# KohakuBlueleaf/UwUDiff

Hardware: AMD Instinct MI355X
Metric: train images/sec (whole node), DiT-S/2 256^2 latent (higher is better)
Workload: dtype bf16; 1 GPU; DiT-S/2 (L12 D384 h6), 4x32x32 synthetic latents + pooled-text cond 1280, eps-MSE, AdamW lr1e-6 wd0.01 cosine; random-init weights; per_gpu_batch=768, global_batch=768, parallelism=dp1

## Files before the change

include/uwu_hip.h:

```cpp
#ifndef UWU_HIP_H
#define UWU_HIP_H

#include <stddef.h>
#include <stdint.h>

#ifdef __cplusplus
extern "C" {
#endif

#define UWU_F32 0
#define UWU_BF16 1
#define UWU_I64 2

#define UWU_OK 0
#define UWU_EINVAL (-1)
#define UWU_ELAUNCH (-2)
#define UWU_ENOTIMPL (-3)

#define UWU_PT_EPSILON 0
#define UWU_PT_V 1
#define UWU_PT_SAMPLE 2
#define UWU_PT_RF 3

#define UWU_LOSS_MSE 0
#define UWU_LOSS_L1 1
#define UWU_LOSS_HUBER 2
#define UWU_LOSS_SMOOTH_L1 3

#define UWU_EPI_NONE 0
#define UWU_EPI_BIAS 1
#define UWU_EPI_BIAS_GELU 2
#define UWU_EPI_DGELU 3
#define UWU_EPI_BIAS_SILU 4
#define UWU_EPI_ACCUM 5

const char* uwu_last_error(void);
int uwu_version(void);
int uwu_env_refresh(void);
int uwu_memset_zero(void* p, uint64_t bytes, void* stream);


int uwu_schedule_gather(const int64_t* timesteps, const float* sigmas_desc, const float* all_snr,
                        const float* alphas_cumprod, int n_train, int B, int snr_mode, float gamma,
                        int debias, float* coef, void* stream);

int uwu_rf_time_to_sigma(const float* u01, float sigma_max, const float* log_sigmas_asc, int n_train,
                         int B, float* coef, float* timesteps, void* stream);

int uwu_qsample(const float* x, const float* noise, const float* coef, int B, int64_t n, float* noisy,
                void* noisy_bf16, void* stream);

int uwu_qsample_norm(const float* x, const float* noise, const float* coef, int B, int64_t n, float vae_mean,
                     float vae_std, float* x_norm, float* noisy, void* stream);

int uwu_philox_raw(uint32_t* out, int64_t n_counters, uint64_t seed, uint64_t offset, void* stream);
int uwu_philox_normal(float* out, int64_t n, uint64_t seed, uint64_t offset, void* stream);
int uwu_draw_timesteps(int64_t* timesteps, int n_train, int B, uint64_t seed, uint64_t offset, void* stream);
int uwu_draw_u01(float* u01, int B, uint64_t seed, uint64_t offset, void* stream);
int uwu_qsample_draw(const float* x, const float* coef, int B, int64_t n, int use_norm, float vae_mean, float vae_std,
                     float* x_norm, float* noise, float* noisy, uint64_t seed, uint64_t offset, void* stream);
int uwu_posterior_draw(const float* moments, int ldm, int B, int latent, int64_t HW, float* z, float* mean_out, float* logvar_out,
                       uint64_t seed, uint64_t offset, void* stream);

int uwu_ctx_place(const void* src, int dtype, const int64_t* mask, float* out, int B, int S, int F, int S_total,
                  int F_total, int s_off, int f_off, void* stream);

int uwu_loss_fwd_bwd(const float* x, const float* noise, const float* xt, const void* model_output,
                     int out_dtype, const float* coef, int pred_type, int target_type, int force_convert,
                     int B, int64_t n, float* losses, float* loss_mean, void* grad_out, float* pred,
                     float* target, void* stream);
int uwu_loss_elem_fwd_bwd(const float* x, const float* noise, const float* xt, const void* model_output,
                          int out_dtype, const float* coef, int pred_type, int target_type, int force_convert,
                          int loss_kind, float loss_param, int B, int64_t n, float* losses, float* loss_mean,
                          void* grad_out, float* pred, float* target, void* stream);

int uwu_scale_inplace(void* y, int dtype, int64_t n, const float* scale, void* stream);
int uwu_scale_into(const void* x, void* y, int dtype, int64_t n, const float* scale, void* stream);
int uwu_cast_i64_to_f32(const int64_t* x, float* y, int64_t n, void* stream);

int uwu_aggregate_concat(const void* emb, const int* starts, void* out, int B, int max_n, int64_t unit_bytes,
                         int elem_size, uint64_t pad_bits, void* stream);
int uwu_aggregate_split(const void* cat, const int* starts, void* out, int B, int max_n, int64_t unit_bytes,
                        void* stream);
int uwu_aggregate_first(const void* emb, const int* starts, void* out, int B, int64_t unit_bytes, void* stream);

int uwu_sampler_step(const float* x, const float* eps_cond, const float* eps_uncond, const float* noise, float* out,
                     float* denoised, int64_t n, float cfg, float sigma, float sigma_down, float sigma_up,
                     float s_noise, void* stream);
int uwu_sampler_combine(const float* base, const float* eps_cond, const float* eps_uncond, const float* noise,
                        float* out, int64_t n, float cfg, float a, float b, float c, void* stream);
int uwu_scale_copy(const float* x, float* y, int64_t n, float scale, void* stream);

int uwu_cfg_input(const float* x, float* y, int B, int64_t n, float c_in, void* stream);
int uwu_sampler_combine_draw(const float* base, const float* eps_cond, const float* eps_uncond, float* out, int64_t n, float cfg,
                             float a, float b, float c, uint64_t seed, uint64_t offset, void* stream);
size_t uwu_latent_finish_ws_bytes(int B, int64_t n);
int uwu_latent_finish(const float* x, float* y, int B, int64_t n, int rescale, float vae_std, float vae_mean, void* ws,
                      size_t ws_bytes, void* stream);
int uwu_image_u8(const void* x, int dtype, void* y, int B, int H, int W, void* stream);

#define UWU_FILTER_BILINEAR 0
#define UWU_FILTER_BICUBIC 1
#define UWU_FILTER_LANCZOS 2
int uwu_resample_ksize(int in_size, int out_size, int filter);
int uwu_resample_coeffs(int in_size, int out_size, int filter, int first, int count, int32_t* coeffs, int32_t* bounds);
size_t uwu_image_resize_crop_ws_bytes(int B, const int32_t* meta, int Ht, int Wt, int filter);
int uwu_image_resize_crop(const void* src, int64_t src_bytes, const int64_t* src_off, const int32_t* meta, const int32_t* tables,
                          int64_t tables_len, const int64_t* tab_off, void* out, int dtype, int B, int Ht, int Wt, int filter,
                          int normalize, void* ws, size_t ws_bytes, void* stream);



int uwu_grad_sqnorm_clip(const float* g, int64_t n, float pre_scale, float max_norm, float* partial,
                         float* out, void* stream);

int uwu_adamw_step(float* p, float* g, float* m, float* v, void* p_bf16, int64_t n, float lr,
                   float beta1, float beta2, float eps, float weight_decay, int step, float pre_scale,
                   const float* clip, int zero_grad, void* stream);

int uwu_lion_step(float* p, float* g, float* m, void* p_bf16, int64_t n, double lr, double beta1, double beta2,
                  double weight_decay, float pre_scale, const float* clip, int zero_grad, void* stream);

int uwu_adamw_fp16_step(float* p, float* g, void* m16, void* v16, void* p_bf16, int64_t n, double lr, double beta1,
                        double beta2, double eps, int step, float pre_scale, const float* clip, int zero_grad,
                        void* stream);

int uwu_param_decay(float* p, void* p_bf16, int64_t n, double factor, void* stream);

int uwu_adamw8_step(float* p, float* g, void* state1, void* state2, float* absmax1, float* absmax2, const float* qmap1,
                    const float* qmap2, void* p_bf16, int64_t n, int64_t e0, int64_t e1, double lr, double beta1, double beta2,
                    double eps, double weight_decay, int step, float pre_scale, const float* clip, int zero_grad, void* stream);

int uwu_lion8_step(float* p, float* g, void* state1, float* absmax1, const float* qmap1, void* p_bf16, int64_t n, int64_t e0,
                   int64_t e1, double lr, double beta1, double beta2, double weight_decay, float pre_scale, const float* clip,
                   int zero_grad, void* stream);

#define UWU_PRODIGY_SCALARS 8
#define UWU_PRODIGY_D 0
#define UWU_PRODIGY_D_MAX 1
#define UWU_PRODIGY_D_NUMERATOR 2
#define UWU_PRODIGY_D_DENOM 3
#define UWU_PRODIGY_D_HAT 4
#define UWU_PRODIGY_K 5
#define UWU_PRODIGY_SKIPPED 6
#define UWU_PRODIGY_DLR 7

int uwu_prodigy_stats_blocks(int64_t n);

int uwu_prodigy_stats(const float* p, float* g, const float* p0, float* exp_avg, float* exp_avg_sq, float* s, int64_t n,
                      const double* scalars, double* ws, int64_t ws_slots, int64_t slot0, double lr, double beta1, double beta2,
                      double beta3, double weight_decay, int decouple, double d0, int use_bias_correction, int safeguard_warmup,
                      float pre_scale, const float* clip, int zero_grad, void* stream);

int uwu_prodigy_finalize(double* scalars, const double* ws, int64_t nslots, double lr, double beta1, double beta2, double beta3,
                         double d0, double d_coef, double growth_rate, int use_bias_correction, void* stream);

int uwu_prodigy_apply(float* p, const float* exp_avg, const float* exp_avg_sq, void* p_bf16, int64_t n, const double* scalars,
                      double eps, double weight_decay, int decouple, void* stream);

int uwu_ema_update(float* avg, const float* p, int64_t n, float keep, float take, void* stream);

int uwu_ema_swap(float* avg, float* p, void* p_bf16, int64_t n, int mode, void* stream);

int uwu_sfadamw_step(float* y, float* g, float* z, float* v, void* p_bf16, int64_t n, double lr_t, double beta1, double beta2,
                     double eps, double weight_decay, double c, double bc2, float pre_scale, const float* clip, int zero_grad,
                     void* stream);

int uwu_sf_average(const float* y, const float* z, float* out, int64_t n, double weight, void* stream);

int uwu_cast_f32_to_bf16(const float* src, void* dst, int64_t n, void* stream);
int uwu_cast_bf16_to_f32(const void* src, float* dst, int64_t n, void* stream);

#define UWU_ADAPTER_NORM 0
#define UWU_ADAPTER_LORA 1
#define UWU_ADAPTER_LOKR 2
#define UWU_ADAPTER_LOKR_LOWRANK 3
int uwu_adapter_merge(const float* base, const float* p, const int64_t* table, const int64_t* blk_start, int nseg,
                      int64_t nblocks, float* eff, void* shadow, void* stream);
int uwu_adapter_grad(const float* dw, int64_t N, int64_t K, int kind, const float* p, float* g, int64_t pa, int64_t pb,
                     int64_t pc, int r, int out_k, int in_n, float scale, float* ws, int64_t ws_elems, void* stream);
int uwu_adapter_dora_norms(const float* base, const float* p, const int64_t* table, const int64_t* table_host,
                           const int64_t* blk_start, int nseg, int64_t nblocks, float* norms, void* stream);
int uwu_adapter_dora_merge(const float* base, const float* p, const int64_t* table, const int64_t* table_host,
                           const int64_t* blk_start, int nseg, int64_t nblocks, const float* norms, float* eff, void* shadow,
                           void* stream);
int uwu_adapter_dora_grad(float* dw, const float* base, int64_t N, int64_t K, int kind, const float* p, float* g, int64_t pa,
                          int64_t pb, int64_t pc, int r, int out_k, int in_n, float scale, int64_t dora_off,
                          const float* norms, int wd_on_out, float* ws, int64_t ws_elems, void* stream);
#define UWU_ADAPTER_CONV_LORA 4
#define UWU_ADAPTER_CONV_TUCKER 5
#define UWU_ADAPTER_CONV_LOKR 6
#define UWU_ADAPTER_CONV_LOKR_LOWRANK 7
int uwu_adapter_conv_merge(const float* base, const float* p, const int64_t* table, const int64_t* table_host,
                           const int64_t* blk_start, const int64_t* form_start, int nseg, int64_t nblocks, int64_t nform,
                           float* tws, int64_t tws_elems, float* eff, void* shadow, void* stream);
int uwu_adapter_conv_grad(const float* dw, int64_t cout_store, int64_t cin_store, int64_t cout, int64_t cin, int kind,
                          const float* p, float* g, int64_t pa, int64_t pb, int64_t pc, int r, int out_k, int in_n,
                          float scale, float* ws, int64_t ws_elems, void* stream);

int uwu_comm_unique_id(void* id128);
int uwu_comm_init(const void* id128, int rank, int world, void** comm);
int uwu_allreduce_flat(void* comm, float* buf, int64_t n, void* stream);
int uwu_comm_destroy(void* comm);


int uwu_gemm(const void* A, const void* B, void* C, void* C2, const float* bias, const void* aux,
             int M, int N, int K, int lda, int ldb, int ldc, int ldaux, int transA, int transB, int dtype,
             int c_dtype, int epilogue, int split_k, void* stream);
const char* uwu_gemm_last_kernel(void);

#define UWU_FP8_E4M3 0
#define UWU_FP8_E5M2 1
size_t uwu_gemm_fp8_scratch_bytes(int M, int N, int K);
int uwu_gemm_fp8(const void* A, const void* B, void* C, void* C2, const float* bias, const void* aux, int M, int N,
                 int K, int lda, int ldb, int ldc, int ldaux, int fmt_a, int epilogue, const float* scale_a,
                 const float* scale_b, void* scratch, size_t scratch_bytes, void* stream);

int uwu_gemm_fp8_emit(const void* A, const void* B, void* C, float* colsum, const float* bias, const void* aux, int M, int N,
                      int K, int lda, int ldb, int ldc, int ldaux, int fmt_a, int epilogue, const float* scale_a,
                      const float* scale_b, void* q8, int ldq, void* q8t, int ldqt, const float* q_scale, float* q_amax,
                      void* stream);

int uwu_conv3x3_implicit_ok(int B, int H, int W, int C, int Cout, int stride, int dtype);
int uwu_conv3x3_fwd(const void* x, const void* w, const float* bias, void* y, int B, int H, int W, int C, int Cout,
                    int stride, int dtype, void* stream);
size_t uwu_conv3x3_s2br_ws_bytes(int B, int H, int W, int C, int Cout, int dtype);
int uwu_conv3x3_s2br_fwd(const void* x, const void* w, const float* bias, void* y, int B, int H, int W, int C, int Cout, int dtype,
                         void* ws, size_t ws_bytes, void* stream);
int uwu_conv3x3_dgrad(const void* dy, const void* w, void* dx, int B, int H, int W, int C, int Cout, int stride, int dtype,
                      void* stream);
size_t uwu_conv3x3_wgrad_scratch_bytes(int C, int Cout, int64_t Mo);
int uwu_conv3x3_wgrad(const void* dy, const void* x, float* dw, float* db, int B, int H, int W, int C, int Cout, int stride,
                      int dtype, void* scratch, size_t scratch_bytes, void* stream);

int uwu_fp8_amax(const void* x, int dtype, int64_t n, float* amax, void* stream);
int uwu_fp8_update_scales(float* amax, float* scale, const int* fmt, int n, float margin, void* stream);
int uwu_fp8_quantize(const void* x, int dtype, int M, int K, int ldx, const float* scale, int fmt, void* out, int ldo,
                     void* out_t, int ldt, float* amax, float* colsum, void* stream);

size_t uwu_gemm_wgrad_scratch_bytes(int M, int N, int K);
int uwu_gemm_wgrad(const void* A, const void* B, float* C, float* bias_grad, int M, int N, int K, int lda, int ldb,
                   int ldc, int dtype, int blocks, void* scratch, size_t scratch_bytes, void* stream);

size_t uwu_gemm_wgrad_pair_scratch_bytes(int M_a, int N_a, int M_b, int N_b, int K);
int uwu_gemm_wgrad_pair(const void* A_a, const void* B_a, float* C_a, float* bias_grad_a, int M_a, int N_a, int lda_a,
                        int ldb_a, int ldc_a, const void* A_b, const void* B_b, float* C_b, float* bias_grad_b, int M_b,
                        int N_b, int lda_b, int ldb_b, int ldc_b, int K, int dtype, int blocks, void* scratch,
                        size_t scratch_bytes, void* stream);

int uwu_gemm_prof_enable(int on);
int uwu_gemm_prof_collect(int kind, double* ms, double* flops, int* launches);

enum {
  UWU_PROF_GEMM_FWD = 0, UWU_PROF_GEMM_DGRAD = 1, UWU_PROF_GEMM_WGRAD = 2, UWU_PROF_GEMM_FC1_GELU = 3,
  UWU_PROF_GEMM_FC2_DGELU = 4, UWU_PROF_ATTN_FWD = 5, UWU_PROF_ATTN_BWD = 6, UWU_PROF_LN_FWD = 7, UWU_PROF_LN_BWD = 8,
  UWU_PROF_CONV = 9, UWU_PROF_OTHER = 10
};
int uwu_prof_enable(int on);
int uwu_prof_collect(int tag, int kind, double* ms, double* flops, double* bytes, int* launches);

int uwu_colsum(const void* X, int dtype, int M, int N, int ldx, float* out, int accumulate, void* stream);

int uwu_skinny_linear_ok(int M, int N, int K);
int uwu_skinny_linear_fwd(const float* X, const float* W, const float* bias, float* Y, float* Y2, int M, int N, int K,
                          int epilogue, void* stream);
int uwu_skinny_linear_dgrad(const float* dY, const float* W, float* dX, int M, int N, int K, void* stream);
int uwu_skinny_linear_wgrad(const float* dY, const float* X, float* dW, float* db, int M, int N, int K, void* stream);
int uwu_colsum_batched(const void* X, int dtype, int batch, int M, int N, int ldx, float* out, int accumulate,
                       void* stream);


int uwu_add_ln_modulate_fwd(const void* x_in, const void* y, const float* gate, const float* shift,
                            const float* scale, int mod_ld, void* x_out, void* h, float* mean, float* rstd,
                            int B, int T, int D, float eps, int affine, int dtype, void* stream);
int uwu_add_ln_modulate_fwd_q8(const void* x_in, const void* y, const float* gate, const float* shift, const float* scale,
                               int mod_ld, void* x_out, void* q8, int ldq, void* q8t, int ldqt, const float* q_scale,
                               float* q_amax, float* mean, float* rstd, int B, int T, int D, float eps, void* stream);


int uwu_add_ln_modulate_bwd(const void* dh, const void* x, const float* mean, const float* rstd,
                            const float* scale, const void* dx_in, const void* y, const float* gate,
                            int mod_ld, void* dx_out, void* dy, float* dshift, float* dscale, float* dgate,
                            int B, int T, int D, int affine, int dtype, void* stream);


int uwu_attention_fwd(const void* q, const void* k, const void* v, void* o, float* lse, int B, int Tq, int Tk,
                      int H, int d, int ldq, int ldk, int ldv, int ldo, float scale, int dtype, void* stream);
int uwu_attention_d512_fwd(const void* q, const void* k, const void* v, void* o, int B, int T, int ldq, int ldk, int ldv, int ldo,
                           float scale, int dtype, void* stream);
int uwu_attention_causal_fwd(const void* q, const void* k, const void* v, const int64_t* key_mask, void* o, int B, int T, int H,
                             int d, int ldq, int ldk, int ldv, int ldo, float scale, int dtype, void* stream);
int uwu_text_embed(const int64_t* ids, const void* tok_table, const void* pos_table, void* out, int B, int T, int D, int vocab,
                   int dtype, void* stream);
#define UWU_ACT_QUICK_GELU 0
#define UWU_ACT_GELU_ERF 1
int uwu_bias_act_fwd(const void* x, const float* bias, void* y, int M, int N, int ld, int kind, int dtype, void* stream);
int uwu_text_pool(const int64_t* ids, const void* h, void* pooled, int B, int T, int D, int eos_id, int dtype, void* stream);
int uwu_attention_relbias_fwd(const void* q, const void* k, const void* v, const float* rel_bias, const int64_t* key_mask, void* o,
                              int B, int T, int H, int d, int ldq, int ldk, int ldv, int ldo, float scale, int dtype, void* stream);
int uwu_attention_bidir_fwd(const void* q, const void* k, const void* v, const int64_t* key_mask, void* o, int B, int T, int H, int d,
                            int ldq, int ldk, int ldv, int ldo, float scale, int dtype, void* stream);
int uwu_clip_patches(const void* images, int in_u8, void* out, int B, int S, int p, int ld, int normalize, const float* mean,
                     const float* std, int dtype, void* stream);
int uwu_vit_embed(const void* patch_out, const void* class_embedding, const void* pos_table, void* out, int B, int T, int D, int dtype,
                  void* stream);
int uwu_clip_score_accum(const void* image_embeds, const void* text_embeds, float* scores, double* acc, int B, int P, int dtype,
                         void* stream);
int uwu_timestep_stats_accum(const float* losses, const void* timesteps, int t_dtype, const float* loss_mean, int B, int n_steps,
                             double* stats, double* totals, void* stream);

int uwu_conv2d_ok(int B, int H, int W, int C, int Cout, int KH, int KW, int stride, int ph, int pw, int ldx, int xoff, int ldy, int yoff,
                  int dtype);
size_t uwu_conv2d_ws_bytes(int B, int H, int W, int C, int Cout, int KH, int KW, int stride, int ph, int pw, int ldx, int xoff, int ldy,
                           int yoff, int dtype);
int uwu_conv2d_fwd(const void* x, const void* w, const float* bias, void* y, int B, int H, int W, int C, int Cout, int KH, int KW,
                   int stride, int ph, int pw, int ldx, int xoff, int ldy, int yoff, int relu, int dtype, void* ws, size_t ws_bytes,
                   void* stream);
int uwu_inception_stem(const void* images, int in_u8, void* out, int B, int H, int W, int dtype, void* stream);
#define UWU_POOL_MAX_S2 0
#define UWU_POOL_MAX_S1P1 1
#define UWU_POOL_AVG_S1P1 2
int uwu_pool2d_fwd(const void* x, void* y, int B, int H, int W, int C, int mode, int ldx, int xoff, int ldy, int yoff, int dtype,
                   void* stream);
int uwu_relu_rows(void* y, int64_t M, int N, int ldy, int yoff, int dtype, void* stream);
int uwu_global_avgpool(const void* x, float* out, int B, int HW, int C, int ldx, int dtype, void* stream);
int uwu_fid_stats_accum(const float* features, double* acc, int B, int D, void* stream);

int uwu_add_rmsnorm_fwd(const void* x_in, const void* y, const float* weight, void* x_out, void* n_out, int M, int D, float eps,
                        int dtype, void* stream);
#define UWU_GATE_GELU_TANH 0
int uwu_gated_act_fwd(const void* u, void* out, int M, int F, int ldu, int ldo, int kind, int dtype, void* stream);
int uwu_t5_rel_bias(const float* weight, const int32_t* bucket, float* out, int num_buckets, int H, int n, void* stream);
int uwu_token_embed(const int64_t* ids, const void* tok_table, void* out, int B, int T, int D, int vocab, int dtype, void* stream);
int uwu_attention_bwd(const void* q, const void* k, const void* v, const void* o, const void* dO,
                      const float* lse, float* delta, void* dq, void* dk, void* dv, int B, int Tq, int Tk, int H,
                      int d, int ldq, int ldk, int ldv, int ldo, float scale, int dtype, void* stream);
int uwu_attention_bias_fwd(const void* q, const void* k, const void* v, const float* key_bias, void* o, float* lse,
                           int B, int Tq, int Tk, int H, int d, int ldq, int ldk, int ldv, int ldo, float scale,
                           int dtype, void* stream);
int uwu_attention_bias_bwd(const void* q, const void* k, const void* v, const float* key_bias, const void* o,
                           const void* dO, const float* lse, float* delta, void* dq, void* dk, void* dv, int B,
                           int Tq, int Tk, int H, int d, int ldq, int ldk, int ldv, int ldo, float scale, int dtype,
                           void* stream);
int uwu_attention_route(int pass, int Tq, int Tk, int d, int ldq, int ldk, int ldv, int ldo, int dtype);

int uwu_axial_rope_fwd(const void* x, const float* pos, const float* fh, const float* fw, void* y, int64_t rows,
                       int H, int d, int ldx, int dtype, void* stream);
int uwu_axial_rope_bwd(const void* x, const void* dy, const float* pos, const float* fh, const float* fw, void* dx,
                       float* dfh, float* dfw, int64_t rows, int H, int d, int ldx, int dtype, void* stream);

int uwu_axial_rope_bwd_shared(const void* x, const void* dy, const float* pos, int pos_rows, const float* fh, const float* fw,
                              void* dx, float* dfh, float* dfw, int64_t rows, int H, int d, int ldx, int dtype, void* stream);
int uwu_axial_rope_table(const float* pos, const float* fh, const float* fw, float* tab, int T, int H, int d, int ldt,
                         void* stream);
int uwu_attention_rope_fwd(const void* q, const void* k, const void* v, const float* rope_tab, void* o, float* lse, int B,
                           int T, int H, int d, int ldq, int ldk, int ldv, int ldo, int ldt, float scale, int dtype,
                           void* stream);
int uwu_attention_rope_bwd(const void* q, const void* k, const void* v, const float* rope_tab, const void* o, const void* dO,
                           const float* lse, void* dq, void* dk, void* dv, int B, int T, int H, int d, int ldq, int ldk,
                           int ldv, int ldo, int ldt, float scale, int dtype, void* stream);


int uwu_timestep_embedding(const float* t, int B, int dim, float max_period, void* out, int dtype,
                           void* stream);
int uwu_silu_fwd(const void* x, void* y, int64_t n, int dtype, void* stream);
int uwu_silu_bwd(const void* x, const void* dy, void* dx, int64_t n, int dtype, void* stream);

int uwu_add(const void* a, const void* b, void* out, int64_t n, int dtype, void* stream);
int uwu_transpose_bf16(const void* src, void* dst, int rows, int cols, int ld_src, int ld_dst, void* stream);

int uwu_patchify(const float* img, void* tok, int B, int C, int H, int W, int p, int dtype, void* stream);
int uwu_unpatchify(const void* tok, int dtype, float* img, int B, int C, int H, int W, int p, void* stream);
int uwu_add_pos(void* x, const float* pos, int B, int T, int D, int dtype, void* stream);


int uwu_groupnorm_fwd(const void* x, const float* gamma, const float* beta, void* y, float* mean, float* rstd,
                      int B, int HW, int C, int G, float eps, int silu, int dtype, void* stream);
size_t uwu_groupnorm_fwd_det_ws_bytes(int B, int HW, int C, int G);
int uwu_groupnorm_fwd_det(const void* x, const float* gamma, const float* beta, void* y, float* mean, float* rstd, void* ws,
                          size_t ws_bytes, int B, int HW, int C, int G, float eps, int silu, int dtype, void* stream);
int uwu_groupnorm_bwd(const void* dy, const void* x, const float* mean, const float* rstd, const float* gamma,
                      const float* beta, void* dx, float* dgamma, float* dbeta, float* ws, int B, int HW, int C, int G,
                      int silu, int dtype, void* stream);
int uwu_im2col3x3(const void* x, void* col, int B, int H, int W, int C, int stride, int dtype, void* stream);
int uwu_col2im3x3(const void* dcol, void* dx, int B, int H, int W, int C, int stride, int dtype, void* stream);
int uwu_geglu_fwd(const void* hg, void* out, int64_t M, int F, int dtype, void* stream);
int uwu_geglu_bwd(const void* hg, const void* dout, void* dhg, int64_t M, int F, int dtype, void* stream);
int uwu_upsample2x(const void* src, void* dst, int B, int H, int W, int C, int backward, int dtype, void* stream);
int uwu_add_rowvec(void* x, const void* v, int B, int HW, int C, int dtype, void* stream);
int uwu_nchw_to_cl(const float* nchw, void* cl, int B, int C, int HW, int dtype, void* stream);
int uwu_cl_to_nchw(const void* cl, float* nchw, int B, int C, int HW, int dtype, void* stream);


typedef struct uwu_dit_desc {
  int32_t B, T, D, H, L, mlp_ratio, in_ch, out_ch, patch, img, dtype, cond_dim, freq_dim;
  float ln_eps;
  int32_t mod_total;
  const void* w;
  const float* w32;
  float* g32;
  int64_t off_patch_w, off_patch_b, off_t_w1, off_t_b1, off_t_w2, off_t_b2, off_y_w, off_y_b,
      off_mod_w, off_mod_b, off_final_w, off_final_b;
  int64_t off_layer0, layer_stride;
  const float* pos;
  void* ws;
  size_t ws_bytes;
  void* const* layer_done;
  void* side_stream;
  int32_t rope;
  int64_t off_rope_h, off_rope_w;
  const float* pos_xy;
  int32_t fp8;
  float* f8_scale;
  float* f8_amax;
  const int32_t* f8_fmt;
  int32_t checkpoint;
} uwu_dit_desc;

size_t uwu_dit_workspace_bytes(const uwu_dit_desc* d);
int uwu_dit_forward(const uwu_dit_desc* d, const float* noisy, const float* t, const float* cond,
                    float* out, void* stream);
int uwu_dit_backward(const uwu_dit_desc* d, const float* dout, void* stream);
int uwu_dit_backward_cond(const uwu_dit_desc* d, const float* cond, void* stream);
int64_t uwu_dit_layer_param_stride(int D, int mlp_ratio);

#ifdef __cplusplus
}
#endif
#endif
```

uwudiff_amd/csrc/dit.cpp:

```cpp
#include <hip/hip_runtime.h>
#include <math.h>
#include <stddef.h>
#include <stdint.h>
#include <stdlib.h>

#include "../../include/uwu_hip.h"
#include "env.h"

void uwu_set_error(const char* fmt, ...);

namespace {

constexpr int WGRAD_BLOCKS = 512;

struct Layout {
  size_t es;
  int64_t M, D, D3, D4, Kp, Ko;
  size_t feat, t_pre, t_h, temb, yemb, c, sc, mod;
  size_t sc16, dmod16;
  size_t tok, xe;
  size_t layer0, layer_stride;
  bool ckpt;
  size_t keep, scratch0;
  size_t o_x0, o_m1, o_r1, o_h1, o_qkv, o_lse, o_ao, o_y1, o_x1, o_m2, o_r2, o_h2, o_u, o_f, o_y2;
  size_t o_rope;
  size_t o_h1t, o_aot, o_h2t, o_ft;
  size_t xF, mF, rF, hF, otok;
  size_t dx, dy, dh, dqkv, dao, du, delta, dotok, dmod, dsc, dc, dth, dtp;
  size_t w2t;
  size_t wsc, wsc_bytes;
  size_t x8, x8t, dy8, dy8t, w8, w8_layer;
  size_t total;
};

inline size_t al(size_t x) { return (x + 255) & ~(size_t)255; }

Layout make_layout(const uwu_dit_desc& d) {
  Layout L{};
  L.es = d.dtype == UWU_BF16 ? 2 : 4;
  L.M = (int64_t)d.B * d.T;
  L.D = d.D;
  L.D3 = 3 * (int64_t)d.D;
  L.D4 = (int64_t)d.mlp_ratio * d.D;
  L.Kp = (int64_t)d.in_ch * d.patch * d.patch;
  L.Ko = (int64_t)d.out_ch * d.patch * d.patch;
  size_t p = 0;
  auto take = [&](size_t bytes) { size_t o = p; p = al(p + bytes); return o; };
  const size_t f4 = 4;
  L.feat = take((size_t)d.B * d.freq_dim * f4);
  L.t_pre = take((size_t)d.B * d.D * f4);
  L.t_h = take((size_t)d.B * d.D * f4);
  L.temb = take((size_t)d.B * d.D * f4);
  L.yemb = take((size_t)d.B * d.D * f4);
  L.c = take((size_t)d.B * d.D * f4);
  L.sc = take((size_t)d.B * d.D * f4);
  L.mod = take((size_t)d.B * d.mod_total * f4);
  L.sc16 = take((size_t)d.B * d.D * 2);
  L.dmod16 = take((size_t)d.B * d.mod_total * 2);
  L.tok = take(L.M * L.Kp * L.es);
  L.xe = take(L.M * L.D * L.es);
  size_t q = 0;
  auto sub = [&](size_t bytes) { size_t o = q; q = al(q + bytes); return o; };
  L.o_x0 = sub(L.M * L.D * L.es);
  L.o_m1 = sub(L.M * f4);
  L.o_r1 = sub(L.M * f4);
  L.o_h1 = sub(L.M * L.D * L.es);
  L.o_qkv = sub(L.M * L.D3 * L.es);
  L.o_lse = sub((size_t)d.B * d.H * d.T * f4);
  L.o_ao = sub(L.M * L.D * L.es);
  L.o_y1 = sub(L.M * L.D * L.es);
  L.o_x1 = sub(L.M * L.D * L.es);
  L.o_m2 = sub(L.M * f4);
  L.o_r2 = sub(L.M * f4);
  L.o_h2 = sub(L.M * L.D * L.es);
  L.o_u = sub(L.M * L.D4 * L.es);
  L.o_f = sub(L.M * L.D4 * L.es);
  L.o_y2 = sub(L.M * L.D * L.es);
  if (d.rope) L.o_rope = sub((size_t)d.T * d.D * f4);
  if (d.fp8) {
    L.o_h1t = sub(L.M * L.D);
    L.o_aot = sub(L.M * L.D);
    L.o_h2t = sub(L.M * L.D);
    L.o_ft = sub(L.M * L.D4);
  }
  L.keep = L.o_h1;
  L.ckpt = d.checkpoint != 0;
  L.layer_stride = L.ckpt ? L.keep : q;
  L.layer0 = p;
  p += (size_t)d.L * L.layer_stride;
  if (L.ckpt) L.scratch0 = take(q);
  L.xF = take(L.M * L.D * L.es);
  L.mF = take(L.M * f4);
  L.rF = take(L.M * f4);
  L.hF = take(L.M * L.D * L.es);
  L.otok = take(L.M * L.Ko * L.es);
  L.dx = take(L.M * L.D * L.es);
  L.dy = take(L.M * L.D * L.es);
  L.dh = take(L.M * L.D * L.es);
  L.dqkv = take(L.M * L.D3 * L.es);
  L.dao = take(L.M * L.D * L.es);
  L.du = take(L.M * L.D4 * L.es);
  L.w2t = take((size_t)L.D4 * d.D * 2);
  L.delta = take((size_t)d.B * d.H * d.T * f4);
  L.dotok = take(L.M * L.Ko * L.es);
  L.dmod = take((size_t)d.B * d.mod_total * f4);
  L.dsc = take((size_t)d.B * d.D * f4);
  L.dc = take((size_t)d.B * d.D * f4);
  L.dth = take((size_t)d.B * d.D * f4);
  L.dtp = take((size_t)d.B * d.D * f4);
  L.wsc_bytes = uwu_gemm_wgrad_scratch_bytes((int)L.D4, d.D, (int)L.M);
  for (const size_t t : {uwu_gemm_wgrad_scratch_bytes(d.D, (int)L.D4, (int)L.M),
                         uwu_gemm_wgrad_scratch_bytes((int)L.D3, d.D, (int)L.M),
                         uwu_gemm_wgrad_scratch_bytes(d.D, d.D, (int)L.M),
                         uwu_gemm_wgrad_pair_scratch_bytes((int)L.D4, d.D, d.D, (int)L.D4, (int)L.M),
                         uwu_gemm_wgrad_pair_scratch_bytes((int)L.D3, d.D, d.D, d.D, (int)L.M)})
    if (t > L.wsc_bytes) L.wsc_bytes = t;
  if (d.fp8) {
    for (const size_t t : {uwu_gemm_fp8_scratch_bytes((int)L.D4, d.D, (int)L.M), uwu_gemm_fp8_scratch_bytes(d.D, (int)L.D4, (int)L.M),
                           uwu_gemm_fp8_scratch_bytes((int)L.D3, d.D, (int)L.M), uwu_gemm_fp8_scratch_bytes(d.D, d.D, (int)L.M)})
      if (t > L.wsc_bytes) L.wsc_bytes = t;
  }
  L.wsc_bytes = (L.wsc_bytes + 255) & ~(size_t)255;
  L.wsc = take(L.wsc_bytes * (L.M <= 16384 ? 4 : 1));
  if (d.fp8) {
    L.x8 = take(L.M * L.D4);
    L.x8t = 0;
    L.dy8 = take(L.M * L.D4);
    L.dy8t = take(L.M * L.D4);
    L.w8_layer = al((size_t)24 * d.D * d.D);
    L.w8 = take((size_t)d.L * L.w8_layer);
  }
  L.total = p;
  return L;
}

int check_desc(const uwu_dit_desc* d) {
  if (!d) { uwu_set_error("dit: null descriptor"); return UWU_EINVAL; }
  if (d->B <= 0 || d->T <= 0 || d->D <= 0 || d->H <= 0 || d->L <= 0 || d->D % d->H || d->D % 8 ||
      d->img % d->patch || (d->img / d->patch) * (d->img / d->patch) != d->T || d->mlp_ratio <= 0 ||
      d->freq_dim <= 0 || d->freq_dim % 8) {
    uwu_set_error("dit: inconsistent shape B=%d T=%d D=%d H=%d L=%d img=%d patch=%d", d->B, d->T, d->D, d->H, d->L,
                  d->img, d->patch);
    return UWU_EINVAL;
  }
  if (d->dtype != UWU_F32 && d->dtype != UWU_BF16) { uwu_set_error("dit: bad dtype"); return UWU_EINVAL; }
  if (d->mod_total != d->L * 6 * d->D + 2 * d->D) { uwu_set_error("dit: mod_total mismatch"); return UWU_EINVAL; }
  if ((d->in_ch * d->patch * d->patch) % 8 || (d->out_ch * d->patch * d->patch) % 8 || (d->cond_dim % 8)) {
    uwu_set_error("dit: C*p*p and cond_dim must be multiples of 8");
    return UWU_EINVAL;
  }
  if (!d->w || !d->w32 || !d->pos || !d->ws) { uwu_set_error("dit: null buffer"); return UWU_EINVAL; }
  if (d->rope && (d->dtype != UWU_BF16 || d->D / d->H != 64 || d->T % 64 || d->T > 256 || !d->pos_xy)) {
    uwu_set_error("dit: the fused axial-RoPE attention needs bf16, head dim 64, T a multiple of 64 up to 256 and pos_xy");
    return UWU_EINVAL;
  }
  if (d->fp8) {
    if (d->fp8 < 0 || d->fp8 > 2 || d->dtype != UWU_BF16 || d->D % 128 || d->mlp_ratio != 4 || ((int64_t)d->B * d->T) % 128 ||
        !d->f8_scale || !d->f8_amax || !d->f8_fmt) {
      uwu_set_error("dit: fp8 mode needs bf16 activations, D %% 128 == 0, B*T %% 128 == 0, mlp_ratio 4 and the scale / amax / fmt arrays");
      return UWU_EINVAL;
    }
  }
  return UWU_OK;
}

#define RUN(expr)              \
  do {                         \
    int rc_ = (expr);          \
    if (rc_ != UWU_OK) return rc_; \
  } while (0)

int lin_fwd(const void* X, const void* W, const float* bias, void* Y, void* Y2, int M, int N, int K, int dt, int cdt,
            int epi, void* st) {
  return uwu_gemm(X, W, Y, Y2, bias, nullptr, M, N, K, K, K, N, 0, 0, 0, dt, cdt, epi, 1, st);
}
int lin_fwd32(const float* X, const float* W, const float* bias, float* Y, float* Y2, int M, int N, int K, int epi, void* st) {
  if (M <= 16 && N <= 4096 && uwu_skinny_linear_ok(M, N, K)) return uwu_skinny_linear_fwd(X, W, bias, Y, Y2, M, N, K, epi, st);
  return lin_fwd(X, W, bias, Y, Y2, M, N, K, UWU_F32, UWU_F32, epi, st);
}
int lin_dgrad(const void* dY, const void* W, void* dX, const void* aux, int M, int N, int K, int dt, void* st,
              float* colsum = nullptr) {
  return uwu_gemm(dY, W, dX, colsum, nullptr, aux, M, K, N, N, K, K, K, 0, 1, dt, dt,
                  aux ? UWU_EPI_DGELU : UWU_EPI_NONE, 1, st);
}
static bool mod_bf16(const uwu_dit_desc& d) {
  return d.dtype == UWU_BF16 && d.B >= 64 && d.mod_total % 8 == 0;
}
int lin_dgrad_splitk(const void* dY, const void* W, float* dX, int M, int N, int K, void* st) {
  if (hipMemsetAsync(dX, 0, (size_t)M * K * sizeof(float), (hipStream_t)st) != hipSuccess) {
    uwu_set_error("dgrad_splitk: memset failed");
    return UWU_ELAUNCH;
  }
  const int tiles = ((M + 127) / 128) * ((K + 127) / 128);
  const int ktiles = (N + 31) / 32;
  int split = (512 + tiles - 1) / tiles;
  if (split > ktiles) split = ktiles;
  return uwu_gemm(dY, W, dX, nullptr, nullptr, nullptr, M, K, N, N, K, K, 0, 0, 1, UWU_F32, UWU_F32, UWU_EPI_ACCUM, split,
                  st);
}
int lin_wgrad(const void* dY, const void* X, float* dW, int M, int N, int K, int dt, void* st, void* scratch = nullptr,
              size_t scratch_bytes = 0, float* db = nullptr) {
  if (dt == UWU_BF16 && scratch && uwu_gemm_wgrad_scratch_bytes(N, K, M) <= scratch_bytes)
    return uwu_gemm_wgrad(dY, X, dW, db, N, K, M, N, K, K, dt, WGRAD_BLOCKS, scratch, scratch_bytes, st);
  if (db) {
    const int rc = uwu_colsum(dY, dt, M, N, N, db, 1, st);
    if (rc != UWU_OK) return rc;
  }
  const int tiles = ((N + 127) / 128) * ((K + 127) / 128);
  const int bk = dt == UWU_BF16 ? 64 : 32;
  const int ktiles = (M + bk - 1) / bk;
  const int target = tiles >= 16 ? 768 : 256;
  int split = (target + tiles - 1) / tiles;
  if (split > ktiles) split = ktiles;
  if (split < 1) split = 1;
  return uwu_gemm(dY, X, dW, nullptr, nullptr, nullptr, N, K, M, N, K, K, 0, 1, 1, dt, UWU_F32, UWU_EPI_ACCUM, split, st);
}

bool wgrad_pair_ok(int M, int Na, int Ka, int Nb, int Kb, size_t scratch_bytes) {
  const size_t need = uwu_gemm_wgrad_pair_scratch_bytes(Na, Ka, Nb, Kb, M);
  return need && need <= scratch_bytes;
}
int lin_wgrad_pair(const void* dYa, const void* Xa, float* dWa, float* dba, int Na, int Ka, const void* dYb, const void* Xb,
                   float* dWb, float* dbb, int Nb, int Kb, int M, void* st, void* scratch, size_t scratch_bytes) {
  return uwu_gemm_wgrad_pair(dYa, Xa, dWa, dba, Na, Ka, Na, Ka, Ka, dYb, Xb, dWb, dbb, Nb, Kb, Nb, Kb, Kb, M, UWU_BF16,
                             WGRAD_BLOCKS, scratch, scratch_bytes, st);
}

int lin_wgrad32(const float* dY, const float* X, float* dW, float* db, int M, int N, int K, void* st) {
  if (M <= 16 && uwu_skinny_linear_ok(M, N, K)) return uwu_skinny_linear_wgrad(dY, X, dW, db, M, N, K, st);
  RUN(lin_wgrad(dY, X, dW, M, N, K, UWU_F32, st));
  return uwu_colsum(dY, UWU_F32, M, N, N, db, 1, st);
}

struct F8 {
  int mode;
  float* scale;
  float* amax;
  const int32_t* fmt;
  char *x8, *x8t, *dy8, *dy8t, *wsc, *w8;
  size_t wsc_bytes, w8_layer;
  int D;
  void* st;
  int role(int l, int r) const { return 12 * l + r; }
  char* w(int l, int i, bool t) const {
    static const int off[4] = {0, 6, 8, 16}, sz[4] = {3, 1, 4, 4};
    return w8 + (size_t)l * w8_layer + ((size_t)off[i] + (t ? sz[i] : 0)) * D * D;
  }
  int quant(const void* x, int dtype, int M, int K, int role, void* out, void* out_t, float* colsum, bool have_scale) const {
    const int fm = role % 12 >= 4 && role % 12 < 8 ? UWU_FP8_E5M2 : UWU_FP8_E4M3;
    if (!have_scale && mode == 1) {
      RUN(uwu_fp8_amax(x, dtype, (int64_t)M * K, amax + role, st));
      RUN(uwu_fp8_update_scales(amax + role, scale + role, fmt + role, 1, 1.f, st));
    }
    return uwu_fp8_quantize(x, dtype, M, K, K, scale + role, fm, out, K, out_t, M,
                            (!have_scale && mode == 2) ? amax + role : nullptr, colsum, st);
  }
};

int f8_fwd(const F8& f, const void* X, void* Xt_save, const void* W8, const float* bias, void* Y, void* Y2, int M, int N, int K,
           int rx, int rw, int epi) {
  if (X) RUN(f.quant(X, UWU_BF16, M, K, rx, f.x8, Xt_save, nullptr, false));
  return uwu_gemm_fp8(f.x8, W8, Y, Y2, bias, nullptr, M, N, K, K, K, N, 0, UWU_FP8_E4M3, epi, f.scale + rx, f.scale + rw,
                      nullptr, 0, f.st);
}
int f8_bwd(const F8& f, const void* dY, const void* X8t, const void* W8t, float* dW, float* db, void* dX, const void* aux,
           float* dcol, int M, int N, int K, int rdy, int rx, int rw, const void* dY8 = nullptr, const void* dY8t = nullptr,
           int rnext = -1, void* q8 = nullptr, void* q8t = nullptr) {
  if (dY) {
    RUN(f.quant(dY, UWU_BF16, M, N, rdy, f.dy8, f.dy8t, db, false));
    dY8 = f.dy8;
    dY8t = f.dy8t;
  }
  RUN(uwu_gemm_fp8(dY8t, X8t, dW, nullptr, nullptr, nullptr, N, K, M, M, M, K, 0, UWU_FP8_E5M2, UWU_EPI_ACCUM,
                   f.scale + rdy, f.scale + rx, f.wsc, f.wsc_bytes, f.st));
  if (rnext >= 0)
    return uwu_gemm_fp8_emit(dY8, W8t, nullptr, dcol, nullptr, aux, M, K, N, N, N, K, K, UWU_FP8_E5M2, UWU_EPI_DGELU, f.scale + rdy,
                             f.scale + rw, q8, K, q8t, M, f.scale + rnext, f.amax + rnext, f.st);
  if (!dX) return UWU_OK;
  return uwu_gemm_fp8(dY8, W8t, dX, dcol, nullptr, aux, M, K, N, N, N, K, K, UWU_FP8_E5M2, aux ? UWU_EPI_DGELU : UWU_EPI_NONE,
                      f.scale + rdy, f.scale + rw, nullptr, 0, f.st);
}
static bool f8_emit(const uwu_dit_desc& d);
static int ln_fwd_f8(const uwu_dit_desc& d, const F8& f, const void* x_in, const void* y, const float* gate, const float* shift,
                     const float* scale, int ML, void* x_out, void* h, void* h8t, int role, float* mean, float* rstd, void* st) {
  const int64_t M = (int64_t)d.B * d.T;
  if (f8_emit(d) && d.D <= 1536 && M % 64 == 0) {
    const int rc = uwu_add_ln_modulate_fwd_q8(x_in, y, gate, shift, scale, ML, x_out, f.x8, d.D, h8t, (int)M, f.scale + role,
                                              f.amax + role, mean, rstd, d.B, d.T, d.D, d.ln_eps, st);
    return rc == UWU_OK ? 1 : rc;
  }
  const int rc = uwu_add_ln_modulate_fwd(x_in, y, gate, shift, scale, ML, x_out, h, mean, rstd, d.B, d.T, d.D, d.ln_eps, 0, d.dtype, st);
  return rc == UWU_OK ? 0 : rc;
}
static bool f8_emit(const uwu_dit_desc& d) {
  static UwuEnv on("UWU_F8_EMIT");
  return !on.get().is('0') && d.fp8 == 2;
}

struct Fork {
  hipStream_t main;
  hipStream_t side[4];
  hipEvent_t ev[8];
  bool on = false;
};
bool fork_resources(Fork& f, hipStream_t caller_side) {
  static hipEvent_t pool[8];
  static hipStream_t extra[3];
  static bool made = false;
  if (!made) {
    for (auto& e : pool)
      if (hipEventCreateWithFlags(&e, hipEventDisableTiming | hipEventReleaseToDevice) != hipSuccess) return false;
    for (auto& x : extra)
      if (hipStreamCreateWithFlags(&x, hipStreamNonBlocking) != hipSuccess) return false;
    made = true;
  }
  for (int i = 0; i < 8; ++i) f.ev[i] = pool[i];
  static int n_side = -1;
  if (n_side < 0) {
    const char* e = getenv("UWU_DIT_SIDE_STREAMS");
    n_side = e ? atoi(e) : 1;
    if (n_side < 1 || n_side > 4) n_side = 1;
  }
  for (int i = 0; i < 3; ++i) f.side[i] = n_side == 1 ? caller_side : extra[i % (n_side - 1)];
  f.side[3] = caller_side;
  return true;
}
template <typename F>
int on_side(const Fork& f, int slot, F&& fn) {
  if (!f.on) return fn(static_cast<void*>(f.main), 0);
  if (hipEventRecord(f.ev[slot], f.main) != hipSuccess || hipStreamWaitEvent(f.side[slot], f.ev[slot], 0) != hipSuccess) {
    uwu_set_error("dit_backward: stream fork failed");
    return UWU_ELAUNCH;
  }
  const int rc = fn(static_cast<void*>(f.side[slot]), f.side[slot] == f.side[3] ? 0 : slot + 1);
  if (rc != UWU_OK) return rc;
  if (hipEventRecord(f.ev[4 + slot], f.side[slot]) != hipSuccess) { uwu_set_error("dit_backward: stream fork failed"); return UWU_ELAUNCH; }
  return UWU_OK;
}
int join_side(const Fork& f, int slot) {
  if (f.on && hipStreamWaitEvent(f.main, f.ev[4 + slot], 0) != hipSuccess) {
    uwu_set_error("dit_backward: stream join failed");
    return UWU_ELAUNCH;
  }
  return UWU_OK;
}

struct Ptrs {
  char* ws;
  const Layout& L;
  template <typename T = void>
  T* at(size_t off) const { return reinterpret_cast<T*>(ws + off); }
  template <typename T = void>
  T* lay(int l, size_t sub) const {
    if (L.ckpt && sub >= L.keep) return reinterpret_cast<T*>(ws + L.scratch0 + sub);
    return reinterpret_cast<T*>(ws + L.layer0 + (size_t)l * L.layer_stride + sub);
  }
};

struct LayerW {
  const void *qkv_w, *o_w, *fc1_w, *fc2_w;
  const float *qkv_b, *o_b, *fc1_b, *fc2_b;
  int64_t off_qkv_w, off_qkv_b, off_o_w, off_o_b, off_fc1_w, off_fc1_b, off_fc2_w, off_fc2_b;
};

inline int64_t pad64(int64_t n) { return (n + 63) & ~(int64_t)63; }

LayerW layer_weights(const uwu_dit_desc& d, int l) {
  LayerW w{};
  const int64_t D = d.D, D4 = (int64_t)d.mlp_ratio * d.D;
  int64_t o = d.off_layer0 + (int64_t)l * d.layer_stride;
  w.off_qkv_w = o; o += pad64(3 * D * D);
  w.off_qkv_b = o; o += pad64(3 * D);
  w.off_o_w = o; o += pad64(D * D);
  w.off_o_b = o; o += pad64(D);
  w.off_fc1_w = o; o += pad64(D4 * D);
  w.off_fc1_b = o; o += pad64(D4);
  w.off_fc2_w = o; o += pad64(D * D4);
  w.off_fc2_b = o; o += pad64(D);
  const size_t es = d.dtype == UWU_BF16 ? 2 : 4;
  const char* wb = static_cast<const char*>(d.w);
  w.qkv_w = wb + w.off_qkv_w * es;
  w.o_w = wb + w.off_o_w * es;
  w.fc1_w = wb + w.off_fc1_w * es;
  w.fc2_w = wb + w.off_fc2_w * es;
  w.qkv_b = d.w32 + w.off_qkv_b;
  w.o_b = d.w32 + w.off_o_b;
  w.fc1_b = d.w32 + w.off_fc1_b;
  w.fc2_b = d.w32 + w.off_fc2_b;
  return w;
}


int block_forward(const uwu_dit_desc& d, const Layout& L, const Ptrs& P, const F8& f8, int l, bool recompute, void* st) {
  const int dt = d.dtype, B = d.B, T = d.T, D = d.D, M = (int)L.M, D3 = (int)L.D3, D4 = (int)L.D4;
  const size_t es = L.es;
  const float* w32 = d.w32;
  const int ML = d.mod_total;
  const float* mod = P.at<float>(L.mod);
  const float scale = 1.f / sqrtf((float)(D / d.H));
  const LayerW w = layer_weights(d, l);
  const float* m = mod + (int64_t)l * 6 * D;
  void* x0 = P.lay(l, L.o_x0);
  int h1q = 0, h2q = 0;
  if (d.fp8) {
    if (l == 0 || recompute) {
      h1q = ln_fwd_f8(d, f8, x0, nullptr, nullptr, m + 0, m + D, ML, x0, P.lay(l, L.o_h1), P.lay(l, L.o_h1t), f8.role(l, 0),
                      P.lay<float>(l, L.o_m1), P.lay<float>(l, L.o_r1), st);
    } else {
      const float* mp = mod + (int64_t)(l - 1) * 6 * D;
      h1q = ln_fwd_f8(d, f8, P.lay(l - 1, L.o_x1), P.lay(l - 1, L.o_y2), mp + 5 * D, m + 0, m + D, ML, x0, P.lay(l, L.o_h1),
                      P.lay(l, L.o_h1t), f8.role(l, 0), P.lay<float>(l, L.o_m1), P.lay<float>(l, L.o_r1), st);
    }
    if (h1q < 0) return h1q;
  } else
  if (l == 0 || recompute) {
    RUN(uwu_add_ln_modulate_fwd(x0, nullptr, nullptr, m + 0, m + D, ML, x0, P.lay(l, L.o_h1),
                                P.lay<float>(l, L.o_m1), P.lay<float>(l, L.o_r1), B, T, D, d.ln_eps, 0, dt, st));
  } else {
    const float* mp = mod + (int64_t)(l - 1) * 6 * D;
    RUN(uwu_add_ln_modulate_fwd(P.lay(l - 1, L.o_x1), P.lay(l - 1, L.o_y2), mp + 5 * D, m + 0, m + D, ML, x0,
                                P.lay(l, L.o_h1), P.lay<float>(l, L.o_m1), P.lay<float>(l, L.o_r1), B, T, D,
                                d.ln_eps, 0, dt, st));
  }
  if (d.fp8) RUN(f8_fwd(f8, h1q ? nullptr : P.lay(l, L.o_h1), P.lay(l, L.o_h1t), f8.w(l, 0, false), w.qkv_b, P.lay(l, L.o_qkv), nullptr, M, D3, D, f8.role(l, 0), f8.role(l, 8), UWU_EPI_BIAS));
  else RUN(lin_fwd(P.lay(l, L.o_h1), w.qkv_w, w.qkv_b, P.lay(l, L.o_qkv), nullptr, M, D3, D, dt, dt, UWU_EPI_BIAS, st));
  char* qkv = P.lay<char>(l, L.o_qkv);
  if (d.rope) {
    const int64_t fo = (int64_t)l * d.H * (D / d.H / 4);
    RUN(uwu_axial_rope_table(d.pos_xy, w32 + d.off_rope_h + fo, w32 + d.off_rope_w + fo, P.lay<float>(l, L.o_rope), T, d.H,
                             D / d.H, D, st));
    RUN(uwu_attention_rope_fwd(qkv, qkv + (size_t)D * es, qkv + (size_t)2 * D * es, P.lay<float>(l, L.o_rope), P.lay(l, L.o_ao),
                               P.lay<float>(l, L.o_lse), B, T, d.H, D / d.H, D3, D3, D3, D, D, scale, dt, st));
  } else
  RUN(uwu_attention_fwd(qkv, qkv + (size_t)D * es, qkv + (size_t)2 * D * es, P.lay(l, L.o_ao), P.lay<float>(l, L.o_lse),
                        B, T, T, d.H, D / d.H, D3, D3, D3, D, scale, dt, st));
  if (d.fp8) RUN(f8_fwd(f8, P.lay(l, L.o_ao), P.lay(l, L.o_aot), f8.w(l, 1, false), w.o_b, P.lay(l, L.o_y1), nullptr, M, D, D, f8.role(l, 1), f8.role(l, 9), UWU_EPI_BIAS));
  else RUN(lin_fwd(P.lay(l, L.o_ao), w.o_w, w.o_b, P.lay(l, L.o_y1), nullptr, M, D, D, dt, dt, UWU_EPI_BIAS, st));
  if (d.fp8) {
    h2q = ln_fwd_f8(d, f8, x0, P.lay(l, L.o_y1), m + 2 * D, m + 3 * D, m + 4 * D, ML, P.lay(l, L.o_x1), P.lay(l, L.o_h2),
                    P.lay(l, L.o_h2t), f8.role(l, 2), P.lay<float>(l, L.o_m2), P.lay<float>(l, L.o_r2), st);
    if (h2q < 0) return h2q;
  } else
  RUN(uwu_add_ln_modulate_fwd(x0, P.lay(l, L.o_y1), m + 2 * D, m + 3 * D, m + 4 * D, ML, P.lay(l, L.o_x1),
                              P.lay(l, L.o_h2), P.lay<float>(l, L.o_m2), P.lay<float>(l, L.o_r2), B, T, D, d.ln_eps,
                              0, dt, st));
  if (d.fp8) {
    if (f8_emit(d)) {
      const int r2 = f8.role(l, 2), r3 = f8.role(l, 3);
      if (!h2q) RUN(f8.quant(P.lay(l, L.o_h2), UWU_BF16, M, D, r2, f8.x8, P.lay(l, L.o_h2t), nullptr, false));
      RUN(uwu_gemm_fp8_emit(f8.x8, f8.w(l, 2, false), P.lay(l, L.o_u), nullptr, w.fc1_b, nullptr, M, D4, D, D, D, D4, 0, UWU_FP8_E4M3,
                            UWU_EPI_BIAS_GELU, f8.scale + r2, f8.scale + f8.role(l, 10), f8.dy8, D4, P.lay(l, L.o_ft), M, f8.scale + r3,
                            f8.amax + r3, st));
      RUN(uwu_gemm_fp8(f8.dy8, f8.w(l, 3, false), P.lay(l, L.o_y2), nullptr, w.fc2_b, nullptr, M, D, D4, D4, D4, D, 0, UWU_FP8_E4M3,
                       UWU_EPI_BIAS, f8.scale + r3, f8.scale + f8.role(l, 11), nullptr, 0, st));
      return UWU_OK;
    }
    RUN(f8_fwd(f8, h2q ? nullptr : P.lay(l, L.o_h2), P.lay(l, L.o_h2t), f8.w(l, 2, false), w.fc1_b, P.lay(l, L.o_u), P.lay(l, L.o_f), M, D4, D, f8.role(l, 2), f8.role(l, 10), UWU_EPI_BIAS_GELU));
    RUN(f8_fwd(f8, P.lay(l, L.o_f), P.lay(l, L.o_ft), f8.w(l, 3, false), w.fc2_b, P.lay(l, L.o_y2), nullptr, M, D, D4, f8.role(l, 3), f8.role(l, 11), UWU_EPI_BIAS));
  } else {
    RUN(lin_fwd(P.lay(l, L.o_h2), w.fc1_w, w.fc1_b, P.lay(l, L.o_u), P.lay(l, L.o_f), M, D4, D, dt, dt,
                UWU_EPI_BIAS_GELU, st));
    RUN(lin_fwd(P.lay(l, L.o_f), w.fc2_w, w.fc2_b, P.lay(l, L.o_y2), nullptr, M, D, D4, dt, dt, UWU_EPI_BIAS, st));
  }
  return UWU_OK;
}

}

extern "C" size_t uwu_dit_workspace_bytes(const uwu_dit_desc* d) {
  if (!d) return 0;
  return make_layout(*d).total;
}

extern "C" int64_t uwu_dit_layer_param_stride(int D, int mlp_ratio) {
  const int64_t d = D, d4 = (int64_t)mlp_ratio * D;
  return pad64(3 * d * d) + pad64(3 * d) + pad64(d * d) + pad64(d) + pad64(d4 * d) + pad64(d4) + pad64(d * d4) + pad64(d);
}

extern "C" int uwu_dit_forward(const uwu_dit_desc* dp, const float* noisy, const float* t, const float* cond,
                               float* out, void* st) {
  RUN(check_desc(dp));
  const uwu_dit_desc& d = *dp;
  if (!noisy || !t || !out) { uwu_set_error("dit_forward: null tensor"); return UWU_EINVAL; }
  if ((d.cond_dim > 0) != (cond != nullptr)) { uwu_set_error("dit_forward: cond / cond_dim mismatch"); return UWU_EINVAL; }
  const Layout L = make_layout(d);
  if (d.ws_bytes < L.total) { uwu_set_error("dit_forward: workspace too small (%zu < %zu)", d.ws_bytes, L.total); return UWU_EINVAL; }
  if (d.layer_stride != uwu_dit_layer_param_stride(d.D, d.mlp_ratio)) { uwu_set_error("dit: layer_stride mismatch"); return UWU_EINVAL; }
  Ptrs P{static_cast<char*>(d.ws), L};
  const int dt = d.dtype, B = d.B, T = d.T, D = d.D, M = (int)L.M, D3 = (int)L.D3, D4 = (int)L.D4;
  const size_t es = L.es;
  const char* wb = static_cast<const char*>(d.w);
  const float* w32 = d.w32;
  const int ML = d.mod_total;

  RUN(uwu_timestep_embedding(t, B, d.freq_dim, 10000.f, P.at(L.feat), UWU_F32, st));
  RUN(lin_fwd32(P.at<float>(L.feat), w32 + d.off_t_w1, w32 + d.off_t_b1, P.at<float>(L.t_pre), P.at<float>(L.t_h), B, D,
                d.freq_dim, UWU_EPI_BIAS_SILU, st));
  RUN(lin_fwd32(P.at<float>(L.t_h), w32 + d.off_t_w2, w32 + d.off_t_b2, P.at<float>(L.temb), nullptr, B, D, D, UWU_EPI_BIAS, st));
  const void* cptr = P.at(L.temb);
  if (cond) {
    RUN(lin_fwd32(cond, w32 + d.off_y_w, w32 + d.off_y_b, P.at<float>(L.yemb), nullptr, B, D, d.cond_dim, UWU_EPI_BIAS, st));
    RUN(uwu_add(P.at(L.temb), P.at(L.yemb), P.at(L.c), (int64_t)B * D, UWU_F32, st));
    cptr = P.at(L.c);
  }
  RUN(uwu_silu_fwd(cptr, P.at(L.sc), (int64_t)B * D, UWU_F32, st));
  if (mod_bf16(d)) {
    RUN(uwu_cast_f32_to_bf16(P.at<float>(L.sc), P.at(L.sc16), (int64_t)B * D, st));
    RUN(lin_fwd(P.at(L.sc16), wb + d.off_mod_w * es, w32 + d.off_mod_b, P.at(L.mod), nullptr, B, ML, D, UWU_BF16, UWU_F32, UWU_EPI_BIAS, st));
  } else {
    RUN(lin_fwd32(P.at<float>(L.sc), w32 + d.off_mod_w, w32 + d.off_mod_b, P.at<float>(L.mod), nullptr, B, ML, D, UWU_EPI_BIAS, st));
  }
  const float* mod = P.at<float>(L.mod);

  const F8 f8{d.fp8, d.f8_scale, d.f8_amax, d.f8_fmt, P.at<char>(L.x8), nullptr, P.at<char>(L.dy8),
              P.at<char>(L.dy8t), P.at<char>(L.wsc), P.at<char>(L.w8), L.wsc_bytes, L.w8_layer, d.D, st};
  if (d.fp8) {
    const F8 fw{2, d.f8_scale, d.f8_amax, d.f8_fmt, nullptr, nullptr, nullptr, nullptr, nullptr, f8.w8, 0, L.w8_layer, d.D, st};
    const int rows[4] = {D3, D, D4, D}, cols[4] = {D, D, D, D4};
    for (int l = 0; l < d.L; ++l) {
      const LayerW w = layer_weights(d, l);
      const void* ws4[4] = {w.qkv_w, w.o_w, w.fc1_w, w.fc2_w};
      for (int i = 0; i < 4; ++i)
        RUN(uwu_fp8_amax(ws4[i], UWU_BF16, (int64_t)rows[i] * cols[i], d.f8_amax + fw.role(l, 8 + i), st));
    }
    RUN(uwu_fp8_update_scales(d.f8_amax, d.f8_scale, d.f8_fmt, 12 * d.L, 1.f, st));
    for (int l = 0; l < d.L; ++l) {
      const LayerW w = layer_weights(d, l);
      const void* ws4[4] = {w.qkv_w, w.o_w, w.fc1_w, w.fc2_w};
      for (int i = 0; i < 4; ++i)
        RUN(fw.quant(ws4[i], UWU_BF16, rows[i], cols[i], fw.role(l, 8 + i), fw.w(l, i, false), fw.w(l, i, true), nullptr, true));
    }
  }

  RUN(uwu_patchify(noisy, P.at(L.tok), B, d.in_ch, d.img, d.img, d.patch, dt, st));
  RUN(lin_fwd(P.at(L.tok), wb + d.off_patch_w * es, w32 + d.off_patch_b, P.lay(0, L.o_x0), nullptr, M, D, (int)L.Kp, dt,
              dt, UWU_EPI_BIAS, st));
  RUN(uwu_add_pos(P.lay(0, L.o_x0), d.pos, B, T, D, dt, st));

  for (int l = 0; l < d.L; ++l) RUN(block_forward(d, L, P, f8, l, false, st));
  {
    const int l = d.L - 1;
    const float* mp = mod + (int64_t)l * 6 * D;
    const float* mf = mod + (int64_t)d.L * 6 * D;
    RUN(uwu_add_ln_modulate_fwd(P.lay(l, L.o_x1), P.lay(l, L.o_y2), mp + 5 * D, mf + 0, mf + D, ML, P.at(L.xF),
                                P.at(L.hF), P.at<float>(L.mF), P.at<float>(L.rF), B, T, D, d.ln_eps, 0, dt, st));
    RUN(lin_fwd(P.at(L.hF), wb + d.off_final_w * es, w32 + d.off_final_b, P.at(L.otok), nullptr, M, (int)L.Ko, D, dt, dt,
                UWU_EPI_BIAS, st));
    RUN(uwu_unpatchify(P.at(L.otok), dt, out, B, d.out_ch, d.img, d.img, d.patch, st));
  }
  return UWU_OK;
}

extern "C" int uwu_dit_backward(const uwu_dit_desc* dp, const float* dout, void* st) {
  RUN(check_desc(dp));
  const uwu_dit_desc& d = *dp;
  if (!dout || !d.g32) { uwu_set_error("dit_backward: null tensor"); return UWU_EINVAL; }
  const Layout L = make_layout(d);
  if (d.ws_bytes < L.total) { uwu_set_error("dit_backward: workspace too small"); return UWU_EINVAL; }
  Ptrs P{static_cast<char*>(d.ws), L};
  const int dt = d.dtype, B = d.B, T = d.T, D = d.D, M = (int)L.M, D3 = (int)L.D3, D4 = (int)L.D4;
  const size_t es = L.es;
  const char* wb = static_cast<const char*>(d.w);
  const float* w32 = d.w32;
  float* g = d.g32;
  const int ML = d.mod_total;
  const float* mod = P.at<float>(L.mod);
  float* dmod = P.at<float>(L.dmod);
  if (hipMemsetAsync(dmod, 0, (size_t)B * ML * sizeof(float), (hipStream_t)st) != hipSuccess) {
    uwu_set_error("dit_backward: memset failed");
    return UWU_ELAUNCH;
  }
  const float scale = 1.f / sqrtf((float)(D / d.H));
  const F8 f8{d.fp8, d.f8_scale, d.f8_amax, d.f8_fmt, P.at<char>(L.x8), nullptr, P.at<char>(L.dy8),
              P.at<char>(L.dy8t), P.at<char>(L.wsc), P.at<char>(L.w8), L.wsc_bytes, L.w8_layer, d.D, st};
  Fork fk{static_cast<hipStream_t>(st), {}, {}, false};
  fk.on = d.side_stream && d.side_stream != st && !d.fp8 && dt == UWU_BF16 && M <= 16384 && !L.ckpt &&
          fork_resources(fk, static_cast<hipStream_t>(d.side_stream));
  char* const wsc = P.at<char>(L.wsc);
  bool side_used[4] = {false, false, false, false};
  const bool pairs = !fk.on && !d.fp8 && dt == UWU_BF16 && M > 16384 && !L.ckpt;
  const bool pair_fc = pairs && wgrad_pair_ok(M, D4, D, D, D4, L.wsc_bytes);
  const bool pair_attn = pairs && wgrad_pair_ok(M, D3, D, D, D, L.wsc_bytes);

  RUN(uwu_patchify(dout, P.at(L.dotok), B, d.out_ch, d.img, d.img, d.patch, dt, st));
  RUN(lin_wgrad(P.at(L.dotok), P.at(L.hF), g + d.off_final_w, M, (int)L.Ko, D, dt, st));
  RUN(uwu_colsum(P.at(L.dotok), dt, M, (int)L.Ko, (int)L.Ko, g + d.off_final_b, 1, st));
  RUN(lin_dgrad(P.at(L.dotok), wb + d.off_final_w * es, P.at(L.dh), nullptr, M, (int)L.Ko, D, dt, st));
  {
    const int l = d.L - 1;
    const float* mp = mod + (int64_t)l * 6 * D;
    const float* mf = mod + (int64_t)d.L * 6 * D;
    float* dmp = dmod + (int64_t)l * 6 * D;
    float* dmf = dmod + (int64_t)d.L * 6 * D;
    RUN(uwu_add_ln_modulate_bwd(P.at(L.dh), P.at(L.xF), P.at<float>(L.mF), P.at<float>(L.rF), mf + D, nullptr,
                                P.lay(l, L.o_y2), mp + 5 * D, ML, P.at(L.dx), P.at(L.dy), dmf + 0, dmf + D, dmp + 5 * D,
                                B, T, D, 0, dt, st));
  }
  for (int l = d.L - 1; l >= 0; --l) {
    const LayerW w = layer_weights(d, l);
    const float* m = mod + (int64_t)l * 6 * D;
    float* dm = dmod + (int64_t)l * 6 * D;
    if (d.fp8) {
      if (f8_emit(d)) {
        RUN(f8_bwd(f8, P.at(L.dy), P.lay(l, L.o_ft), f8.w(l, 3, true), g + w.off_fc2_w, g + w.off_fc2_b, nullptr, P.lay(l, L.o_u),
                   g + w.off_fc1_b, M, D, D4, f8.role(l, 7), f8.role(l, 3), f8.role(l, 11), nullptr, nullptr, f8.role(l, 6), f8.x8, f8.dy8t));
        RUN(f8_bwd(f8, nullptr, P.lay(l, L.o_h2t), f8.w(l, 2, true), g + w.off_fc1_w, nullptr, P.at(L.dh), nullptr, nullptr, M, D4, D,
                   f8.role(l, 6), f8.role(l, 2), f8.role(l, 10), f8.x8, f8.dy8t));
      } else {
      RUN(f8_bwd(f8, P.at(L.dy), P.lay(l, L.o_ft), f8.w(l, 3, true), g + w.off_fc2_w, g + w.off_fc2_b, P.at(L.du), P.lay(l, L.o_u),
                 g + w.off_fc1_b, M, D, D4, f8.role(l, 7), f8.role(l, 3), f8.role(l, 11)));
      RUN(f8_bwd(f8, P.at(L.du), P.lay(l, L.o_h2t), f8.w(l, 2, true), g + w.off_fc1_w, nullptr, P.at(L.dh), nullptr, nullptr, M, D4, D,
                 f8.role(l, 6), f8.role(l, 2), f8.role(l, 10)));
      }
    } else {
    if (!pair_fc) {
    RUN(on_side(fk, 0, [&](void* s2, int k) {
      return lin_wgrad(P.at(L.dy), P.lay(l, L.o_f), g + w.off_fc2_w, M, D, D4, dt, s2, wsc + (size_t)k * L.wsc_bytes, L.wsc_bytes, g + w.off_fc2_b);
    }));
    side_used[0] = true;
    }
    if (side_used[1]) RUN(join_side(fk, 1));
    if (dt == UWU_BF16 && D == 384 && M % 256 == 0 && M >= 256 * 256 && D4 % 64 == 0 && D4 >= 1024 && D4 <= 2048) {
      RUN(uwu_transpose_bf16(w.fc2_w, P.at(L.w2t), D, D4, D4, D, st));
      RUN(uwu_gemm(P.at(L.dy), P.at(L.w2t), P.at(L.du), nullptr, nullptr, P.lay(l, L.o_u), M, D4, D, D, D, D4, D4, 0, 0, dt, dt,
                   UWU_EPI_DGELU, 1, st));
    } else {
      RUN(lin_dgrad(P.at(L.dy), w.fc2_w, P.at(L.du), P.lay(l, L.o_u), M, D, D4, dt, st, nullptr));
    }
    if (pair_fc) {
      RUN(lin_wgrad_pair(P.at(L.du), P.lay(l, L.o_h2), g + w.off_fc1_w, g + w.off_fc1_b, D4, D, P.at(L.dy), P.lay(l, L.o_f),
                         g + w.off_fc2_w, g + w.off_fc2_b, D, D4, M, st, wsc, L.wsc_bytes));
    } else {
    RUN(on_side(fk, 1, [&](void* s2, int k) {
      return lin_wgrad(P.at(L.du), P.lay(l, L.o_h2), g + w.off_fc1_w, M, D4, D, dt, s2, wsc + (size_t)k * L.wsc_bytes, L.wsc_bytes, g + w.off_fc1_b);
    }));
    side_used[1] = true;
    }
    RUN(lin_dgrad(P.at(L.du), w.fc1_w, P.at(L.dh), nullptr, M, D4, D, dt, st));
    RUN(join_side(fk, 0));
    }
    RUN(uwu_add_ln_modulate_bwd(P.at(L.dh), P.lay(l, L.o_x1), P.lay<float>(l, L.o_m2), P.lay<float>(l, L.o_r2), m + 4 * D,
                                P.at(L.dx), P.lay(l, L.o_y1), m + 2 * D, ML, P.at(L.dx), P.at(L.dy), dm + 3 * D,
                                dm + 4 * D, dm + 2 * D, B, T, D, 0, dt, st));
    if (d.fp8) {
      RUN(f8_bwd(f8, P.at(L.dy), P.lay(l, L.o_aot), f8.w(l, 1, true), g + w.off_o_w, g + w.off_o_b, P.at(L.dao), nullptr, nullptr, M, D, D,
                 f8.role(l, 5), f8.role(l, 1), f8.role(l, 9)));
    } else {
    if (!pair_attn) {
    RUN(on_side(fk, 2, [&](void* s2, int k) {
      return lin_wgrad(P.at(L.dy), P.lay(l, L.o_ao), g + w.off_o_w, M, D, D, dt, s2, wsc + (size_t)k * L.wsc_bytes, L.wsc_bytes, g + w.off_o_b);
    }));
    side_used[2] = true;
    }
    RUN(lin_dgrad(P.at(L.dy), w.o_w, P.at(L.dao), nullptr, M, D, D, dt, st));
    if (side_used[3]) RUN(join_side(fk, 3));
    }
    char* qkv = P.lay<char>(l, L.o_qkv);
    char* dqkv = P.at<char>(L.dqkv);
    if (d.rope) {
      const int64_t fo = (int64_t)l * d.H * (D / d.H / 4);
      RUN(uwu_attention_rope_bwd(qkv, qkv + (size_t)D * es, qkv + (size_t)2 * D * es, P.lay<float>(l, L.o_rope), P.lay(l, L.o_ao),
                                 P.at(L.dao), P.lay<float>(l, L.o_lse), dqkv, dqkv + (size_t)D * es, dqkv + (size_t)2 * D * es,
                                 B, T, d.H, D / d.H, D3, D3, D3, D, D, scale, dt, st));
      for (int qk = 0; qk < 2; ++qk)
        RUN(uwu_axial_rope_bwd_shared(qkv + (size_t)qk * D * es, dqkv + (size_t)qk * D * es, d.pos_xy, T,
                                      w32 + d.off_rope_h + fo, w32 + d.off_rope_w + fo, dqkv + (size_t)qk * D * es,
                                      g + d.off_rope_h + fo, g + d.off_rope_w + fo, (int64_t)M, d.H, D / d.H, D3, dt, st));
    } else
    RUN(uwu_attention_bwd(qkv, qkv + (size_t)D * es, qkv + (size_t)2 * D * es, P.lay(l, L.o_ao), P.at(L.dao),
                          P.lay<float>(l, L.o_lse), P.at<float>(L.delta), dqkv, dqkv + (size_t)D * es,
                          dqkv + (size_t)2 * D * es, B, T, T, d.H, D / d.H, D3, D3, D3, D, scale, dt, st));
    if (d.fp8) {
      RUN(f8_bwd(f8, dqkv, P.lay(l, L.o_h1t), f8.w(l, 0, true), g + w.off_qkv_w, g + w.off_qkv_b, P.at(L.dh), nullptr, nullptr, M, D3, D,
                 f8.role(l, 4), f8.role(l, 0), f8.role(l, 8)));
    } else if (pair_attn) {
      RUN(lin_wgrad_pair(dqkv, P.lay(l, L.o_h1), g + w.off_qkv_w, g + w.off_qkv_b, D3, D, P.at(L.dy), P.lay(l, L.o_ao),
                         g + w.off_o_w, g + w.off_o_b, D, D, M, st, wsc, L.wsc_bytes));
    } else {
    RUN(on_side(fk, 3, [&](void* s2, int k) {
      return lin_wgrad(dqkv, P.lay(l, L.o_h1), g + w.off_qkv_w, M, D3, D, dt, s2, wsc + (size_t)k * L.wsc_bytes, L.wsc_bytes, g + w.off_qkv_b);
    }));
    side_used[3] = true;
    }
    if (fk.on && d.layer_done && d.layer_done[l])
      for (int k = 0; k < 3; ++k)
        if (fk.side[k] != fk.side[3] && hipStreamWaitEvent(fk.side[3], fk.ev[4 + k], 0) != hipSuccess) {
          uwu_set_error("dit_backward: stream join failed");
          return UWU_ELAUNCH;
        }
    if (d.layer_done && d.layer_done[l] &&
        hipEventRecord(static_cast<hipEvent_t>(d.layer_done[l]), fk.on ? fk.side[3] : static_cast<hipStream_t>(st)) != hipSuccess) {
      uwu_set_error("dit_backward: hipEventRecord(layer_done[%d]) failed", l);
      return UWU_ELAUNCH;
    }
    if (!d.fp8) RUN(lin_dgrad(dqkv, w.qkv_w, P.at(L.dh), nullptr, M, D3, D, dt, st));
    if (!d.fp8) RUN(join_side(fk, 2));
    if (L.ckpt && l > 0) RUN(block_forward(d, L, P, f8, l - 1, true, st));
    if (l > 0) {
      const float* mp = mod + (int64_t)(l - 1) * 6 * D;
      float* dmp = dmod + (int64_t)(l - 1) * 6 * D;
      RUN(uwu_add_ln_modulate_bwd(P.at(L.dh), P.lay(l, L.o_x0), P.lay<float>(l, L.o_m1), P.lay<float>(l, L.o_r1), m + D,
                                  P.at(L.dx), P.lay(l - 1, L.o_y2), mp + 5 * D, ML, P.at(L.dx), P.at(L.dy), dm + 0,
                                  dm + D, dmp + 5 * D, B, T, D, 0, dt, st));
    } else {
      RUN(uwu_add_ln_modulate_bwd(P.at(L.dh), P.lay(l, L.o_x0), P.lay<float>(l, L.o_m1), P.lay<float>(l, L.o_r1), m + D,
                                  P.at(L.dx), nullptr, nullptr, ML, P.at(L.dx), nullptr, dm + 0, dm + D, nullptr, B, T, D, 0, dt, st));
    }
  }
  if (fk.on)
    for (int k = 0; k < 4; ++k) RUN(join_side(fk, k));
  RUN(lin_wgrad(P.at(L.dx), P.at(L.tok), g + d.off_patch_w, M, D, (int)L.Kp, dt, st));
  RUN(uwu_colsum(P.at(L.dx), dt, M, D, D, g + d.off_patch_b, 1, st));

  if (mod_bf16(d)) {
    RUN(uwu_cast_f32_to_bf16(dmod, P.at(L.dmod16), (int64_t)B * ML, st));
    RUN(lin_wgrad(P.at(L.dmod16), P.at(L.sc16), g + d.off_mod_w, B, ML, D, UWU_BF16, st));
    RUN(uwu_colsum(dmod, UWU_F32, B, ML, ML, g + d.off_mod_b, 1, st));
    if (hipMemsetAsync(P.at(L.dsc), 0, (size_t)B * D * sizeof(float), (hipStream_t)st) != hipSuccess) {
      uwu_set_error("dit_backward: memset failed");
      return UWU_ELAUNCH;
    }
    {
      const int tiles = ((B + 127) / 128) * ((D + 127) / 128), ktiles = (ML + 63) / 64;
      int split = (512 + tiles - 1) / tiles;
      if (split > ktiles) split = ktiles;
      RUN(uwu_gemm(P.at(L.dmod16), wb + d.off_mod_w * es, P.at(L.dsc), nullptr, nullptr, nullptr, B, D, ML, ML, D, D, 0, 0, 1, UWU_BF16,
                   UWU_F32, UWU_EPI_ACCUM, split, st));
    }
  } else {
    RUN(lin_wgrad32(dmod, P.at<float>(L.sc), g + d.off_mod_w, g + d.off_mod_b, B, ML, D, st));
    RUN(lin_dgrad_splitk(dmod, w32 + d.off_mod_w, P.at<float>(L.dsc), B, ML, D, st));
  }
  const void* cptr = d.cond_dim > 0 ? P.at(L.c) : P.at(L.temb);
  RUN(uwu_silu_bwd(cptr, P.at(L.dsc), P.at(L.dc), (int64_t)B * D, UWU_F32, st));
  if (d.cond_dim > 0) {
  }
  RUN(lin_wgrad32(P.at<float>(L.dc), P.at<float>(L.t_h), g + d.off_t_w2, g + d.off_t_b2, B, D, D, st));
  if (B <= 16 && uwu_skinny_linear_ok(B, D, D) && D <= 512) RUN(uwu_skinny_linear_dgrad(P.at<float>(L.dc), w32 + d.off_t_w2, P.at<float>(L.dth), B, D, D, st));
  else RUN(lin_dgrad(P.at(L.dc), w32 + d.off_t_w2, P.at(L.dth), nullptr, B, D, D, UWU_F32, st));
  RUN(uwu_silu_bwd(P.at(L.t_pre), P.at(L.dth), P.at(L.dtp), (int64_t)B * D, UWU_F32, st));
  RUN(lin_wgrad32(P.at<float>(L.dtp), P.at<float>(L.feat), g + d.off_t_w1, g + d.off_t_b1, B, D, d.freq_dim, st));
  return UWU_OK;
}

extern "C" int uwu_dit_backward_cond(const uwu_dit_desc* dp, const float* cond, void* st) {
  RUN(check_desc(dp));
  const uwu_dit_desc& d = *dp;
  if (d.cond_dim <= 0) return UWU_OK;
  if (!cond || !d.g32) { uwu_set_error("dit_backward_cond: null tensor"); return UWU_EINVAL; }
  const Layout L = make_layout(d);
  Ptrs P{static_cast<char*>(d.ws), L};
  return lin_wgrad32(P.at<float>(L.dc), cond, d.g32 + d.off_y_w, d.g32 + d.off_y_b, d.B, d.D, d.cond_dim, st);
}
```

uwudiff_amd/csrc/embed.hip:

```cpp
#include "common.h"

namespace {

template <typename T>
__global__ void timestep_embedding_kernel(const float* __restrict__ t, int B, int dim, float max_period,
                                          T* __restrict__ out) {
  const int half = dim >> 1;
  const int i = blockIdx.x * blockDim.x + threadIdx.x;
  if (i >= B * half) return;
  const int b = i / half, j = i - b * half;
  const float f = expf(-logf(max_period) * (float)j / (float)half);
  const float a = t[b] * f;
  out[(int64_t)b * dim + j] = from_f32<T>(cosf(a));
  out[(int64_t)b * dim + half + j] = from_f32<T>(sinf(a));
}

template <typename T>
__global__ void silu_fwd_kernel(const T* __restrict__ x, T* __restrict__ y, int64_t n4) {
  const int64_t stride = (int64_t)gridDim.x * blockDim.x;
  for (int64_t i = (int64_t)blockIdx.x * blockDim.x + threadIdx.x; i < n4; i += stride) {
    f32x4 v = load4(x + 4 * i);
#pragma unroll
    for (int e = 0; e < 4; ++e) v[e] = silu_f(v[e]);
    store4(y + 4 * i, v);
  }
}
template <typename T>
__global__ void silu_bwd_kernel(const T* __restrict__ x, const T* __restrict__ dy, T* __restrict__ dx, int64_t n4) {
  const int64_t stride = (int64_t)gridDim.x * blockDim.x;
  for (int64_t i = (int64_t)blockIdx.x * blockDim.x + threadIdx.x; i < n4; i += stride) {
    f32x4 v = load4(x + 4 * i), g = load4(dy + 4 * i);
#pragma unroll
    for (int e = 0; e < 4; ++e) g[e] *= dsilu_f(v[e]);
    store4(dx + 4 * i, g);
  }
}

template <typename T, bool TO_TOKENS>
__global__ void patch_kernel(float* __restrict__ img, T* __restrict__ tok, int B, int C, int H, int W, int p) {
  const int gh = H / p, gw = W / p, kp = C * p * p;
  const int64_t total = (int64_t)B * gh * gw * kp;
  const int64_t stride = (int64_t)gridDim.x * blockDim.x;
  for (int64_t i = (int64_t)blockIdx.x * blockDim.x + threadIdx.x; i < total; i += stride) {
    int64_t m = i / kp;
    int k = (int)(i - m * kp);
    int tw = (int)(m % gw);
    int64_t r = m / gw;
    int th = (int)(r % gh);
    int b = (int)(r / gh);
    int pw = k % p, ph = (k / p) % p, c = k / (p * p);
    int64_t src = (((int64_t)b * C + c) * H + (th * p + ph)) * W + (tw * p + pw);
    if (TO_TOKENS)
      tok[i] = from_f32<T>(img[src]);
    else
      img[src] = to_f32(tok[i]);
  }
}

template <typename T>
__global__ void add_kernel(const T* __restrict__ a, const T* __restrict__ b, T* __restrict__ o, int64_t n4) {
  const int64_t stride = (int64_t)gridDim.x * blockDim.x;
  for (int64_t i = (int64_t)blockIdx.x * blockDim.x + threadIdx.x; i < n4; i += stride)
    store4(o + 4 * i, load4(a + 4 * i) + load4(b + 4 * i));
}

template <typename T>
__global__ void add_pos_kernel(T* __restrict__ x, const float* __restrict__ pos, int64_t total4, int64_t td4) {
  const int64_t stride = (int64_t)gridDim.x * blockDim.x;
  for (int64_t i = (int64_t)blockIdx.x * blockDim.x + threadIdx.x; i < total4; i += stride) {
    f32x4 v = load4(x + 4 * i), pv = load4(pos + 4 * (i % td4));
    store4(x + 4 * i, v + pv);
  }
}

}

#define DISPATCH_T(dtype, NAME, ...)                                                    \
  if ((dtype) == UWU_F32) { NAME(float, __VA_ARGS__); }                                  \
  else if ((dtype) == UWU_BF16) { NAME(bf16_t, __VA_ARGS__); }                           \
  else { uwu_set_error("bad dtype %d", (int)(dtype)); return UWU_EINVAL; }

extern "C" int uwu_timestep_embedding(const float* t, int B, int dim, float max_period, void* out, int dtype,
                                      void* stream) {
  UWU_CHECK_ARG(t && out && B > 0 && dim > 0 && dim % 2 == 0, "timestep_embedding: bad args");
  hipStream_t st = (hipStream_t)stream;
  const int n = B * dim / 2;
#define TE(T, ...) hipLaunchKernelGGL((timestep_embedding_kernel<T>), dim3(cdiv(n, 256)), dim3(256), 0, st, t, B, dim, max_period, (T*)out)
  DISPATCH_T(dtype, TE, 0)
#undef TE
  UWU_LAUNCH_CHECK("timestep_embedding");
  return UWU_OK;
}

extern "C" int uwu_silu_fwd(const void* x, void* y, int64_t n, int dtype, void* stream) {
  UWU_CHECK_ARG(x && y && n > 0 && n % 4 == 0, "silu_fwd: n must be a positive multiple of 4");
  hipStream_t st = (hipStream_t)stream;
#define SF(T, ...) hipLaunchKernelGGL((silu_fwd_kernel<T>), dim3(ew_grid(n / 4, 256)), dim3(256), 0, st, (const T*)x, (T*)y, n / 4)
  DISPATCH_T(dtype, SF, 0)
#undef SF
  UWU_LAUNCH_CHECK("silu_fwd");
  return UWU_OK;
}

extern "C" int uwu_silu_bwd(const void* x, const void* dy, void* dx, int64_t n, int dtype, void* stream) {
  UWU_CHECK_ARG(x && dy && dx && n > 0 && n % 4 == 0, "silu_bwd: n must be a positive multiple of 4");
  hipStream_t st = (hipStream_t)stream;
#define SB(T, ...) hipLaunchKernelGGL((silu_bwd_kernel<T>), dim3(ew_grid(n / 4, 256)), dim3(256), 0, st, (const T*)x, (const T*)dy, (T*)dx, n / 4)
  DISPATCH_T(dtype, SB, 0)
#undef SB
  UWU_LAUNCH_CHECK("silu_bwd");
  return UWU_OK;
}

extern "C" int uwu_patchify(const float* img, void* tok, int B, int C, int H, int W, int p, int dtype, void* stream) {
  UWU_CHECK_ARG(img && tok && B > 0 && C > 0 && p > 0 && H % p == 0 && W % p == 0, "patchify: bad shape");
  hipStream_t st = (hipStream_t)stream;
  const int64_t total = (int64_t)B * C * H * W;
#define PF(T, ...) hipLaunchKernelGGL((patch_kernel<T, true>), dim3(ew_grid(total, 256)), dim3(256), 0, st, const_cast<float*>(img), (T*)tok, B, C, H, W, p)
  DISPATCH_T(dtype, PF, 0)
#undef PF
  UWU_LAUNCH_CHECK("patchify");
  return UWU_OK;
}

extern "C" int uwu_unpatchify(const void* tok, int dtype, float* img, int B, int C, int H, int W, int p, void* stream) {
  UWU_CHECK_ARG(img && tok && B > 0 && C > 0 && p > 0 && H % p == 0 && W % p == 0, "unpatchify: bad shape");
  hipStream_t st = (hipStream_t)stream;
  const int64_t total = (int64_t)B * C * H * W;
#define UF(T, ...) hipLaunchKernelGGL((patch_kernel<T, false>), dim3(ew_grid(total, 256)), dim3(256), 0, st, img, (T*)const_cast<void*>(tok), B, C, H, W, p)
  DISPATCH_T(dtype, UF, 0)
#undef UF
  UWU_LAUNCH_CHECK("unpatchify");
  return UWU_OK;
}

extern "C" int uwu_add_pos(void* x, const float* pos, int B, int T, int D, int dtype, void* stream) {
  UWU_CHECK_ARG(x && pos && B > 0 && T > 0 && D > 0 && D % 4 == 0, "add_pos: bad args");
  hipStream_t st = (hipStream_t)stream;
  const int64_t td4 = (int64_t)T * D / 4, total4 = td4 * B;
#define AP(T_, ...) hipLaunchKernelGGL((add_pos_kernel<T_>), dim3(ew_grid(total4, 256)), dim3(256), 0, st, (T_*)x, pos, total4, td4)
  DISPATCH_T(dtype, AP, 0)
#undef AP
  UWU_LAUNCH_CHECK("add_pos");
  return UWU_OK;
}

extern "C" int uwu_add(const void* a, const void* b, void* out, int64_t n, int dtype, void* stream) {
  UWU_CHECK_ARG(a && b && out && n > 0 && n % 4 == 0, "add: n must be a positive multiple of 4");
  hipStream_t st = (hipStream_t)stream;
#define AD(T, ...) hipLaunchKernelGGL((add_kernel<T>), dim3(ew_grid(n / 4, 256)), dim3(256), 0, st, (const T*)a, (const T*)b, (T*)out, n / 4)
  DISPATCH_T(dtype, AD, 0)
#undef AD
  UWU_LAUNCH_CHECK("add");
  return UWU_OK;
}

namespace {
__global__ void __launch_bounds__(256) transpose_bf16_kernel(const bf16_t* __restrict__ src, bf16_t* __restrict__ dst, int rows,
                                                             int cols, int lds, int ldd) {
  __shared__ bf16_t tile[32][34];
  const int tx = threadIdx.x & 31, ty = threadIdx.x >> 5;
  const int r0 = blockIdx.y * 32, c0 = blockIdx.x * 32;
#pragma unroll
  for (int k = 0; k < 4; ++k) {
    const int r = r0 + ty + 8 * k, c = c0 + tx;
    tile[ty + 8 * k][tx] = (r < rows && c < cols) ? src[(int64_t)r * lds + c] : (bf16_t)0.f;
  }
  __syncthreads();
#pragma unroll
  for (int k = 0; k < 4; ++k) {
    const int c = c0 + ty + 8 * k, r = r0 + tx;
    if (c < cols && r < rows) dst[(int64_t)c * ldd + r] = tile[tx][ty + 8 * k];
  }
}
}

extern "C" int uwu_transpose_bf16(const void* src, void* dst, int rows, int cols, int ld_src, int ld_dst, void* stream) {
  UWU_CHECK_ARG(src && dst && rows > 0 && cols > 0 && ld_src >= cols && ld_dst >= rows, "transpose_bf16: bad argument");
  hipLaunchKernelGGL(transpose_bf16_kernel, dim3((cols + 31) / 32, (rows + 31) / 32), dim3(256), 0, (hipStream_t)stream,
                     (const bf16_t*)src, (bf16_t*)dst, rows, cols, ld_src, ld_dst);
  UWU_LAUNCH_CHECK("transpose_bf16");
  return UWU_OK;
}
```

uwudiff_amd/csrc/gemm.hip:

```cpp
#include "gemm_shared.h"

namespace {

template <typename T, typename TC, bool TA, bool TB, bool ACC, bool GL = false, int EPI = -1>
__global__ void __launch_bounds__(256, 2) gemm_kernel(const GemmArgs g) {
  extern __shared__ __attribute__((aligned(16))) char smem[];
  constexpr int BK = GT<T>::BK;
  const int tid = threadIdx.x, lane = tid & 63, wave = tid >> 6;
  const int wm = wave >> 1, wn = wave & 1;

  const int nblk = g.tiles_m * g.tiles_n;
  int tile;
  {
    const int bid = blockIdx.x, xcd = bid & 7, loc = bid >> 3;
    const int q = nblk >> 3, rm = nblk & 7;
    tile = (xcd < rm ? xcd * (q + 1) : rm * (q + 1) + (xcd - rm) * q) + loc;
  }
  const int tm = tile / g.tiles_n, tn = tile - tm * g.tiles_n;
  const int m0 = tm * BM, n0 = tn * BN;

  const int ktiles = (g.K + BK - 1) / BK;
  const int kt_begin = blockIdx.z * g.k_tiles_per_split;
  int kt_end = kt_begin + g.k_tiles_per_split;
  if (kt_end > ktiles) kt_end = ktiles;
  if (kt_begin >= kt_end) return;

  const T* A = static_cast<const T*>(g.A);
  const T* B = static_cast<const T*>(g.B);

  Stager<T, TA> sa;
  Stager<T, TB> sb;
  EpiPre<T, 4, 4> pre;
  if constexpr (!ACC && EPI >= 0) epi_prefetch<T, 4, 4, EPI>(pre, g, m0 + wm * 64, n0 + wn * 64, lane & 15, lane >> 4);
  f32x4 acc[4][4];
#pragma unroll
  for (int i = 0; i < 4; ++i)
#pragma unroll
    for (int j = 0; j < 4; ++j) acc[i][j] = f32x4{0.f, 0.f, 0.f, 0.f};

  if constexpr (GL) {
    glds_tile<T>(A, g.lda, m0, kt_begin * BK, g.M, smem, tid);
    glds_tile<T>(B, g.ldb, n0, kt_begin * BK, g.N, smem + TILE_BYTES, tid);
  } else {
    sa.load(A, g.lda, m0, kt_begin * BK, g.M, g.K, tid);
    sb.load(B, g.ldb, n0, kt_begin * BK, g.N, g.K, tid);
    sa.store(smem, tid);
    sb.store(smem + TILE_BYTES, tid);
  }
  __syncthreads();

  const int fr = lane & 15, fq = lane >> 4;
  for (int kt = kt_begin; kt < kt_end; ++kt) {
    const int cur = (kt - kt_begin) & 1;
    const char* la = smem + cur * 2 * TILE_BYTES;
    const char* lb = la + TILE_BYTES;
    const bool more = (kt + 1 < kt_end);
    if (more) {
      if constexpr (GL) {
        char* na = smem + (cur ^ 1) * 2 * TILE_BYTES;
        glds_tile<T>(A, g.lda, m0, (kt + 1) * BK, g.M, na, tid);
        glds_tile<T>(B, g.ldb, n0, (kt + 1) * BK, g.N, na + TILE_BYTES, tid);
      } else {
        sa.load(A, g.lda, m0, (kt + 1) * BK, g.M, g.K, tid);
        sb.load(B, g.ldb, n0, (kt + 1) * BK, g.N, g.K, tid);
      }
    }
    if constexpr (GL) {
      uint4 af[2][4], bf[2][4];
#pragma unroll
      for (int kk = 0; kk < 2; ++kk) {
#pragma unroll
        for (int i = 0; i < 4; ++i) af[kk][i] = lds_read128_asm(la + swz(wm * 64 + 16 * i + fr, 4 * kk + fq));
#pragma unroll
        for (int j = 0; j < 4; ++j) bf[kk][j] = lds_read128_asm(lb + swz(wn * 64 + 16 * j + fr, 4 * kk + fq));
        if (kk == 0) asm volatile("s_waitcnt lgkmcnt(0)" ::: "memory");
      }
      __builtin_amdgcn_sched_barrier(0);
#pragma unroll
      for (int i = 0; i < 4; ++i)
#pragma unroll
        for (int j = 0; j < 4; ++j) mma_frag<T>(bf[0][j], af[0][i], acc[i][j]);
      asm volatile("s_waitcnt lgkmcnt(0)" ::: "memory");
      __builtin_amdgcn_sched_barrier(0);
#pragma unroll
      for (int i = 0; i < 4; ++i)
#pragma unroll
        for (int j = 0; j < 4; ++j) mma_frag<T>(bf[1][j], af[1][i], acc[i][j]);
      asm volatile("s_waitcnt vmcnt(0)" ::: "memory");
      __builtin_amdgcn_s_barrier();
      continue;
    }
#pragma unroll
    for (int kk = 0; kk < 2; ++kk) {
      uint4 af[4], bf[4];
#pragma unroll
      for (int i = 0; i < 4; ++i)
        af[i] = *reinterpret_cast<const uint4*>(la + swz(wm * 64 + 16 * i + fr, 4 * kk + fq));
#pragma unroll
      for (int j = 0; j < 4; ++j)
        bf[j] = *reinterpret_cast<const uint4*>(lb + swz(wn * 64 + 16 * j + fr, 4 * kk + fq));
#pragma unroll
      for (int i = 0; i < 4; ++i)
#pragma unroll
        for (int j = 0; j < 4; ++j) {
          if constexpr (ACC)
            mma_frag<T>(af[i], bf[j], acc[i][j]);
          else
            mma_frag<T>(bf[j], af[i], acc[i][j]);
        }
    }
    if constexpr (!GL) {
      if (more) {
        char* na = smem + (cur ^ 1) * 2 * TILE_BYTES;
        sa.store(na, tid);
        sb.store(na + TILE_BYTES, tid);
      }
    }
    __syncthreads();
  }

  if constexpr (ACC) {
    float* C = static_cast<float*>(g.C);
    const bool alone = gridDim.z == 1;
#pragma unroll
    for (int i = 0; i < 4; ++i)
#pragma unroll
      for (int j = 0; j < 4; ++j) {
        const int n = n0 + wn * 64 + 16 * j + fr;
#pragma unroll
        for (int r = 0; r < 4; ++r) {
          const int m = m0 + wm * 64 + 16 * i + 4 * fq + r;
          if (m < g.M && n < g.N) {
            float* c = C + (int64_t)m * g.ldc + n;
            if (alone) *c += acc[i][j][r];
            else atomicAdd(c, acc[i][j][r]);
          }
        }
      }
  } else {
    if constexpr (EPI < 0) epi_prefetch<T, 4, 4, EPI>(pre, g, m0 + wm * 64, n0 + wn * 64, fr, fq);
    epilogue_tile<T, TC, 4, 4, EPI>(acc, pre, g, m0 + wm * 64, n0 + wn * 64, fr, fq, reinterpret_cast<float*>(smem), wm, wn);
  }
}


template <typename TC, int EPI, bool TB, int FI, int CONV = 0>
__global__ void __launch_bounds__(256, 2) gemm_r3_kernel(const GemmArgs g) {
  extern __shared__ __attribute__((aligned(16))) char smem[];
  typedef bf16_t T;
  static_assert(FI == 8 || FI == 4, "256x128 or 128x128");
  constexpr int RBM = 32 * FI, RBN = 128;
  constexpr int A_BYTES = RBM * R_ROWB, STAGE = A_BYTES + R_BSUB;
  constexpr int NST = FI == 8 ? 3 : 4;
  constexpr int QA = FI / 2, PS = QA + 2;
  const int tid = threadIdx.x, lane = tid & 63, wave = tid >> 6;
  const int wm = wave >> 1, wn = wave & 1;
  const int fr = lane & 15, fq = lane >> 4;
  const int nblk = g.tiles_m * g.tiles_n;
  int tile;
  {
    const int bid = blockIdx.x, xcd = bid & 7, loc = bid >> 3;
    const int q = nblk >> 3, rm = nblk & 7;
    tile = (xcd < rm ? xcd * (q + 1) : rm * (q + 1) + (xcd - rm) * q) + loc;
  }
  const int tm = tile / g.tiles_n, tn = tile - tm * g.tiles_n;
  const int m0 = tm * RBM, n0 = tn * RBN;
  const int nk = g.K >> 5;

  const int prow = lane >> 2;
  const int csrc = ((lane & 3) ^ r_gsw(prow)) & 3;
  const T* pa[QA];
  const T* pb[2];
  int cy[QA], cx[QA];
  const T* const zsrc = static_cast<const T*>(g.zero) + 8 * 0;
#pragma unroll
  for (int q = 0; q < QA; ++q) {
    int row = m0 + 16 * (wave + 4 * q) + prow;
    if constexpr (CONV == 0) {
      if (row >= g.M) row = g.M - 1;
      pa[q] = static_cast<const T*>(g.A) + (int64_t)row * g.lda + 8 * csrc;
    } else {
      const int RH = CONV != 2 ? g.cHo : g.cH, RW = CONV != 2 ? g.cWo : g.cW;
      const int GH = CONV != 2 ? g.cH : g.cHo, GW = CONV != 2 ? g.cW : g.cWo;
      int b, rem, y, x;
      divmod24(row < g.M ? row : 0, RH * RW, 1.f / (float)(RH * RW), b, rem);
      divmod24(rem, RW, 1.f / (float)RW, y, x);
      if (row >= g.M) y = -100000;
      cy[q] = y;
      cx[q] = x;
      pa[q] = static_cast<const T*>(g.A) + (int64_t)b * GH * GW * g.lda + 8 * csrc;
    }
  }
#pragma unroll
  for (int q = 0; q < 2; ++q) {
    if constexpr (!TB) {
      int row = n0 + 16 * (wave + 4 * q) + prow;
      if (row >= g.N) row = g.N - 1;
      pb[q] = static_cast<const T*>(g.B) + (int64_t)row * g.ldb + 8 * csrc;
    } else {
      const int drow = lane >> 4;
      const int dchunk = (lane & 15) ^ (((drow & 3) << 2) | (wave & 3));
      int x = n0 + 8 * dchunk;
      if (x > g.N - 8) x = g.N - 8;
      pb[q] = static_cast<const T*>(g.B) + (int64_t)(4 * (wave + 4 * q) + drow) * g.ldb + x;
    }
  }
  const int64_t bstep = TB ? (int64_t)32 * g.ldb : 32;
  auto issue = [&](int s) {
    char* st = smem + (s % NST) * STAGE + wave * 1024;
    int64_t boff = s * bstep;
    if constexpr (CONV != 0) {
      const int ch = s / 9, tap = s - 9 * ch, ky = tap / 3, kx = tap - 3 * ky;
      boff = TB ? (int64_t)32 * ch * g.ldb + tap * g.cC : (int64_t)tap * g.cC + 32 * ch;
#pragma unroll
      for (int q = 0; q < QA; ++q) {
        int gy, gx;
        bool ok;
        if constexpr (CONV == 1) {
          gy = cy[q] * g.cS + ky - 1;
          gx = cx[q] * g.cS + kx - 1;
          ok = gy >= 0 && gy < g.cH && gx >= 0 && gx < g.cW;
        } else if constexpr (CONV == 3) {
          gy = cy[q] * 2 + ky;
          gx = cx[q] * 2 + kx;
          ok = gy >= 0 && gy < g.cH && gx < g.cW;
        } else {
          const int ty = cy[q] + 1 - ky, tx = cx[q] + 1 - kx;
          ok = ty >= 0 && tx >= 0;
          if (g.cS == 2) {
            ok = ok && !((ty | tx) & 1);
            gy = ty >> 1;
            gx = tx >> 1;
          } else {
            gy = ty;
            gx = tx;
          }
          ok = ok && gy < g.cHo && gx < g.cWo;
        }
        const int GW = CONV != 2 ? g.cW : g.cWo;
        const T* src = ok ? pa[q] + (int64_t)(gy * GW + gx) * g.lda + 32 * ch : zsrc;
        __builtin_amdgcn_global_load_lds((const __attribute__((address_space(1))) void*)src,
                                         (__attribute__((address_space(3))) void*)(st + q * 4096), 16, 0, 0);
      }
    } else {
#pragma unroll
      for (int q = 0; q < QA; ++q)
        __builtin_amdgcn_global_load_lds((const __attribute__((address_space(1))) void*)(pa[q] + s * 32),
                                         (__attribute__((address_space(3))) void*)(st + q * 4096), 16, 0, 0);
    }
#pragma unroll
    for (int q = 0; q < 2; ++q)
      __builtin_amdgcn_global_load_lds((const __attribute__((address_space(1))) void*)(pb[q] + boff),
                                       (__attribute__((address_space(3))) void*)(st + A_BYTES + q * 4096), 16, 0, 0);
  };

  f32x4 acc[FI][4];
#pragma unroll
  for (int i = 0; i < FI; ++i)
#pragma unroll
    for (int j = 0; j < 4; ++j) acc[i][j] = f32x4{0.f, 0.f, 0.f, 0.f};
  EpiPre<T, FI, 4> pre;
  if constexpr (EPI >= 0) epi_prefetch<T, FI, 4, EPI>(pre, g, m0 + wm * 16 * FI, n0 + wn * 64, fr, fq);

  const unsigned smem_base = (unsigned)(size_t)((const __attribute__((address_space(3))) char*)smem);
  const unsigned a_off = (unsigned)r_swz(wm * 16 * FI + fr, fq);
  const unsigned b_off = (unsigned)(A_BYTES + r_swz(wn * 64 + fr, fq));
  const unsigned b_t0 = A_BYTES + tr_lane_base(lane, 0, 8 * wn), b_t1 = A_BYTES + tr_lane_base(lane, 1, 8 * wn);

  issue(0);
  if (nk > 1) issue(1);
  if (NST > 3 && nk > 2) issue(2);
  for (int s = 0; s < nk; ++s) {
    const int ahead = nk - 1 - s < NST - 2 ? nk - 1 - s : NST - 2;
    if (ahead >= 2) r_wait_vm<2 * PS>();
    else if (ahead == 1) r_wait_vm<PS>();
    else r_wait_vm<0>();
    __builtin_amdgcn_s_barrier();
    if (s + NST - 1 < nk) issue(s + NST - 1);
    const unsigned sb0 = smem_base + (unsigned)((s % NST) * STAGE);
    uint4 bf[4], af[FI];
    if constexpr (!TB) {
      bf[0] = r_read128<0>(sb0 + b_off);
      bf[1] = r_read128<1024>(sb0 + b_off);
      bf[2] = r_read128<2048>(sb0 + b_off);
      bf[3] = r_read128<3072>(sb0 + b_off);
    } else {
#pragma unroll
      for (int j = 0; j < 4; ++j) {
        const uint2 lo = t_read_tr<0>(sb0 + (b_t0 ^ (unsigned)(j << 5)));
        const uint2 hi = t_read_tr<0>(sb0 + (b_t1 ^ (unsigned)(j << 5)));
        bf[j] = uint4{lo.x, lo.y, hi.x, hi.y};
      }
    }
    const unsigned sa = sb0 + a_off;
    af[0] = r_read128<0>(sa);
    af[1] = r_read128<1024>(sa);
    af[2] = r_read128<2048>(sa);
    af[3] = r_read128<3072>(sa);
    asm volatile("s_waitcnt lgkmcnt(0)" ::: "memory");
    if constexpr (FI == 8) {
      af[4] = r_read128<4096>(sa);
      af[5] = r_read128<5120>(sa);
      af[6] = r_read128<6144>(sa);
      af[7] = r_read128<7168>(sa);
    }
    __builtin_amdgcn_sched_barrier(0);
#pragma unroll
    for (int i = 0; i < 4; ++i)
#pragma unroll
      for (int j = 0; j < 4; ++j) mma_frag<T>(bf[j], af[i], acc[i][j]);
    if constexpr (FI == 8) {
      asm volatile("s_waitcnt lgkmcnt(0)" ::: "memory");
      __builtin_amdgcn_sched_barrier(0);
#pragma unroll
      for (int i = 4; i < 8; ++i)
#pragma unroll
        for (int j = 0; j < 4; ++j) mma_frag<T>(bf[j], af[i], acc[i][j]);
    }
  }
  if constexpr (EPI < 0) epi_prefetch<T, FI, 4, EPI>(pre, g, m0 + wm * 16 * FI, n0 + wn * 64, fr, fq);
  epilogue_tile<T, TC, FI, 4, EPI>(acc, pre, g, m0 + wm * 16 * FI, n0 + wn * 64, fr, fq, reinterpret_cast<float*>(smem),
                                   wm, wn);
}

template <typename TC, int EPI, bool TB>
__global__ void __launch_bounds__(512, 2) gemm_big_kernel(const GemmArgs g) {
  extern __shared__ __attribute__((aligned(16))) char smem[];
  typedef bf16_t T;
  constexpr int STAGE = 4 * TILE_BYTES;
  const int tid = threadIdx.x, lane = tid & 63, wave = tid >> 6;
  const int wm = wave >> 2, wn = wave & 3;
  const int fr = lane & 15, fq = lane >> 4;
  const int nblk = g.tiles_m * g.tiles_n;
  int tile;
  {
    const int bid = blockIdx.x, xcd = bid & 7, loc = bid >> 3;
    const int q = nblk >> 3, rm = nblk & 7;
    tile = (xcd < rm ? xcd * (q + 1) : rm * (q + 1) + (xcd - rm) * q) + loc;
  }
  const int tm = tile / g.tiles_n, tn = tile - tm * g.tiles_n;
  const int m0 = tm * 256, n0 = tn * 256;
  const int nk = g.K >> 6;
  const T* A = static_cast<const T*>(g.A);
  const T* B = static_cast<const T*>(g.B);
  const int half = tid >> 8, t256 = tid & 255;
  const T* pbt[2] = {nullptr, nullptr};
  if constexpr (TB) {
    const int drow = lane >> 4;
    const int dchunk = (lane & 15) ^ (((drow & 3) << 2) | (wave & 3));
#pragma unroll
    for (int nh = 0; nh < 2; ++nh) {
      int x = n0 + 128 * nh + 8 * dchunk;
      if (x > g.N - 8) x = g.N - 8;
      pbt[nh] = B + (int64_t)(4 * wave + drow) * g.ldb + x;
    }
  }
  auto issue = [&](int s) {
    char* st = smem + (s & 1) * STAGE;
    glds_tile<T>(A, g.lda, m0 + 128 * half, s * 64, g.M, st + half * TILE_BYTES, t256);
    if constexpr (!TB) {
      glds_tile<T>(B, g.ldb, n0 + 128 * half, s * 64, g.N, st + (2 + half) * TILE_BYTES, t256);
    } else {
#pragma unroll
      for (int kh = 0; kh < 2; ++kh)
#pragma unroll
        for (int nh = 0; nh < 2; ++nh)
          __builtin_amdgcn_global_load_lds(
              (const __attribute__((address_space(1))) void*)(pbt[nh] + (int64_t)(64 * s + 32 * kh) * g.ldb),
              (__attribute__((address_space(3))) void*)(st + 2 * TILE_BYTES + (2 * kh + nh) * R_BSUB + wave * 1024), 16,
              0, 0);
    }
  };
  const unsigned smem_base = (unsigned)(size_t)((const __attribute__((address_space(3))) char*)smem);
  const unsigned b_t0 = tr_lane_base(lane, 0, 8 * (wn & 1)), b_t1 = tr_lane_base(lane, 1, 8 * (wn & 1));
  f32x4 acc[8][4];
#pragma unroll
  for (int i = 0; i < 8; ++i)
#pragma unroll
    for (int j = 0; j < 4; ++j) acc[i][j] = f32x4{0.f, 0.f, 0.f, 0.f};

  issue(0);
  for (int s = 0; s < nk; ++s) {
    asm volatile("s_waitcnt vmcnt(0)" ::: "memory");
    __builtin_amdgcn_s_barrier();
    if (s + 1 < nk) issue(s + 1);
    const char* la = smem + (s & 1) * STAGE + wm * TILE_BYTES;
    const char* lb = smem + (s & 1) * STAGE + (2 + (wn >> 1)) * TILE_BYTES;
#pragma unroll
    for (int kk = 0; kk < 2; ++kk) {
      uint4 bf[4], af[8];
      if constexpr (!TB) {
#pragma unroll
        for (int j = 0; j < 4; ++j) bf[j] = lds_read128_asm(lb + swz((wn & 1) * 64 + 16 * j + fr, 4 * kk + fq));
      } else {
        const unsigned sub = smem_base + (unsigned)((s & 1) * STAGE + 2 * TILE_BYTES + (2 * kk + (wn >> 1)) * R_BSUB);
#pragma unroll
        for (int j = 0; j < 4; ++j) {
          const uint2 lo = t_read_tr<0>(sub + (b_t0 ^ (unsigned)(j << 5)));
          const uint2 hi = t_read_tr<0>(sub + (b_t1 ^ (unsigned)(j << 5)));
          bf[j] = uint4{lo.x, lo.y, hi.x, hi.y};
        }
      }
#pragma unroll
      for (int i = 0; i < 4; ++i) af[i] = lds_read128_asm(la + swz(16 * i + fr, 4 * kk + fq));
      asm volatile("s_waitcnt lgkmcnt(0)" ::: "memory");
#pragma unroll
      for (int i = 4; i < 8; ++i) af[i] = lds_read128_asm(la + swz(16 * i + fr, 4 * kk + fq));
      __builtin_amdgcn_sched_barrier(0);
#pragma unroll
      for (int i = 0; i < 4; ++i)
#pragma unroll
        for (int j = 0; j < 4; ++j) mma_frag<T>(bf[j], af[i], acc[i][j]);
      asm volatile("s_waitcnt lgkmcnt(0)" ::: "memory");
      __builtin_amdgcn_sched_barrier(0);
#pragma unroll
      for (int i = 4; i < 8; ++i)
#pragma unroll
        for (int j = 0; j < 4; ++j) mma_frag<T>(bf[j], af[i], acc[i][j]);
    }
  }
  EpiPre<T, 8, 4> pre;
  epi_prefetch<T, 8, 4, EPI>(pre, g, m0 + wm * 128, n0 + wn * 64, fr, fq);
  epilogue_tile<T, TC, 8, 4, EPI>(acc, pre, g, m0 + wm * 128, n0 + wn * 64, fr, fq,
                                  reinterpret_cast<float*>(smem) + (wn >> 1) * 256, wm, wn & 1, wm == 0 ? (tid & 127) : 128);
}

template <typename TC, int EPI, bool TB>
__global__ void __launch_bounds__(512, 2) gemm_wide_kernel(const GemmArgs g) {
  extern __shared__ __attribute__((aligned(16))) char smem[];
  typedef bf16_t T;
  constexpr int FI = 6, FJ = 6, BMR = 192, BNC = 384;
  constexpr int A_BYTES = BMR * ROW_BYTES, STAGE = (BMR + BNC) * ROW_BYTES;
  const int tid = threadIdx.x, lane = tid & 63, wave = tid >> 6;
  const int wm = wave >> 2, wn = wave & 3;
  const int fr = lane & 15, fq = lane >> 4;
  const int nblk = g.tiles_m * g.tiles_n;
  int tile;
  {
    const int bid = blockIdx.x, xcd = bid & 7, loc = bid >> 3;
    const int q = nblk >> 3, rm = nblk & 7;
    tile = (xcd < rm ? xcd * (q + 1) : rm * (q + 1) + (xcd - rm) * q) + loc;
  }
  const int tm = tile / g.tiles_n, tn = tile - tm * g.tiles_n;
  const int m0 = tm * BMR, n0 = tn * BNC;
  const int nk = g.K >> 6;
  const T* A = static_cast<const T*>(g.A);
  const T* B = static_cast<const T*>(g.B);

  const T* pa[3];
  const T* pb[6];
#pragma unroll
  for (int q = 0; q < 3; ++q) {
    const int row = 8 * (wave + 8 * q) + (lane >> 3);
    const int c = ((lane & 7) ^ (row >> 1) ^ (row >> 4)) & 7;
    int grow = m0 + row;
    if (grow >= g.M) grow = g.M - 1;
    pa[q] = A + (int64_t)grow * g.lda + 8 * c;
  }
#pragma unroll
  for (int q = 0; q < 6; ++q) {
    if constexpr (!TB) {
      const int row = 8 * (wave + 8 * q) + (lane >> 3);
      const int c = ((lane & 7) ^ (row >> 1) ^ (row >> 4)) & 7;
      int grow = n0 + row;
      if (grow >= g.N) grow = g.N - 1;
      pb[q] = B + (int64_t)grow * g.ldb + 8 * c;
    } else {
      const int kh = q / 3, nh = q - 3 * kh;
      const int drow = lane >> 4;
      const int dchunk = (lane & 15) ^ (((drow & 3) << 2) | (wave & 3));
      int x = n0 + 128 * nh + 8 * dchunk;
      if (x > g.N - 8) x = g.N - 8;
      pb[q] = B + (int64_t)(32 * kh + 4 * wave + drow) * g.ldb + x;
    }
  }
  const bool a_once = g.tiles_n == 1;
  auto issue = [&](int s) {
    char* st = smem + (s & 1) * STAGE;
    if (a_once) {
#pragma unroll
      for (int q = 0; q < 3; ++q)
        __builtin_amdgcn_global_load_lds((const __attribute__((address_space(1))) void*)(pa[q] + 64 * s),
                                         (__attribute__((address_space(3))) void*)(st + (wave + 8 * q) * 1024), 16, 0, 2);
    } else {
#pragma unroll
      for (int q = 0; q < 3; ++q)
        __builtin_amdgcn_global_load_lds((const __attribute__((address_space(1))) void*)(pa[q] + 64 * s),
                                         (__attribute__((address_space(3))) void*)(st + (wave + 8 * q) * 1024), 16, 0, 0);
    }
#pragma unroll
    for (int q = 0; q < 6; ++q) {
      if constexpr (!TB)
        __builtin_amdgcn_global_load_lds((const __attribute__((address_space(1))) void*)(pb[q] + 64 * s),
                                         (__attribute__((address_space(3))) void*)(st + A_BYTES + (wave + 8 * q) * 1024),
                                         16, 0, 0);
      else
        __builtin_amdgcn_global_load_lds((const __attribute__((address_space(1))) void*)(pb[q] + (int64_t)(64 * s) * g.ldb),
                                         (__attribute__((address_space(3))) void*)(st + A_BYTES + q * R_BSUB + wave * 1024),
                                         16, 0, 0);
    }
  };
  const unsigned smem_base = (unsigned)(size_t)((const __attribute__((address_space(3))) char*)smem);
  unsigned tb0[FJ], tb1[FJ];
  if constexpr (TB) {
#pragma unroll
    for (int j = 0; j < FJ; ++j) {
      const int col = 96 * wn + 16 * j;
      tb0[j] = A_BYTES + (col >> 7) * R_BSUB + tr_lane_base(lane, 0, (col & 127) >> 3);
      tb1[j] = A_BYTES + (col >> 7) * R_BSUB + tr_lane_base(lane, 1, (col & 127) >> 3);
    }
  }
  f32x4 acc[FI][FJ];
#pragma unroll
  for (int i = 0; i < FI; ++i)
#pragma unroll
    for (int j = 0; j < FJ; ++j) acc[i][j] = f32x4{0.f, 0.f, 0.f, 0.f};

  issue(0);
  for (int s = 0; s < nk; ++s) {
    asm volatile("s_waitcnt vmcnt(0)" ::: "memory");
    __builtin_amdgcn_s_barrier();
    if (s + 1 < nk) issue(s + 1);
    const char* la = smem + (s & 1) * STAGE;
    const char* lb = la + A_BYTES;
#pragma unroll
    for (int kk = 0; kk < 2; ++kk) {
      uint4 bf[FJ], af[FI];
      if constexpr (!TB) {
#pragma unroll
        for (int j = 0; j < FJ; ++j) bf[j] = lds_read128_asm(lb + swz(96 * wn + 16 * j + fr, 4 * kk + fq));
      } else {
        const unsigned sb = smem_base + (unsigned)((s & 1) * STAGE + kk * 3 * R_BSUB);
#pragma unroll
        for (int j = 0; j < FJ; ++j) {
          const uint2 lo = t_read_tr<0>(sb + tb0[j]);
          const uint2 hi = t_read_tr<0>(sb + tb1[j]);
          bf[j] = uint4{lo.x, lo.y, hi.x, hi.y};
        }
      }
#pragma unroll
      for (int i = 0; i < 3; ++i) af[i] = lds_read128_asm(la + swz(96 * wm + 16 * i + fr, 4 * kk + fq));
      asm volatile("s_waitcnt lgkmcnt(0)" ::: "memory");
#pragma unroll
      for (int i = 3; i < FI; ++i) af[i] = lds_read128_asm(la + swz(96 * wm + 16 * i + fr, 4 * kk + fq));
      __builtin_amdgcn_sched_barrier(0);
#pragma unroll
      for (int i = 0; i < 3; ++i)
#pragma unroll
        for (int j = 0; j < FJ; ++j) mma_frag<T>(bf[j], af[i], acc[i][j]);
      asm volatile("s_waitcnt lgkmcnt(0)" ::: "memory");
      __builtin_amdgcn_sched_barrier(0);
#pragma unroll
      for (int i = 3; i < FI; ++i)
#pragma unroll
        for (int j = 0; j < FJ; ++j) mma_frag<T>(bf[j], af[i], acc[i][j]);
    }
  }
  EpiPre<T, FI, FJ> pre;
  epi_prefetch<T, FI, FJ, EPI>(pre, g, m0 + wm * 96, n0 + wn * 96, fr, fq);
  epilogue_tile<T, TC, FI, FJ, EPI>(acc, pre, g, m0 + wm * 96, n0 + wn * 96, fr, fq, nullptr, wm, wn & 1);
}

constexpr int M64_NST = 3;
template <typename TC, int EPI, bool TB>
__global__ void __launch_bounds__(256, 2) gemm_m64_kernel(const GemmArgs g) {
  extern __shared__ __attribute__((aligned(16))) char smem[];
  typedef bf16_t T;
  constexpr int A_BYTES = 64 * ROW_BYTES, STAGE = A_BYTES + TILE_BYTES;
  const int tid = threadIdx.x, lane = tid & 63, wave = tid >> 6;
  const int wm = wave >> 1, wn = wave & 1;
  const int fr = lane & 15, fq = lane >> 4;
  const int nblk = g.tiles_m * g.tiles_n;
  int tile;
  {
    const int bid = blockIdx.x, xcd = bid & 7, loc = bid >> 3;
    const int q = nblk >> 3, rm = nblk & 7;
    tile = (xcd < rm ? xcd * (q + 1) : rm * (q + 1) + (xcd - rm) * q) + loc;
  }
  const int tm = tile / g.tiles_n, tn = tile - tm * g.tiles_n;
  const int m0 = tm * 64, n0 = tn * 128;
  const int nk = g.K >> 6;
  const T* A = static_cast<const T*>(g.A);
  const T* B = static_cast<const T*>(g.B);
  const T* pa[2];
  const T* pbt[2] = {nullptr, nullptr};
#pragma unroll
  for (int q = 0; q < 2; ++q) {
    const int row = 8 * (wave + 4 * q) + (lane >> 3);
    const int c = ((lane & 7) ^ (row >> 1) ^ (row >> 4)) & 7;
    int grow = m0 + row;
    if (grow >= g.M) grow = g.M - 1;
    pa[q] = A + (int64_t)grow * g.lda + 8 * c;
    if constexpr (TB) {
      const int drow = lane >> 4;
      const int dchunk = (lane & 15) ^ (((drow & 3) << 2) | (wave & 3));
      int x = n0 + 8 * dchunk;
      if (x > g.N - 8) x = g.N - 8;
      pbt[q] = B + (int64_t)(4 * (wave + 4 * q) + drow) * g.ldb + x;
    }
  }
  auto issue = [&](int s) {
    char* st = smem + (s % M64_NST) * STAGE;
#pragma unroll
    for (int q = 0; q < 2; ++q)
      __builtin_amdgcn_global_load_lds((const __attribute__((address_space(1))) void*)(pa[q] + 64 * s),
                                       (__attribute__((address_space(3))) void*)(st + (wave + 4 * q) * 1024), 16, 0, 0);
    if constexpr (!TB) {
      glds_tile<T>(B, g.ldb, n0, s * 64, g.N, st + A_BYTES, tid);
    } else {
#pragma unroll
      for (int kh = 0; kh < 2; ++kh)
#pragma unroll
        for (int q = 0; q < 2; ++q)
          __builtin_amdgcn_global_load_lds(
              (const __attribute__((address_space(1))) void*)(pbt[q] + (int64_t)(64 * s + 32 * kh) * g.ldb),
              (__attribute__((address_space(3))) void*)(st + A_BYTES + kh * R_BSUB + (wave + 4 * q) * 1024), 16, 0, 0);
    }
  };
  const unsigned smem_base = (unsigned)(size_t)((const __attribute__((address_space(3))) char*)smem);
  const unsigned b_t0 = A_BYTES + tr_lane_base(lane, 0, 8 * wn), b_t1 = A_BYTES + tr_lane_base(lane, 1, 8 * wn);
  f32x4 acc[2][4];
#pragma unroll
  for (int i = 0; i < 2; ++i)
#pragma unroll
    for (int j = 0; j < 4; ++j) acc[i][j] = f32x4{0.f, 0.f, 0.f, 0.f};
  EpiPre<T, 2, 4> pre;
  epi_prefetch<T, 2, 4, EPI>(pre, g, m0 + wm * 32, n0 + wn * 64, fr, fq);

  issue(0);
  if (nk > 1) issue(1);
  for (int s = 0; s < nk; ++s) {
    if (s + 1 < nk) r_wait_vm<6>(); else r_wait_vm<0>();
    __builtin_amdgcn_s_barrier();
    if (s + 2 < nk) issue(s + 2);
    const char* la = smem + (s % M64_NST) * STAGE;
    const char* lb = la + A_BYTES;
    uint4 af[2][2], bf[2][4];
#pragma unroll
    for (int kk = 0; kk < 2; ++kk) {
#pragma unroll
      for (int i = 0; i < 2; ++i) af[kk][i] = lds_read128_asm(la + swz(wm * 32 + 16 * i + fr, 4 * kk + fq));
      if constexpr (!TB) {
#pragma unroll
        for (int j = 0; j < 4; ++j) bf[kk][j] = lds_read128_asm(lb + swz(wn * 64 + 16 * j + fr, 4 * kk + fq));
      } else {
        const unsigned sb = smem_base + (unsigned)((s % M64_NST) * STAGE + kk * R_BSUB);
#pragma unroll
        for (int j = 0; j < 4; ++j) {
          const uint2 lo = t_read_tr<0>(sb + (b_t0 ^ (unsigned)(j << 5)));
          const uint2 hi = t_read_tr<0>(sb + (b_t1 ^ (unsigned)(j << 5)));
          bf[kk][j] = uint4{lo.x, lo.y, hi.x, hi.y};
        }
      }
    }
    asm volatile("s_waitcnt lgkmcnt(0)" ::: "memory");
    __builtin_amdgcn_sched_barrier(0);
#pragma unroll
    for (int kk = 0; kk < 2; ++kk)
#pragma unroll
      for (int i = 0; i < 2; ++i)
#pragma unroll
        for (int j = 0; j < 4; ++j) mma_frag<T>(bf[kk][j], af[kk][i], acc[i][j]);
  }
  epilogue_tile<T, TC, 2, 4, EPI>(acc, pre, g, m0 + wm * 32, n0 + wn * 64, fr, fq, reinterpret_cast<float*>(smem), wm, wn);
}

template <typename T, typename TC, bool TA, bool TB, bool ACC, bool GL = false, int EPI = -1>
int launch(const GemmArgs& g, int split, hipStream_t st) {
  const GemmProf prof = {gemm_tag(g, TB, ACC), sizeof(T) == 2 ? 0 : 1, 2.0 * g.M * g.N * g.K, gemm_bytes(g, sizeof(T), sizeof(TC))};
  return gemm_launch<gemm_kernel<T, TC, TA, TB, ACC, GL, EPI>>("gemm", 4 * TILE_BYTES, dim3(g.tiles_m * g.tiles_n, 1, split), 256, st,
                                                              prof, g);
}

template <typename TC, int EPI, bool TB, int FI, int CONV = 0>
int launch_r3(GemmArgs g, hipStream_t st) {
  constexpr int LDS = (FI == 8 ? 3 : 4) * (32 * FI * R_ROWB + R_BSUB);
  g.tiles_m = (g.M + 32 * FI - 1) / (32 * FI);
  g.tiles_n = (g.N + 127) / 128;
  GemmProf prof = gemm_prof(g, TB, sizeof(TC));
  if (CONV) prof = {UWU_PROF_CONV, 0, 2.0 * g.M * g.N * g.K, ((double)g.M * g.K / 9 + (double)g.N * g.K + (double)g.M * g.N) * 2};
  return gemm_launch<gemm_r3_kernel<TC, EPI, TB, FI, CONV>>(FI == 8 ? "gemm_r3_256" : "gemm_r3_128", LDS,
                                                           dim3(g.tiles_m * g.tiles_n), 256, st, prof, g);
}
template <typename TC, int EPI, bool TB>
int launch_big(GemmArgs g, hipStream_t st) {
  g.tiles_m = (g.M + 255) / 256;
  g.tiles_n = (g.N + 255) / 256;
  return gemm_launch<gemm_big_kernel<TC, EPI, TB>>("gemm_big", 2 * 4 * TILE_BYTES, dim3(g.tiles_m * g.tiles_n), 512, st,
                                                  gemm_prof(g, TB, sizeof(TC)), g);
}
template <typename TC, int EPI, bool TB>
int launch_wide(GemmArgs g, hipStream_t st) {
  g.tiles_m = (g.M + 191) / 192;
  g.tiles_n = g.N / 384;
  return gemm_launch<gemm_wide_kernel<TC, EPI, TB>>("gemm_wide", 2 * (192 + 384) * ROW_BYTES, dim3(g.tiles_m * g.tiles_n), 512, st,
                                                   gemm_prof(g, TB, sizeof(TC)), g);
}
template <typename TC, int EPI, bool TB>
int launch_m64(GemmArgs g, hipStream_t st) {
  g.tiles_m = (g.M + 63) / 64;
  g.tiles_n = (g.N + 127) / 128;
  return gemm_launch<gemm_m64_kernel<TC, EPI, TB>>("gemm_m64", M64_NST * (64 * ROW_BYTES + TILE_BYTES), dim3(g.tiles_m * g.tiles_n),
                                                  256, st, gemm_prof(g, TB, sizeof(TC)), g);
}

static int pick_r3(const GemmArgs& g, bool tb) {
  static UwuEnv on("UWU_GEMM_R3");
  if (on.get().is('0')) return 0;
  if (g.K % 32 || g.K < 96) return 0;
  if ((((uintptr_t)g.A | (uintptr_t)g.B) & 15) || g.lda % 8 || g.ldb % 8) return 0;
  if (tb && (g.N % 8 || g.N < 8)) return 0;
  const int64_t t8 = (int64_t)((g.M + 255) / 256) * ((g.N + 127) / 128);
  if (t8 >= (g.K >= 640 ? 256 : 512)) return 8;
  const int64_t t4 = (int64_t)((g.M + 127) / 128) * ((g.N + 127) / 128);
  return (tb && t4 >= 128) ? 4 : 0;
}

static bool use_big(const GemmArgs& g) {
  static UwuEnv on("UWU_GEMM_BIG");
  return !on.get().is('0') && g.K % 64 == 0 && g.N % 256 == 0;
}

static bool use_wide(const GemmArgs& g) {
  if (g.K % 64 || g.N % 384 || g.N % 256 == 0) return false;
  static UwuEnv on("UWU_GEMM_WIDE");
  if (on.get().is('0')) return false;
  if (on.is('1')) return true;
  const int64_t tiles = (int64_t)((g.M + 191) / 192) * (g.N / 384);
  const int64_t rounds = (tiles + 255) / 256;
  return tiles * 100 >= rounds * 256 * 85;
}
static bool use_m64(const GemmArgs& g, bool tb) {
  static UwuEnv on("UWU_GEMM_M64");
  if (on.get().is('0')) return false;
  if (g.K % 64 || (((uintptr_t)g.A | (uintptr_t)g.B) & 15) || g.lda % 8 || g.ldb % 8) return false;
  if (tb && (g.N % 8 || g.N < 8)) return false;
  const int64_t tiles = (int64_t)((g.M + 127) / 128) * ((g.N + 127) / 128);
  return tiles < 256 && g.M > 64;
}

template <typename T, typename TC>
int dispatch_trans(const GemmArgs& g, int ta, int tb, bool acc, int split, hipStream_t st) {
  if (acc) {
    if constexpr (sizeof(TC) == 4) {
      if constexpr (sizeof(T) == 2) {
        if (ta == 1 && tb == 1) {
          const int tr = split > 1 ? uwu_gemm_pick_tr(g) : 0;
          GemmArgs gt = g;
          gt.bias = nullptr;
          if (tr == 1) return uwu_launch_gemm_tr<8, 4>(gt, nullptr, 0, st);
          if (tr == 2) return uwu_launch_gemm_tr<4, 8>(gt, nullptr, 0, st);
        }
      }
      if (ta == 1 && tb == 1) return launch<T, float, true, true, true>(g, split, st);
      if (ta == 0 && tb == 0) return launch<T, float, false, false, true>(g, split, st);
      if (ta == 0 && tb == 1) return launch<T, float, false, true, true>(g, split, st);
    }
    uwu_set_error("gemm: ACCUM epilogue needs fp32 C and (transA,transB) in {(0,0),(0,1),(1,1)}");
    return UWU_EINVAL;
  }
  constexpr bool hot = sizeof(T) == 2 && sizeof(TC) == 2;
  if (ta == 0 && tb == 0) {
    if constexpr (hot) {
      if (uwu_gemm_p8_ok(g, false)) return uwu_launch_gemm_p8(g, false, st);
      if (g.N % 256 && uwu_gemm_p8n_ok(g, false)) return uwu_launch_gemm_p8n(g, false, st);
    }
    if constexpr (sizeof(T) == 2) {
      const int r3 = pick_r3(g, false);
      if (r3 == 8) {
        if constexpr (hot) {
          if (g.epi == UWU_EPI_BIAS && uwu_gemm_use_as_bias() && uwu_gemm_use_as(g, sizeof(TC))) return uwu_launch_gemm_as<TC, UWU_EPI_BIAS>(g, st);
          if (use_wide(g)) {
            if (g.epi == UWU_EPI_NONE) return launch_wide<TC, UWU_EPI_NONE, false>(g, st);
            if (g.epi == UWU_EPI_BIAS) return launch_wide<TC, UWU_EPI_BIAS, false>(g, st);
          }
          if (g.epi == UWU_EPI_BIAS_GELU && uwu_gemm_use_as(g, sizeof(TC))) return uwu_launch_gemm_as<TC, UWU_EPI_BIAS_GELU>(g, st);
          if (g.epi == UWU_EPI_DGELU && g.C2 == nullptr && g.aux && g.ldaux % 8 == 0 && ((uintptr_t)g.aux & 15) == 0 &&
              uwu_gemm_use_as(g, sizeof(TC)))
            return uwu_launch_gemm_as<TC, UWU_EPI_DGELU>(g, st);
          if (use_big(g)) {
            if (g.epi == UWU_EPI_BIAS_GELU) return launch_big<TC, UWU_EPI_BIAS_GELU, false>(g, st);
            if (g.epi == UWU_EPI_NONE) return launch_big<TC, UWU_EPI_NONE, false>(g, st);
            if (g.epi == UWU_EPI_BIAS) return launch_big<TC, UWU_EPI_BIAS, false>(g, st);
          }
          if (g.epi == UWU_EPI_NONE) return launch_r3<TC, UWU_EPI_NONE, false, 8>(g, st);
          if (g.epi == UWU_EPI_BIAS) return launch_r3<TC, UWU_EPI_BIAS, false, 8>(g, st);
          if (g.epi == UWU_EPI_BIAS_GELU) return launch_r3<TC, UWU_EPI_BIAS_GELU, false, 8>(g, st);
        }
        return launch_r3<TC, -1, false, 8>(g, st);
      }
    }
    if constexpr (hot) {
      if (use_m64(g, false)) {
        if (g.epi == UWU_EPI_NONE) return launch_m64<TC, UWU_EPI_NONE, false>(g, st);
        if (g.epi == UWU_EPI_BIAS) return launch_m64<TC, UWU_EPI_BIAS, false>(g, st);
        if (g.epi == UWU_EPI_BIAS_GELU) return launch_m64<TC, UWU_EPI_BIAS_GELU, false>(g, st);
      }
    }
    if (g.K % GT<T>::BK == 0) {
      if constexpr (hot) {
        if (g.epi == UWU_EPI_NONE) return launch<T, TC, false, false, false, true, UWU_EPI_NONE>(g, split, st);
        if (g.epi == UWU_EPI_BIAS) return launch<T, TC, false, false, false, true, UWU_EPI_BIAS>(g, split, st);
        if (g.epi == UWU_EPI_BIAS_GELU) return launch<T, TC, false, false, false, true, UWU_EPI_BIAS_GELU>(g, split, st);
      }
      return launch<T, TC, false, false, false, true>(g, split, st);
    }
    return launch<T, TC, false, false, false>(g, split, st);
  }
  if (ta == 0 && tb == 1) {
    if constexpr (hot) {
      if (uwu_gemm_p8_ok(g, true)) return uwu_launch_gemm_p8(g, true, st);
      if (g.N % 256 && uwu_gemm_p8n_ok(g, true)) return uwu_launch_gemm_p8n(g, true, st);
      const int r3 = pick_r3(g, true);
      if (r3 == 8 && use_wide(g) && g.epi == UWU_EPI_NONE) return launch_wide<TC, UWU_EPI_NONE, true>(g, st);
      if (r3 == 8 && use_big(g)) {
        if (g.epi == UWU_EPI_DGELU) return launch_big<TC, UWU_EPI_DGELU, true>(g, st);
        if (g.epi == UWU_EPI_NONE) return launch_big<TC, UWU_EPI_NONE, true>(g, st);
      }
      if (r3 == 8 && g.epi == UWU_EPI_NONE) return launch_r3<TC, UWU_EPI_NONE, true, 8>(g, st);
      if (r3 == 8 && g.epi == UWU_EPI_DGELU) return launch_r3<TC, UWU_EPI_DGELU, true, 8>(g, st);
      if (r3 != 8 && use_m64(g, true)) {
        if (g.epi == UWU_EPI_NONE) return launch_m64<TC, UWU_EPI_NONE, true>(g, st);
        if (g.epi == UWU_EPI_DGELU) return launch_m64<TC, UWU_EPI_DGELU, true>(g, st);
      }
      if (r3 == 4 && g.epi == UWU_EPI_NONE) return launch_r3<TC, UWU_EPI_NONE, true, 4>(g, st);
      if (r3 == 4 && g.epi == UWU_EPI_DGELU) return launch_r3<TC, UWU_EPI_DGELU, true, 4>(g, st);
      if (g.epi == UWU_EPI_NONE) return launch<T, TC, false, true, false, false, UWU_EPI_NONE>(g, split, st);
      if (g.epi == UWU_EPI_DGELU) return launch<T, TC, false, true, false, false, UWU_EPI_DGELU>(g, split, st);
    }
    return launch<T, TC, false, true, false>(g, split, st);
  }
  if (ta == 1 && tb == 1) return launch<T, TC, true, true, false>(g, split, st);
  uwu_set_error("gemm: (transA=1, transB=0) is not instantiated");
  return UWU_EINVAL;
}

}

__device__ uint4 g_conv_zero[4];

static const void* conv_zero_page() {
  static void* p = nullptr;
  if (!p && hipGetSymbolAddress(&p, HIP_SYMBOL(g_conv_zero)) != hipSuccess) p = nullptr;
  return p;
}

extern "C" int uwu_conv3x3_implicit_ok(int B, int H, int W, int C, int Cout, int stride, int dtype) {
  if (dtype != UWU_BF16 || C % 32 || Cout % 32 || C < 32 || Cout < 32 || (stride != 1 && stride != 2)) return 0;
  if (B <= 0 || H <= 0 || W <= 0) return 0;
  const int Ho = (H - 1) / stride + 1, Wo = (W - 1) / stride + 1;
  const int64_t Mi = (int64_t)B * H * W, Mo = (int64_t)B * Ho * Wo;
  if (Mi >= (1 << 24) || Mo >= (1 << 24) || Mo % 32 || 9 * (int64_t)C >= (1 << 24)) return 0;
  return 1;
}

int uwu_conv3x3_args(GemmArgs& g, int B, int H, int W, int C, int stride) {
  g.cH = H; g.cW = W; g.cC = C; g.cS = stride;
  g.cHo = (H - 1) / stride + 1;
  g.cWo = (W - 1) / stride + 1;
  g.zero = conv_zero_page();
  if (!g.zero) { uwu_set_error("conv3x3: zero page unavailable"); return UWU_ELAUNCH; }
  return UWU_OK;
}

extern "C" int uwu_conv3x3_fwd(const void* x, const void* w, const float* bias, void* y, int B, int H, int W, int C, int Cout,
                               int stride, int dtype, void* stream) {
  UWU_CHECK_ARG(x && w && y && B > 0 && H > 0 && W > 0, "conv3x3_fwd: bad argument");
  UWU_CHECK_ARG(uwu_conv3x3_implicit_ok(B, H, W, C, Cout, stride, dtype), "conv3x3_fwd: shape not covered by the implicit-GEMM kernel (C=%d Cout=%d)", C, Cout);
  UWU_CHECK_ARG((((uintptr_t)x | (uintptr_t)w | (uintptr_t)y) & 15) == 0 && (!bias || ((uintptr_t)bias & 15) == 0), "conv3x3_fwd: misaligned tensor");
  GemmArgs g{};
  RETURN_IF(uwu_conv3x3_args(g, B, H, W, C, stride));
  g.A = x; g.B = w; g.C = y; g.bias = bias;
  g.M = B * g.cHo * g.cWo; g.N = Cout; g.K = 9 * C; g.lda = C; g.ldb = 9 * C; g.ldc = Cout;
  g.epi = bias ? UWU_EPI_BIAS : UWU_EPI_NONE;
  g.wide = (Cout % 8 == 0) ? 1 : 0;
  hipStream_t st = (hipStream_t)stream;
  if (bias) return launch_r3<bf16_t, UWU_EPI_BIAS, false, 8, 1>(g, st);
  return launch_r3<bf16_t, UWU_EPI_NONE, false, 8, 1>(g, st);
}

extern "C" int uwu_conv3x3_dgrad(const void* dy, const void* w, void* dx, int B, int H, int W, int C, int Cout, int stride,
                                 int dtype, void* stream) {
  UWU_CHECK_ARG(dy && w && dx && B > 0 && H > 0 && W > 0, "conv3x3_dgrad: bad argument");
  UWU_CHECK_ARG(uwu_conv3x3_implicit_ok(B, H, W, C, Cout, stride, dtype), "conv3x3_dgrad: shape not covered by the implicit-GEMM kernel");
  UWU_CHECK_ARG((((uintptr_t)dy | (uintptr_t)w | (uintptr_t)dx) & 15) == 0, "conv3x3_dgrad: misaligned tensor");
  GemmArgs g{};
  RETURN_IF(uwu_conv3x3_args(g, B, H, W, C, stride));
  g.A = dy; g.B = w; g.C = dx;
  g.M = B * H * W; g.N = C; g.K = 9 * Cout; g.lda = Cout; g.ldb = 9 * C; g.ldc = C;
  g.epi = UWU_EPI_NONE;
  g.wide = (C % 8 == 0) ? 1 : 0;
  return launch_r3<bf16_t, UWU_EPI_NONE, true, 8, 2>(g, (hipStream_t)stream);
}

int uwu_im2col3x3_s2br(const void* x, void* col, int B, int H, int W, int C, int dtype, hipStream_t st);

static bool conv_s2br_implicit(int B, int H, int W, int C, int Cout, int dtype) {
  if (dtype != UWU_BF16 || C % 32 || Cout % 32 || C < 32 || Cout < 32) return false;
  const int Ho = (H - 2) / 2 + 1, Wo = (W - 2) / 2 + 1;
  const int64_t Mi = (int64_t)B * H * W, Mo = (int64_t)B * Ho * Wo;
  return Mi < (1 << 24) && Mo % 32 == 0 && 9 * (int64_t)C < (1 << 24);
}

static bool conv_s2br_shape_ok(int B, int H, int W, int C, int Cout, int dtype) {
  if (dtype != UWU_BF16 && dtype != UWU_F32) return false;
  const int epc = dtype == UWU_BF16 ? 8 : 4;
  if (B <= 0 || H < 2 || W < 2 || C <= 0 || Cout <= 0 || C % epc) return false;
  return (int64_t)B * H * W < ((int64_t)1 << 31) / 9 && (int64_t)B * H * W * C < ((int64_t)1 << 40);
}

extern "C" size_t uwu_conv3x3_s2br_ws_bytes(int B, int H, int W, int C, int Cout, int dtype) {
  if (!conv_s2br_shape_ok(B, H, W, C, Cout, dtype) || conv_s2br_implicit(B, H, W, C, Cout, dtype)) return 0;
  const int Ho = (H - 2) / 2 + 1, Wo = (W - 2) / 2 + 1;
  return (size_t)B * Ho * Wo * 9 * C * (dtype == UWU_BF16 ? 2 : 4);
}

extern "C" int uwu_conv3x3_s2br_fwd(const void* x, const void* w, const float* bias, void* y, int B, int H, int W, int C, int Cout,
                                    int dtype, void* ws, size_t ws_bytes, void* stream) {
  UWU_CHECK_ARG(x && w && y, "conv3x3_s2br_fwd: null pointer");
  UWU_CHECK_ARG(conv_s2br_shape_ok(B, H, W, C, Cout, dtype),
                "conv3x3_s2br_fwd: bad shape B=%d H=%d W=%d C=%d Cout=%d dtype=%d (H, W >= 2; C a multiple of 8 (bf16) / 4 (fp32))", B, H, W, C,
                Cout, dtype);
  UWU_CHECK_ARG((((uintptr_t)x | (uintptr_t)w | (uintptr_t)y) & 15) == 0 && (!bias || ((uintptr_t)bias & 15) == 0),
                "conv3x3_s2br_fwd: misaligned tensor");
  const int Ho = (H - 2) / 2 + 1, Wo = (W - 2) / 2 + 1;
  hipStream_t st = (hipStream_t)stream;
  if (conv_s2br_implicit(B, H, W, C, Cout, dtype)) {
    GemmArgs g{};
    RETURN_IF(uwu_conv3x3_args(g, B, H, W, C, 2));
    g.cHo = Ho; g.cWo = Wo;
    g.A = x; g.B = w; g.C = y; g.bias = bias;
    g.M = B * Ho * Wo; g.N = Cout; g.K = 9 * C; g.lda = C; g.ldb = 9 * C; g.ldc = Cout;
    g.epi = bias ? UWU_EPI_BIAS : UWU_EPI_NONE;
    g.wide = (Cout % 8 == 0) ? 1 : 0;
    if (bias) return launch_r3<bf16_t, UWU_EPI_BIAS, false, 8, 3>(g, st);
    return launch_r3<bf16_t, UWU_EPI_NONE, false, 8, 3>(g, st);
  }
  const size_t need = (size_t)B * Ho * Wo * 9 * C * (dtype == UWU_BF16 ? 2 : 4);
  UWU_CHECK_ARG(ws && ws_bytes >= need && ((uintptr_t)ws & 15) == 0,
                "conv3x3_s2br_fwd: this shape needs a 16-byte aligned workspace of %zu bytes (uwu_conv3x3_s2br_ws_bytes)", need);
  RETURN_IF(uwu_im2col3x3_s2br(x, ws, B, H, W, C, dtype, st));
  return uwu_gemm(ws, w, y, nullptr, bias, nullptr, B * Ho * Wo, Cout, 9 * C, 9 * C, 9 * C, Cout, 0, 0, 0, dtype, dtype,
                  bias ? UWU_EPI_BIAS : UWU_EPI_NONE, 1, stream);
}

extern "C" int uwu_gemm(const void* A, const void* B, void* C, void* C2, const float* bias, const void* aux, int M,
                        int N, int K, int lda, int ldb, int ldc, int ldaux, int transA, int transB, int dtype,
                        int c_dtype, int epilogue, int split_k, void* stream) {
  UWU_CHECK_ARG(A && B && C, "gemm: null operand");
  UWU_CHECK_ARG(M > 0 && N > 0 && K > 0, "gemm: bad shape M=%d N=%d K=%d", M, N, K);
  UWU_CHECK_ARG(dtype == UWU_F32 || dtype == UWU_BF16, "gemm: bad dtype %d", dtype);
  UWU_CHECK_ARG(c_dtype == UWU_F32 || c_dtype == dtype, "gemm: c_dtype must be fp32 or the operand dtype");
  const int epc = dtype == UWU_BF16 ? 8 : 4;
  const int bk = dtype == UWU_BF16 ? 64 : 32;
  UWU_CHECK_ARG((((uintptr_t)A | (uintptr_t)B) & 15) == 0, "gemm: A/B must be 16-byte aligned");
  UWU_CHECK_ARG(lda % epc == 0 && ldb % epc == 0, "gemm: lda/ldb must be multiples of %d", epc);
  UWU_CHECK_ARG(transA ? (M % epc == 0) : (K % epc == 0), "gemm: A contiguous extent must be a multiple of %d", epc);
  UWU_CHECK_ARG(transB ? (N % epc == 0) : (K % epc == 0), "gemm: B contiguous extent must be a multiple of %d", epc);
  UWU_CHECK_ARG(lda >= (transA ? M : K) && ldb >= (transB ? N : K), "gemm: leading dimension too small");
  UWU_CHECK_ARG(epilogue >= UWU_EPI_NONE && epilogue <= UWU_EPI_ACCUM, "gemm: bad epilogue %d", epilogue);
  const bool acc = epilogue == UWU_EPI_ACCUM;
  if (!acc) {
    UWU_CHECK_ARG(split_k <= 1, "gemm: split_k needs UWU_EPI_ACCUM");
    UWU_CHECK_ARG(N % 4 == 0 && ldc % 4 == 0 && ldc >= N, "gemm: N and ldc must be multiples of 4");
    const int cal = c_dtype == UWU_BF16 ? 7 : 15;
    UWU_CHECK_ARG(((uintptr_t)C & cal) == 0, "gemm: C misaligned");
    if (epilogue == UWU_EPI_BIAS || epilogue == UWU_EPI_BIAS_GELU || epilogue == UWU_EPI_BIAS_SILU)
      UWU_CHECK_ARG(bias && ((uintptr_t)bias & 15) == 0, "gemm: bias missing/misaligned");
    if (epilogue == UWU_EPI_BIAS_GELU || epilogue == UWU_EPI_BIAS_SILU)
      UWU_CHECK_ARG(C2 && ((uintptr_t)C2 & cal) == 0, "gemm: C2 missing/misaligned");
    if (epilogue == UWU_EPI_DGELU)
      UWU_CHECK_ARG(aux && ldaux % 4 == 0 && ldaux >= N && ((uintptr_t)aux & (dtype == UWU_BF16 ? 7 : 15)) == 0,
                    "gemm: aux missing/misaligned");
  } else {
    UWU_CHECK_ARG(c_dtype == UWU_F32 && ldc >= N, "gemm: ACCUM needs fp32 C");
  }
  GemmArgs g{};
  g.A = A; g.B = B; g.C = C; g.C2 = C2; g.bias = bias; g.aux = aux;
  g.M = M; g.N = N; g.K = K; g.lda = lda; g.ldb = ldb; g.ldc = ldc; g.ldaux = ldaux; g.epi = epilogue;
  g.tiles_m = (M + BM - 1) / BM;
  g.tiles_n = (N + BN - 1) / BN;
  g.wide = (!acc && c_dtype == UWU_BF16 && N % 8 == 0 && ldc % 8 == 0 && ((uintptr_t)C & 15) == 0 &&
            (C2 == nullptr || epilogue == UWU_EPI_DGELU || ((uintptr_t)C2 & 15) == 0)) ? 1 : 0;
  g.aux16 = (epilogue == UWU_EPI_DGELU && dtype == UWU_BF16 && N % 8 == 0 && ldaux % 8 == 0 && ((uintptr_t)aux & 15) == 0) ? 1 : 0;

  const int ktiles = (K + bk - 1) / bk;
  int split = split_k < 1 ? 1 : split_k;
  if (split > ktiles) split = ktiles;
  g.k_tiles_per_split = (ktiles + split - 1) / split;
  split = (ktiles + g.k_tiles_per_split - 1) / g.k_tiles_per_split;
  hipStream_t st = (hipStream_t)stream;
  if (dtype == UWU_BF16) {
    if (c_dtype == UWU_BF16) return dispatch_trans<bf16_t, bf16_t>(g, transA, transB, acc, split, st);
    return dispatch_trans<bf16_t, float>(g, transA, transB, acc, split, st);
  }
  return dispatch_trans<float, float>(g, transA, transB, acc, split, st);
}
```

uwudiff_amd/csrc/gemm_shared.h:

```cpp
#pragma once
#include <stdlib.h>

#include <atomic>
#include <type_traits>

#include "common.h"

#define RETURN_IF(...)             \
  do {                             \
    const int rc_ = (__VA_ARGS__); \
    if (rc_ != UWU_OK) return rc_; \
  } while (0)

extern std::atomic<const char*> g_uwu_gemm_last_kernel;

struct GemmArgs {
  const void* A;
  const void* B;
  void* C;
  void* C2;
  const float* bias;
  const void* aux;
  int M, N, K, lda, ldb, ldc, ldaux, epi, tiles_m, tiles_n, k_tiles_per_split, wide;
  int xs, nloc, part_m;
  int aux16;
  int cH, cW, cC, cHo, cWo, cS;
  const void* zero;
  void* q8;
  void* q8t;
  const float* q_scale;
  float* q_amax;
  int ldq, ldqt;
};

namespace {

constexpr int BM = 128, BN = 128;
constexpr int ROW_BYTES = 128;
constexpr int TILE_BYTES = 128 * ROW_BYTES;

template <typename T> struct GT;
template <> struct GT<bf16_t> { static constexpr int EPC = 8; static constexpr int BK = 64; };
template <> struct GT<float> { static constexpr int EPC = 4; static constexpr int BK = 32; };

__device__ __forceinline__ int swz(int row, int chunk) {
  return row * ROW_BYTES + (((chunk ^ (row >> 1) ^ (row >> 4)) & 7) << 4);
}

typedef unsigned gu32x4 __attribute__((ext_vector_type(4)));
__device__ __forceinline__ uint4 lds_read128_asm(const char* p) {
  gu32x4 v;
  const unsigned a = (unsigned)(size_t)((const __attribute__((address_space(3))) char*)p);
  asm volatile("ds_read_b128 %0, %1" : "=v"(v) : "v"(a) : "memory");
  return uint4{v[0], v[1], v[2], v[3]};
}

template <typename T, bool TRANS>
struct Stager {
  uint4 r[4];

  __device__ __forceinline__ void load(const T* __restrict__ base, int ld, int row0, int k0, int nrows, int K,
                                       int tid) {
    constexpr int EPC = GT<T>::EPC;
    if constexpr (!TRANS) {
      const int c = tid & 7, rr = tid >> 3;
      const int kk = k0 + c * EPC;
#pragma unroll
      for (int p = 0; p < 4; ++p) {
        const int grow = row0 + rr + 32 * p;
        if (grow < nrows && kk < K)
          r[p] = *reinterpret_cast<const uint4*>(base + (int64_t)grow * ld + kk);
        else
          r[p] = uint4{0, 0, 0, 0};
      }
    } else if constexpr (sizeof(T) == 2) {
      const int xg = tid & 15, kg = tid >> 4;
      const int x = row0 + 8 * xg;
#pragma unroll
      for (int kr = 0; kr < 4; ++kr) {
        const int k = k0 + 4 * kg + kr;
        if (k < K && x < nrows)
          r[kr] = *reinterpret_cast<const uint4*>(base + (int64_t)k * ld + x);
        else
          r[kr] = uint4{0, 0, 0, 0};
      }
    } else {
      const int xg = tid & 31, kg = tid >> 5;
      const int x = row0 + 4 * xg;
#pragma unroll
      for (int kr = 0; kr < 4; ++kr) {
        const int k = k0 + 4 * kg + kr;
        if (k < K && x < nrows)
          r[kr] = *reinterpret_cast<const uint4*>(base + (int64_t)k * ld + x);
        else
          r[kr] = uint4{0, 0, 0, 0};
      }
    }
  }

  __device__ __forceinline__ void store(char* __restrict__ lds, int tid) const {
    if constexpr (!TRANS) {
      const int c = tid & 7, rr = tid >> 3;
#pragma unroll
      for (int p = 0; p < 4; ++p) *reinterpret_cast<uint4*>(lds + swz(rr + 32 * p, c)) = r[p];
    } else if constexpr (sizeof(T) == 2) {
      const int xg = tid & 15, kg = tid >> 4;
      const unsigned* w0 = reinterpret_cast<const unsigned*>(&r[0]);
      const unsigned* w1 = reinterpret_cast<const unsigned*>(&r[1]);
      const unsigned* w2 = reinterpret_cast<const unsigned*>(&r[2]);
      const unsigned* w3 = reinterpret_cast<const unsigned*>(&r[3]);
#pragma unroll
      for (int xi = 0; xi < 8; ++xi) {
        const int row = 8 * xg + xi;
        const unsigned sel = (xi & 1) ? 0x07060302u : 0x05040100u;
        uint2 o;
        o.x = __builtin_amdgcn_perm(w1[xi >> 1], w0[xi >> 1], sel);
        o.y = __builtin_amdgcn_perm(w3[xi >> 1], w2[xi >> 1], sel);
        *reinterpret_cast<uint2*>(lds + swz(row, kg >> 1) + 8 * (kg & 1)) = o;
      }
    } else {
      const int xg = tid & 31, kg = tid >> 5;
      const unsigned* w0 = reinterpret_cast<const unsigned*>(&r[0]);
      const unsigned* w1 = reinterpret_cast<const unsigned*>(&r[1]);
      const unsigned* w2 = reinterpret_cast<const unsigned*>(&r[2]);
      const unsigned* w3 = reinterpret_cast<const unsigned*>(&r[3]);
#pragma unroll
      for (int xi = 0; xi < 4; ++xi) {
        const int row = 4 * xg + xi;
        *reinterpret_cast<uint4*>(lds + swz(row, kg)) = uint4{w0[xi], w1[xi], w2[xi], w3[xi]};
      }
    }
  }
};

template <typename T>
__device__ __forceinline__ void glds_tile(const T* __restrict__ base, int ld, int row0, int k0, int nrows,
                                          char* __restrict__ lds_tile, int tid) {
  constexpr int EPC = GT<T>::EPC;
  const int wave = tid >> 6, lane = tid & 63;
#pragma unroll
  for (int g = 0; g < 4; ++g) {
    const int grp = wave + 4 * g;
    const int row = 8 * grp + (lane >> 3);
    const int c = ((lane & 7) ^ (row >> 1) ^ (row >> 4)) & 7;
    int grow = row0 + row;
    if (grow >= nrows) grow = nrows - 1;
    const T* src = base + (int64_t)grow * ld + k0 + c * EPC;
    __builtin_amdgcn_global_load_lds((const __attribute__((address_space(1))) void*)src,
                                     (__attribute__((address_space(3))) void*)(lds_tile + grp * 1024), 16, 0, 0);
  }
}

template <typename T>
__device__ __forceinline__ void mma_frag(const uint4& a, const uint4& b, f32x4& c) {
  if constexpr (sizeof(T) == 2) {
    c = __builtin_amdgcn_mfma_f32_16x16x32_bf16(*reinterpret_cast<const bf16x8*>(&a),
                                                *reinterpret_cast<const bf16x8*>(&b), c, 0, 0, 0);
  } else {
    const float* af = reinterpret_cast<const float*>(&a);
    const float* bf = reinterpret_cast<const float*>(&b);
#pragma unroll
    for (int e = 0; e < 4; ++e) c = __builtin_amdgcn_mfma_f32_16x16x4f32(af[e], bf[e], c, 0, 0, 0);
  }
}



__device__ __forceinline__ void divmod24(int n, int d, float rcp, int& q, int& r) {
  q = (int)((float)n * rcp);
  r = n - q * d;
  if (r < 0) { r += d; --q; }
  if (r >= d) { r -= d; ++q; }
}

template <typename T, int FI, int FJ>
struct EpiPre {
  static constexpr int PD = FI < 4 ? FI : 4;
  typedef typename std::conditional<sizeof(T) == 2, uint2, f32x4>::type AuxRaw;
  f32x4 bias[FJ];
  AuxRaw aux[PD][FJ];
};
template <typename T, int FI, int FJ>
__device__ __forceinline__ void epi_load_aux_row(const GemmArgs& g, int m_w, int n_w, int fr, int fq, int i,
                                                 typename EpiPre<T, FI, FJ>::AuxRaw (&dst)[FJ]) {
  typedef typename EpiPre<T, FI, FJ>::AuxRaw AuxRaw;
  const T* aux = static_cast<const T*>(g.aux);
  const int m = m_w + 16 * i + fr;
  if constexpr (sizeof(T) == 2 && FJ % 2 == 0) {
    if (g.aux16) {
      const bool odd = fq & 1;
#pragma unroll
      for (int jp = 0; jp < FJ / 2; ++jp) {
        const int nb = n_w + 32 * jp;
        const int n = odd ? nb + 16 + 4 * (fq - 1) : nb + 4 * fq;
        uint4 v = {0u, 0u, 0u, 0u};
        if (m < g.M && n < g.N) v = *reinterpret_cast<const uint4*>(aux + (int64_t)m * g.ldaux + n);
        dst[2 * jp] = AuxRaw{v.x, v.y};
        dst[2 * jp + 1] = AuxRaw{v.z, v.w};
      }
      return;
    }
  }
#pragma unroll
  for (int j = 0; j < FJ; ++j) {
    const int n = n_w + 16 * j + 4 * fq;
    if (m < g.M && n < g.N) dst[j] = *reinterpret_cast<const AuxRaw*>(aux + (int64_t)m * g.ldaux + n);
    else dst[j] = AuxRaw{};
  }
}
template <typename T, int FI, int FJ, int EPI>
__device__ __forceinline__ void epi_prefetch(EpiPre<T, FI, FJ>& pre, const GemmArgs& g, int m_w, int n_w, int fr,
                                             int fq) {
  const int epi = EPI >= 0 ? EPI : g.epi;
  const bool has_bias = epi == UWU_EPI_BIAS || epi == UWU_EPI_BIAS_GELU || epi == UWU_EPI_BIAS_SILU;
#pragma unroll
  for (int j = 0; j < FJ; ++j) {
    const int n = n_w + 16 * j + 4 * fq;
    pre.bias[j] = (has_bias && n < g.N) ? load4(g.bias + n) : f32x4{0.f, 0.f, 0.f, 0.f};
  }
  if (epi == UWU_EPI_DGELU) {
#pragma unroll
    for (int i = 0; i < EpiPre<T, FI, FJ>::PD; ++i) epi_load_aux_row<T, FI, FJ>(g, m_w, n_w, fr, fq, i, pre.aux[i]);
  }
}

template <typename T, typename TC, int FI, int FJ, int EPI = -1>
__device__ __forceinline__ void epilogue_tile(f32x4 (&acc)[FI][FJ], EpiPre<T, FI, FJ>& pre, const GemmArgs& g, int m_w,
                                              int n_w, int fr, int fq, float* cs_lds, int wm, int wn, int cs_t = -1,
                                              f32x4* cs_out = nullptr) {
  TC* C = static_cast<TC*>(g.C);
  TC* C2 = static_cast<TC*>(g.C2);
  const int epi = EPI >= 0 ? EPI : g.epi;
  const bool has_bias = epi == UWU_EPI_BIAS || epi == UWU_EPI_BIAS_GELU || epi == UWU_EPI_BIAS_SILU;
  const bool two = epi == UWU_EPI_BIAS_GELU || epi == UWU_EPI_BIAS_SILU;
  const bool dgelu = epi == UWU_EPI_DGELU;
  constexpr int PD = EpiPre<T, FI, FJ>::PD;
  typedef typename EpiPre<T, FI, FJ>::AuxRaw AuxRaw;
  auto aux_f32 = [](const AuxRaw& r) {
    if constexpr (sizeof(T) == 2) {
      const bf16x4 b = *reinterpret_cast<const bf16x4*>(&r);
      return f32x4{(float)b[0], (float)b[1], (float)b[2], (float)b[3]};
    } else {
      return r;
    }
  };

  auto finish = [&](f32x4 v, const f32x4& b, const AuxRaw& a, f32x4& second) {
    if (has_bias) v = v + b;
    if (dgelu) {
      v = v * dgelu_tanh_f4(aux_f32(a));
    }
    if (epi == UWU_EPI_BIAS_GELU) {
      second = gelu_tanh_f4(v);
    } else if (epi == UWU_EPI_BIAS_SILU) {
#pragma unroll
      for (int e = 0; e < 4; ++e) second[e] = silu_f(v[e]);
    }
    return v;
  };
  float* colsum = dgelu ? reinterpret_cast<float*>(g.C2) : nullptr;
  f32x4 csum[FJ];
#pragma unroll
  for (int j = 0; j < FJ; ++j) csum[j] = f32x4{0.f, 0.f, 0.f, 0.f};
  auto add_cs = [&](f32x4& acc_, const f32x4& v) { acc_ = acc_ + v; };
  auto flush_cs = [&]() {
    if (!colsum) return;
    constexpr int BNT = 2 * 16 * FJ;
    __syncthreads();
#pragma unroll
    for (int j = 0; j < FJ; ++j) {
      f32x4 v = csum[j];
#pragma unroll
      for (int e = 0; e < 4; ++e) v[e] = row16_sum(v[e]);
      if (fr == 0) store4(cs_lds + wm * BNT + wn * 16 * FJ + 16 * j + 4 * fq, v);
    }
    __syncthreads();
    const int t = cs_t >= 0 ? cs_t : (int)threadIdx.x, n = n_w - wn * 16 * FJ + t;
    if (t < BNT && n < g.N) atomicAdd(colsum + n, cs_lds[t] + cs_lds[BNT + t]);
  };
  const bool wide = sizeof(TC) == 2 && g.wide;
  const bool odd = fq & 1;
  auto pack = [](const f32x4& v) {
    bf16x4 b = {(bf16_t)v[0], (bf16_t)v[1], (bf16_t)v[2], (bf16_t)v[3]};
    return *reinterpret_cast<uint2*>(&b);
  };
#pragma unroll
  for (int i = 0; i < FI; ++i) {
    const int m = m_w + 16 * i + fr;
    const bool mok = m < g.M;
    AuxRaw(&arow)[FJ] = pre.aux[i % PD];
    if constexpr (sizeof(T) == 2 && FJ % 2 == 0) {
      if (dgelu && g.aux16) {
#pragma unroll
        for (int jp = 0; jp < FJ / 2; ++jp) {
          typedef unsigned su32x2 __attribute__((ext_vector_type(2)));
          const su32x2 sx = __builtin_amdgcn_permlane16_swap(arow[2 * jp].x, arow[2 * jp + 1].x, false, false);
          const su32x2 sy = __builtin_amdgcn_permlane16_swap(arow[2 * jp].y, arow[2 * jp + 1].y, false, false);
          arow[2 * jp] = AuxRaw{sx[0], sy[0]};
          arow[2 * jp + 1] = AuxRaw{sx[1], sy[1]};
        }
      }
    }
    f32x4 v[FJ], sec[FJ];
#pragma unroll
    for (int j = 0; j < FJ; ++j) {
      const int n = n_w + 16 * j + 4 * fq;
      sec[j] = f32x4{0.f, 0.f, 0.f, 0.f};
      v[j] = (mok && n < g.N) ? finish(acc[i][j], pre.bias[j], arow[j], sec[j]) : acc[i][j];
      if (colsum && mok && n < g.N) add_cs(csum[j], v[j]);
    }
    if (dgelu && i + PD < FI) epi_load_aux_row<T, FI, FJ>(g, m_w, n_w, fr, fq, i + PD, arow);
    if (wide) {
      if constexpr (sizeof(TC) == 2) {
#pragma unroll
        for (int jp = 0; jp < FJ / 2; ++jp) {
          const int nb = n_w + 32 * jp;
          auto exchange_store = [&](TC* dst, const f32x4& x0, const f32x4& x1, bool stream_out = false) {
            const uint2 p0 = pack(x0), p1 = pack(x1);
            typedef unsigned su32x2 __attribute__((ext_vector_type(2)));
            const su32x2 sx = __builtin_amdgcn_permlane16_swap(p0.x, p1.x, false, false);
            const su32x2 sy = __builtin_amdgcn_permlane16_swap(p0.y, p1.y, false, false);
            const int n = odd ? nb + 16 + 4 * (fq - 1) : nb + 4 * fq;
            if (mok && n < g.N) {
              typedef unsigned su32x4 __attribute__((ext_vector_type(4)));
              const su32x4 o = su32x4{sx[0], sy[0], sx[1], sy[1]};
              su32x4* ptr = reinterpret_cast<su32x4*>(dst + (int64_t)m * g.ldc + n);
              if (stream_out) __builtin_nontemporal_store(o, ptr);
              else *ptr = o;
            }
          };
          exchange_store(C, v[2 * jp], v[2 * jp + 1], epi == UWU_EPI_BIAS_GELU);
          if (two) exchange_store(C2, sec[2 * jp], sec[2 * jp + 1], false);
        }
      }
    } else {
#pragma unroll
      for (int j = 0; j < FJ; ++j) {
        const int n = n_w + 16 * j + 4 * fq;
        if (!mok || n >= g.N) continue;
        store4(C + (int64_t)m * g.ldc + n, v[j]);
        if (two) store4(C2 + (int64_t)m * g.ldc + n, sec[j]);
      }
    }
  }
  if (cs_out) {
#pragma unroll
    for (int j = 0; j < FJ; ++j) cs_out[j] = cs_out[j] + csum[j];
  } else {
    flush_cs();
  }
}

constexpr int R_ROWB = 64;
constexpr int R_BSUB = 32 * 256;

__device__ __forceinline__ int r_gsw(int row) { return (0 - (row >> 2)) & 3; }
__device__ __forceinline__ int r_swz(int row, int chunk) { return row * R_ROWB + (((chunk ^ r_gsw(row)) & 3) << 4); }
template <int OFF>
__device__ __forceinline__ uint4 r_read128(unsigned addr) {
  gu32x4 v;
  asm volatile("ds_read_b128 %0, %1 offset:%2" : "=v"(v) : "v"(addr), "n"(OFF) : "memory");
  return uint4{v[0], v[1], v[2], v[3]};
}
template <int N>
__device__ __forceinline__ void r_wait_vm() {
  asm volatile("s_waitcnt vmcnt(%0)" ::"n"(N) : "memory");
}
__device__ __forceinline__ void glds16_asm(const void* gsrc, unsigned lds_dst ) {
  unsigned keep;
  asm volatile("s_mov_b32 %0, m0\n\ts_mov_b32 m0, %2\n\ts_nop 0\n\tglobal_load_lds_dwordx4 %1, off\n\ts_mov_b32 m0, %0"
               : "=&s"(keep)
               : "v"(gsrc), "s"(lds_dst)
               : "memory");
}
template <int H>
using IC = std::integral_constant<int, H>;
__device__ __forceinline__ int p8_swz(int row, int chunk) { return row * ROW_BYTES + (((chunk ^ (row >> 1)) & 7) << 4); }

template <int OFF>
__device__ __forceinline__ uint2 t_read_tr(unsigned addr) {
  typedef unsigned tu32x2 __attribute__((ext_vector_type(2)));
  tu32x2 v;
  asm volatile("ds_read_b64_tr_b16 %0, %1 offset:%2" : "=v"(v) : "v"(addr), "n"(OFF) : "memory");
  return uint2{v[0], v[1]};
}
__device__ __forceinline__ unsigned tr_lane_base(int lane, int t, int xb8) {
  const int tg = lane >> 4, tq = (lane >> 2) & 3, tp = lane & 3;
  const int krow = 8 * tg + 4 * t + tq;
  const int f = (tq << 2) | ((2 * tg + t) & 3);
  return (unsigned)(256 * krow + 16 * ((xb8 + (tp >> 1)) ^ f) + 8 * (tp & 1));
}

static int gemm_tag(const GemmArgs& g, bool tb, bool acc) {
  if (acc) return UWU_PROF_GEMM_WGRAD;
  if (g.epi == UWU_EPI_BIAS_GELU) return UWU_PROF_GEMM_FC1_GELU;
  if (g.epi == UWU_EPI_DGELU) return UWU_PROF_GEMM_FC2_DGELU;
  return tb ? UWU_PROF_GEMM_DGRAD : UWU_PROF_GEMM_FWD;
}
static double gemm_bytes(const GemmArgs& g, int es, int esc) {
  double b = ((double)g.M * g.K + (double)g.N * g.K) * es + (double)g.M * g.N * esc;
  if (g.epi == UWU_EPI_BIAS_GELU || g.epi == UWU_EPI_BIAS_SILU) b += (double)g.M * g.N * esc;
  if (g.epi == UWU_EPI_DGELU) b += (double)g.M * g.N * es;
  return b;
}

template <auto KERN>
int gemm_lds_optin(const char* name, int lds) {
  static unsigned char done[UWU_MAX_DEV];
  if (uwu_func_lds(reinterpret_cast<const void*>(KERN), lds, done)) return UWU_OK;
  uwu_set_error("%s: the device cannot give a workgroup %d bytes of LDS", name, lds);
  return UWU_ELAUNCH;
}
struct GemmProf {
  int tag, kind;
  double flops, bytes;
};
static GemmProf gemm_prof(const GemmArgs& g, bool tb, int esc) {
  return {gemm_tag(g, tb, false), 0, 2.0 * g.M * g.N * g.K, gemm_bytes(g, 2, esc)};
}
template <auto KERN, typename... Args>
int gemm_launch(const char* name, int lds, dim3 grid, int block, hipStream_t st, const GemmProf& p, const Args&... args) {
  RETURN_IF(gemm_lds_optin<KERN>(name, lds));
  g_uwu_gemm_last_kernel.store(name, std::memory_order_relaxed);
  UwuProfScope prof(st);
  hipLaunchKernelGGL(KERN, grid, dim3(block), lds, st, args...);
  prof.done(p.tag, p.kind, p.flops, p.bytes);
  UWU_LAUNCH_CHECK(name);
  return UWU_OK;
}

}

bool uwu_gemm_use_as(const GemmArgs& g, int out_bytes);
bool uwu_gemm_use_as_bias();
template <typename TC, int EPI> int uwu_launch_gemm_as(GemmArgs g, hipStream_t st);
int uwu_conv3x3_args(GemmArgs& g, int B, int H, int W, int C, int stride);
int uwu_gemm_pick_tr(const GemmArgs& g);
template <int FI, int FJ, bool CONVW = false> int uwu_launch_gemm_tr(GemmArgs g, void* scratch, size_t scratch_bytes, hipStream_t st);
void uwu_launch_splitk_reduce(const float* part, float* C, int M, int N, int ldc, int split, hipStream_t st);
int uwu_launch_gemm_p8(const GemmArgs& g, bool tb, hipStream_t st);
int uwu_p8_cus();
bool uwu_gemm_p8_ok(const GemmArgs& g, bool tb);
int uwu_launch_gemm_p8n(const GemmArgs& g, bool tb, hipStream_t st);
bool uwu_gemm_p8n_ok(const GemmArgs& g, bool tb);
bool uwu_gemm_p8f_ok(const GemmArgs& g);
int uwu_launch_gemm_p8f(GemmArgs g, int fmt_a, const float* sa, const float* sb, hipStream_t st);
int uwu_gemm_p8f_split(int tiles, int steps);
bool uwu_gemm_p8f_part_ok(const GemmArgs& g);
int uwu_launch_gemm_p8f_part(GemmArgs& g, int fmt_a, const float* sa, const float* sb, void* scratch, hipStream_t st);
```

uwudiff_amd/lib.py:

```python
import ctypes
import os
from ctypes import c_char_p, c_double, c_float, c_int, c_int32, c_int64, c_size_t, c_void_p

import torch

_HERE = os.path.dirname(os.path.abspath(__file__))
LIB_PATH = os.path.join(_HERE, "libuwu_hip.so")

F32, BF16, I64 = 0, 1, 2
PT = {"epsilon": 0, "v_prediction": 1, "sample": 2, "rectified_flow": 3}
LOSS_MSE, LOSS_L1, LOSS_HUBER, LOSS_SMOOTH_L1 = 0, 1, 2, 3
EPI_NONE, EPI_BIAS, EPI_BIAS_GELU, EPI_DGELU, EPI_BIAS_SILU, EPI_ACCUM = 0, 1, 2, 3, 4, 5
ACT = {"quick_gelu": 0, "gelu": 1}
GATE = {"gated-gelu": 0}
FILTER = {"bilinear": 0, "bicubic": 1, "lanczos": 2}


class UwuError(RuntimeError):
    pass


class DitDesc(ctypes.Structure):
    _fields_ = (
        [(n, c_int32) for n in ("B", "T", "D", "H", "L", "mlp_ratio", "in_ch", "out_ch", "patch", "img", "dtype",
                                "cond_dim", "freq_dim")]
        + [("ln_eps", c_float), ("mod_total", c_int32)]
        + [("w", c_void_p), ("w32", c_void_p), ("g32", c_void_p)]
        + [(n, c_int64) for n in ("off_patch_w", "off_patch_b", "off_t_w1", "off_t_b1", "off_t_w2", "off_t_b2",
                                  "off_y_w", "off_y_b", "off_mod_w", "off_mod_b", "off_final_w", "off_final_b",
                                  "off_layer0", "layer_stride")]
        + [("pos", c_void_p), ("ws", c_void_p), ("ws_bytes", c_size_t), ("layer_done", c_void_p)]
        + [("side_stream", c_void_p)]
        + [("rope", c_int32), ("off_rope_h", c_int64), ("off_rope_w", c_int64), ("pos_xy", c_void_p)]
        + [("fp8", c_int32), ("f8_scale", c_void_p), ("f8_amax", c_void_p), ("f8_fmt", c_void_p)]
        + [("checkpoint", c_int32)]
    )


P = c_void_p
_SIGS = {
    "uwu_last_error": (c_char_p, []),
    "uwu_version": (c_int, []),
    "uwu_env_refresh": (c_int, []),
    "uwu_memset_zero": (c_int, [P, ctypes.c_uint64, P]),
    "uwu_schedule_gather": (c_int, [P, P, P, P, c_int, c_int, c_int, c_float, c_int, P, P]),
    "uwu_rf_time_to_sigma": (c_int, [P, c_float, P, c_int, c_int, P, P, P]),
    "uwu_qsample": (c_int, [P, P, P, c_int, c_int64, P, P, P]),
    "uwu_philox_raw": (c_int, [P, c_int64, ctypes.c_uint64, ctypes.c_uint64, P]),
    "uwu_philox_normal": (c_int, [P, c_int64, ctypes.c_uint64, ctypes.c_uint64, P]),
    "uwu_draw_timesteps": (c_int, [P, c_int, c_int, ctypes.c_uint64, ctypes.c_uint64, P]),
    "uwu_draw_u01": (c_int, [P, c_int, ctypes.c_uint64, ctypes.c_uint64, P]),
    "uwu_qsample_draw": (c_int, [P, P, c_int, c_int64, c_int, c_float, c_float, P, P, P, ctypes.c_uint64, ctypes.c_uint64, P]),
    "uwu_posterior_draw": (c_int, [P, c_int, c_int, c_int, c_int64, P, P, P, ctypes.c_uint64, ctypes.c_uint64, P]),
    "uwu_qsample_norm": (c_int, [P, P, P, c_int, c_int64, c_float, c_float, P, P, P]),
    "uwu_ctx_place": (c_int, [P, c_int, P, P] + [c_int] * 7 + [P]),
    "uwu_loss_fwd_bwd": (c_int, [P, P, P, P, c_int, P, c_int, c_int, c_int, c_int, c_int64, P, P, P, P, P, P]),
    "uwu_loss_elem_fwd_bwd": (c_int, [P, P, P, P, c_int, P, c_int, c_int, c_int, c_int, c_float, c_int, c_int64, P, P, P, P, P, P]),
    "uwu_scale_inplace": (c_int, [P, c_int, c_int64, P, P]),
    "uwu_scale_into": (c_int, [P, P, c_int, c_int64, P, P]),
    "uwu_cast_i64_to_f32": (c_int, [P, P, c_int64, P]),
    "uwu_sampler_step": (c_int, [P, P, P, P, P, P, c_int64, c_float, c_float, c_float, c_float, c_float, P]),
    "uwu_aggregate_concat": (c_int, [P, P, P, c_int, c_int, c_int64, c_int, ctypes.c_uint64, P]),
    "uwu_aggregate_split": (c_int, [P, P, P, c_int, c_int, c_int64, P]),
    "uwu_aggregate_first": (c_int, [P, P, P, c_int, c_int64, P]),
    "uwu_sampler_combine": (c_int, [P, P, P, P, P, c_int64, c_float, c_float, c_float, c_float, P]),
    "uwu_scale_copy": (c_int, [P, P, c_int64, c_float, P]),
    "uwu_cfg_input": (c_int, [P, P, c_int, c_int64, c_float, P]),
    "uwu_sampler_combine_draw": (c_int, [P, P, P, P, c_int64, c_float, c_float, c_float, c_float, ctypes.c_uint64, ctypes.c_uint64, P]),
    "uwu_latent_finish_ws_bytes": (ctypes.c_size_t, [c_int, c_int64]),
    "uwu_latent_finish": (c_int, [P, P, c_int, c_int64, c_int, c_float, c_float, P, ctypes.c_size_t, P]),
    "uwu_image_u8": (c_int, [P, c_int, P, c_int, c_int, c_int, P]),
    "uwu_resample_ksize": (c_int, [c_int, c_int, c_int]),
    "uwu_resample_coeffs": (c_int, [c_int, c_int, c_int, c_int, c_int, P, P]),
    "uwu_image_resize_crop_ws_bytes": (ctypes.c_size_t, [c_int, P, c_int, c_int, c_int]),
    "uwu_image_resize_crop": (c_int, [P, c_int64, P, P, P, c_int64, P, P] + [c_int] * 6 + [P, ctypes.c_size_t, P]),
    "uwu_grad_sqnorm_clip": (c_int, [P, c_int64, c_float, c_float, P, P, P]),
    "uwu_adamw_step": (c_int, [P, P, P, P, P, c_int64, c_float, c_float, c_float, c_float, c_float, c_int, c_float,
                               P, c_int, P]),
    "uwu_lion_step": (c_int, [P, P, P, P, c_int64, c_double, c_double, c_double, c_double, c_float, P, c_int, P]),
    "uwu_adamw_fp16_step": (c_int, [P, P, P, P, P, c_int64, c_double, c_double, c_double, c_double, c_int, c_float, P,
                                    c_int, P]),
    "uwu_param_decay": (c_int, [P, P, c_int64, c_double, P]),
    "uwu_adamw8_step": (c_int, [P] * 9 + [c_int64] * 3 + [c_double] * 5 + [c_int, c_float, P, c_int, P]),
    "uwu_lion8_step": (c_int, [P] * 6 + [c_int64] * 3 + [c_double] * 4 + [c_float, P, c_int, P]),
    "uwu_prodigy_stats_blocks": (c_int, [c_int64]),
    "uwu_prodigy_stats": (c_int, [P] * 6 + [c_int64, P, P, c_int64, c_int64] + [c_double] * 5 + [c_int, c_double, c_int, c_int,
                                  c_float, P, c_int, P]),
    "uwu_prodigy_finalize": (c_int, [P, P, c_int64] + [c_double] * 7 + [c_int, P]),
    "uwu_prodigy_apply": (c_int, [P, P, P, P, c_int64, P, c_double, c_double, c_int, P]),
    "uwu_ema_update": (c_int, [P, P, c_int64, c_float, c_float, P]),
    "uwu_ema_swap": (c_int, [P, P, P, c_int64, c_int, P]),
    "uwu_sfadamw_step": (c_int, [P, P, P, P, P, c_int64] + [c_double] * 7 + [c_float, P, c_int, P]),
    "uwu_sf_average": (c_int, [P, P, P, c_int64, c_double, P]),
    "uwu_cast_f32_to_bf16": (c_int, [P, P, c_int64, P]),
    "uwu_cast_bf16_to_f32": (c_int, [P, P, c_int64, P]),
    "uwu_adapter_merge": (c_int, [P, P, P, P, c_int, c_int64, P, P, P]),
    "uwu_adapter_grad": (c_int, [P, c_int64, c_int64, c_int, P, P, c_int64, c_int64, c_int64, c_int, c_int, c_int, c_float,
                                 P, c_int64, P]),
    "uwu_adapter_dora_norms": (c_int, [P, P, P, P, P, c_int, c_int64, P, P]),
    "uwu_adapter_dora_merge": (c_int, [P, P, P, P, P, c_int, c_int64, P, P, P, P]),
    "uwu_adapter_dora_grad": (c_int, [P, P, c_int64, c_int64, c_int, P, P, c_int64, c_int64, c_int64, c_int, c_int, c_int,
                                      c_float, c_int64, P, c_int, P, c_int64, P]),
    "uwu_adapter_conv_merge": (c_int, [P, P, P, P, P, P, c_int, c_int64, c_int64, P, c_int64, P, P, P]),
    "uwu_adapter_conv_grad": (c_int, [P, c_int64, c_int64, c_int64, c_int64, c_int, P, P, c_int64, c_int64, c_int64, c_int,
                                      c_int, c_int, c_float, P, c_int64, P]),
    "uwu_comm_unique_id": (c_int, [P]),
    "uwu_comm_init": (c_int, [P, c_int, c_int, ctypes.POINTER(c_void_p)]),
    "uwu_allreduce_flat": (c_int, [P, P, c_int64, P]),
    "uwu_comm_destroy": (c_int, [P]),
    "uwu_gemm": (c_int, [P, P, P, P, P, P] + [c_int] * 13 + [P]),
    "uwu_gemm_last_kernel": (c_char_p, []),
    "uwu_gemm_fp8_scratch_bytes": (ctypes.c_size_t, [c_int, c_int, c_int]),
    "uwu_gemm_fp8": (c_int, [P, P, P, P, P, P] + [c_int] * 9 + [P, P, P, ctypes.c_size_t, P]),
    "uwu_fp8_amax": (c_int, [P, c_int, c_int64, P, P]),
    "uwu_fp8_update_scales": (c_int, [P, P, P, c_int, c_float, P]),
    "uwu_fp8_quantize": (c_int, [P, c_int, c_int, c_int, c_int, P, c_int, P, c_int, P, c_int, P, P, P]),
    "uwu_gemm_fp8_emit": (c_int, [P, P, P, P, P, P, c_int, c_int, c_int, c_int, c_int, c_int, c_int, c_int, c_int, P, P, P, c_int, P, c_int, P,
                                  P, P]),
    "uwu_gemm_wgrad_scratch_bytes": (ctypes.c_size_t, [c_int, c_int, c_int]),
    "uwu_gemm_wgrad": (c_int, [P, P, P, P] + [c_int] * 8 + [P, ctypes.c_size_t, P]),
    "uwu_gemm_wgrad_pair_scratch_bytes": (ctypes.c_size_t, [c_int] * 5),
    "uwu_gemm_wgrad_pair": (c_int, ([P, P, P, P] + [c_int] * 5) * 2 + [c_int] * 3 + [P, ctypes.c_size_t, P]),
    "uwu_gemm_prof_enable": (c_int, [c_int]),
    "uwu_gemm_prof_collect": (c_int, [c_int, P, P, P]),
    "uwu_prof_enable": (c_int, [c_int]),
    "uwu_prof_collect": (c_int, [c_int, c_int, P, P, P, P]),
    "uwu_colsum": (c_int, [P, c_int, c_int, c_int, c_int, P, c_int, P]),
    "uwu_colsum_batched": (c_int, [P, c_int, c_int, c_int, c_int, c_int, P, c_int, P]),
    "uwu_skinny_linear_ok": (c_int, [c_int, c_int, c_int]),
    "uwu_skinny_linear_fwd": (c_int, [P, P, P, P, P, c_int, c_int, c_int, c_int, P]),
    "uwu_skinny_linear_dgrad": (c_int, [P, P, P, c_int, c_int, c_int, P]),
    "uwu_skinny_linear_wgrad": (c_int, [P, P, P, P, c_int, c_int, c_int, P]),
    "uwu_add_ln_modulate_fwd": (c_int, [P, P, P, P, P, c_int, P, P, P, P, c_int, c_int, c_int, c_float, c_int, c_int, P]),
    "uwu_add_ln_modulate_fwd_q8": (c_int, [P, P, P, P, P, c_int, P, P, c_int, P, c_int, P, P, P, P, c_int, c_int, c_int, c_float, P]),
    "uwu_add_ln_modulate_bwd": (c_int, [P, P, P, P, P, P, P, P, c_int, P, P, P, P, P, c_int, c_int, c_int, c_int, c_int, P]),
    "uwu_attention_fwd": (c_int, [P, P, P, P, P] + [c_int] * 9 + [c_float, c_int, P]),
    "uwu_attention_d512_fwd": (c_int, [P, P, P, P] + [c_int] * 6 + [c_float, c_int, P]),
    "uwu_attention_causal_fwd": (c_int, [P] * 5 + [c_int] * 8 + [c_float, c_int, P]),
    "uwu_text_embed": (c_int, [P, P, P, P, c_int, c_int, c_int, c_int, c_int, P]),
    "uwu_bias_act_fwd": (c_int, [P, P, P, c_int, c_int, c_int, c_int, c_int, P]),
    "uwu_text_pool": (c_int, [P, P, P, c_int, c_int, c_int, c_int, c_int, P]),
    "uwu_attention_relbias_fwd": (c_int, [P] * 6 + [c_int] * 8 + [c_float, c_int, P]),
    "uwu_attention_bidir_fwd": (c_int, [P] * 5 + [c_int] * 8 + [c_float, c_int, P]),
    "uwu_clip_patches": (c_int, [P, c_int, P] + [c_int] * 5 + [P, P, c_int, P]),
    "uwu_vit_embed": (c_int, [P, P, P, P, c_int, c_int, c_int, c_int, P]),
    "uwu_clip_score_accum": (c_int, [P, P, P, P, c_int, c_int, c_int, P]),
    "uwu_timestep_stats_accum": (c_int, [P, P, c_int, P, c_int, c_int, P, P, P]),
    "uwu_conv2d_ok": (c_int, [c_int] * 15),
    "uwu_conv2d_ws_bytes": (ctypes.c_size_t, [c_int] * 15),
    "uwu_conv2d_fwd": (c_int, [P, P, P, P] + [c_int] * 16 + [P, ctypes.c_size_t, P]),
    "uwu_inception_stem": (c_int, [P, c_int, P, c_int, c_int, c_int, c_int, P]),
    "uwu_pool2d_fwd": (c_int, [P, P] + [c_int] * 10 + [P]),
    "uwu_relu_rows": (c_int, [P, c_int64, c_int, c_int, c_int, c_int, P]),
    "uwu_global_avgpool": (c_int, [P, P, c_int, c_int, c_int, c_int, c_int, P]),
    "uwu_fid_stats_accum": (c_int, [P, P, c_int, c_int, P]),
    "uwu_add_rmsnorm_fwd": (c_int, [P] * 5 + [c_int, c_int, c_float, c_int, P]),
    "uwu_gated_act_fwd": (c_int, [P, P] + [c_int] * 6 + [P]),
    "uwu_t5_rel_bias": (c_int, [P, P, P, c_int, c_int, c_int, P]),
    "uwu_token_embed": (c_int, [P, P, P, c_int, c_int, c_int, c_int, c_int, P]),
    "uwu_attention_bwd": (c_int, [P] * 10 + [c_int] * 9 + [c_float, c_int, P]),
    "uwu_attention_bias_fwd": (c_int, [P] * 6 + [c_int] * 9 + [c_float, c_int, P]),
    "uwu_attention_bias_bwd": (c_int, [P] * 11 + [c_int] * 9 + [c_float, c_int, P]),
    "uwu_attention_route": (c_int, [c_int] * 9),
    "uwu_axial_rope_fwd": (c_int, [P, P, P, P, P, c_int64, c_int, c_int, c_int, c_int, P]),
    "uwu_axial_rope_bwd": (c_int, [P, P, P, P, P, P, P, P, c_int64, c_int, c_int, c_int, c_int, P]),
    "uwu_axial_rope_bwd_shared": (c_int, [P, P, P, c_int, P, P, P, P, P, c_int64, c_int, c_int, c_int, c_int, P]),
    "uwu_axial_rope_table": (c_int, [P, P, P, P, c_int, c_int, c_int, c_int, P]),
    "uwu_attention_rope_fwd": (c_int, [P] * 6 + [c_int] * 9 + [c_float, c_int, P]),
    "uwu_attention_rope_bwd": (c_int, [P] * 10 + [c_int] * 9 + [c_float, c_int, P]),
    "uwu_timestep_embedding": (c_int, [P, c_int, c_int, c_float, P, c_int, P]),
    "uwu_silu_fwd": (c_int, [P, P, c_int64, c_int, P]),
    "uwu_silu_bwd": (c_int, [P, P, P, c_int64, c_int, P]),
    "uwu_add": (c_int, [P, P, P, c_int64, c_int, P]),
    "uwu_transpose_bf16": (c_int, [P, P, c_int, c_int, c_int, c_int, P]),
    "uwu_patchify": (c_int, [P, P, c_int, c_int, c_int, c_int, c_int, c_int, P]),
    "uwu_unpatchify": (c_int, [P, c_int, P, c_int, c_int, c_int, c_int, c_int, P]),
    "uwu_add_pos": (c_int, [P, P, c_int, c_int, c_int, c_int, P]),
    "uwu_groupnorm_fwd": (c_int, [P, P, P, P, P, P, c_int, c_int, c_int, c_int, c_float, c_int, c_int, P]),
    "uwu_groupnorm_fwd_det_ws_bytes": (ctypes.c_size_t, [c_int] * 4),
    "uwu_groupnorm_fwd_det": (c_int, [P, P, P, P, P, P, P, ctypes.c_size_t, c_int, c_int, c_int, c_int, c_float, c_int, c_int, P]),
    "uwu_groupnorm_bwd": (c_int, [P] * 10 + [c_int] * 6 + [P]),
    "uwu_im2col3x3": (c_int, [P, P] + [c_int] * 6 + [P]),
    "uwu_col2im3x3": (c_int, [P, P] + [c_int] * 6 + [P]),
    "uwu_conv3x3_implicit_ok": (c_int, [c_int] * 7),
    "uwu_conv3x3_fwd": (c_int, [P, P, P, P] + [c_int] * 7 + [P]),
    "uwu_conv3x3_s2br_ws_bytes": (ctypes.c_size_t, [c_int] * 6),
    "uwu_conv3x3_s2br_fwd": (c_int, [P, P, P, P] + [c_int] * 6 + [P, ctypes.c_size_t, P]),
    "uwu_conv3x3_dgrad": (c_int, [P, P, P] + [c_int] * 7 + [P]),
    "uwu_conv3x3_wgrad_scratch_bytes": (ctypes.c_size_t, [c_int, c_int, c_int64]),
    "uwu_conv3x3_wgrad": (c_int, [P, P, P, P] + [c_int] * 7 + [P, ctypes.c_size_t, P]),
    "uwu_geglu_fwd": (c_int, [P, P, c_int64, c_int, c_int, P]),
    "uwu_geglu_bwd": (c_int, [P, P, P, c_int64, c_int, c_int, P]),
    "uwu_upsample2x": (c_int, [P, P] + [c_int] * 6 + [P]),
    "uwu_add_rowvec": (c_int, [P, P, c_int, c_int, c_int, c_int, P]),
    "uwu_nchw_to_cl": (c_int, [P, P, c_int, c_int, c_int, c_int, P]),
    "uwu_cl_to_nchw": (c_int, [P, P, c_int, c_int, c_int, c_int, P]),
    "uwu_dit_workspace_bytes": (c_size_t, [ctypes.POINTER(DitDesc)]),
    "uwu_dit_forward": (c_int, [ctypes.POINTER(DitDesc), P, P, P, P, P]),
    "uwu_dit_backward": (c_int, [ctypes.POINTER(DitDesc), P, P]),
    "uwu_dit_backward_cond": (c_int, [ctypes.POINTER(DitDesc), P, P]),
    "uwu_dit_layer_param_stride": (c_int64, [c_int, c_int]),
}

_lib = None


def exported_symbols():
    return sorted(_SIGS)


def load():
    global _lib
    if _lib is not None:
        return _lib
    if not os.path.exists(LIB_PATH):
        raise UwuError(
            f"{LIB_PATH} not found: build it with `python -m uwudiff_amd.build` "
            "(the HIP extension is required; there is no fallback path)"
        )
    lib = ctypes.CDLL(LIB_PATH)
    for name, (res, args) in _SIGS.items():
        fn = getattr(lib, name)
        fn.restype = res
        fn.argtypes = args
    _lib = lib
    return lib


def check(rc, what=""):
    if rc != 0:
        msg = load().uwu_last_error().decode(errors="replace")
        raise UwuError(f"{what} failed (code {rc}): {msg}")


def dt(t: torch.Tensor) -> int:
    if t.dtype == torch.float32:
        return F32
    if t.dtype == torch.bfloat16:
        return BF16
    raise UwuError(f"unsupported dtype {t.dtype}")


def ptr(t):
    if t is None:
        return None
    if not t.is_cuda:
        raise UwuError("libuwu_hip kernels need device tensors (got a CPU tensor); there is no CPU path")
    if not t.is_contiguous():
        raise UwuError("libuwu_hip kernels need contiguous tensors")
    return t.data_ptr()


def stream():
    return torch.cuda.current_stream().cuda_stream


def call(name, *args):
    lib = load()
    rc = getattr(lib, name)(*args)
    check(rc, name)
```

Before: 17990 images/s.

## Fuse DiT edge ops: patch-embed bias+pos table epilogue, batched fc2 transpose, fused colsum

```diff
diff --git a/include/uwu_hip.h b/include/uwu_hip.h
--- a/include/uwu_hip.h
+++ b/include/uwu_hip.h
@@ -33,6 +33,7 @@
 #define UWU_EPI_DGELU 3
 #define UWU_EPI_BIAS_SILU 4
 #define UWU_EPI_ACCUM 5
+#define UWU_EPI_BIAS_TABLE 6
 
 const char* uwu_last_error(void);
 int uwu_version(void);
@@ -207,6 +208,8 @@
 int uwu_gemm(const void* A, const void* B, void* C, void* C2, const float* bias, const void* aux,
              int M, int N, int K, int lda, int ldb, int ldc, int ldaux, int transA, int transB, int dtype,
              int c_dtype, int epilogue, int split_k, void* stream);
+int uwu_gemm_bias_table(const void* A, const void* B, void* C, const float* bias, const float* table, int table_rows,
+                        int M, int N, int K, int lda, int ldb, int ldc, int dtype, int c_dtype, void* stream);
 const char* uwu_gemm_last_kernel(void);
 
 #define UWU_FP8_E4M3 0
@@ -368,6 +371,8 @@
 
 int uwu_add(const void* a, const void* b, void* out, int64_t n, int dtype, void* stream);
 int uwu_transpose_bf16(const void* src, void* dst, int rows, int cols, int ld_src, int ld_dst, void* stream);
+int uwu_transpose_bf16_batched(const void* src, void* dst, int batch, int rows, int cols, int ld_src, int ld_dst,
+                               int64_t stride_src, int64_t stride_dst, void* stream);
 
 int uwu_patchify(const float* img, void* tok, int B, int C, int H, int W, int p, int dtype, void* stream);
 int uwu_unpatchify(const void* tok, int dtype, float* img, int B, int C, int H, int W, int p, void* stream);
@@ -418,6 +423,7 @@
 } uwu_dit_desc;
 
 size_t uwu_dit_workspace_bytes(const uwu_dit_desc* d);
+int uwu_dit_workspace_region(const uwu_dit_desc* d, const char* name, int layer, size_t* offset, size_t* bytes);
 int uwu_dit_forward(const uwu_dit_desc* d, const float* noisy, const float* t, const float* cond,
                     float* out, void* stream);
 int uwu_dit_backward(const uwu_dit_desc* d, const float* dout, void* stream);
diff --git a/uwudiff_amd/csrc/dit.cpp b/uwudiff_amd/csrc/dit.cpp
--- a/uwudiff_amd/csrc/dit.cpp
+++ b/uwudiff_amd/csrc/dit.cpp
@@ -3,6 +3,7 @@
 #include <stddef.h>
 #include <stdint.h>
 #include <stdlib.h>
+#include <string.h>
 
 #include "../../include/uwu_hip.h"
 #include "env.h"
@@ -27,13 +28,22 @@
   size_t o_h1t, o_aot, o_h2t, o_ft;
   size_t xF, mF, rF, hF, otok;
   size_t dx, dy, dh, dqkv, dao, du, delta, dotok, dmod, dsc, dc, dth, dtp;
-  size_t w2t;
+  size_t w2t, w2t_stride;
   size_t wsc, wsc_bytes;
   size_t x8, x8t, dy8, dy8t, w8, w8_layer;
   size_t total;
 };
 
 inline size_t al(size_t x) { return (x + 255) & ~(size_t)255; }
+
+bool edge_fuse() {
+  static UwuEnv on("UWU_DIT_EDGE_FUSE");
+  return !on.get().is('0');
+}
+bool dgelu_as(const uwu_dit_desc& d) {
+  const int64_t M = (int64_t)d.B * d.T, D4 = (int64_t)d.mlp_ratio * d.D;
+  return !d.fp8 && d.dtype == UWU_BF16 && d.D == 384 && M % 256 == 0 && M >= 256 * 256 && D4 % 64 == 0 && D4 >= 1024 && D4 <= 2048;
+}
 
 Layout make_layout(const uwu_dit_desc& d) {
   Layout L{};
@@ -100,7 +110,8 @@
   L.dqkv = take(L.M * L.D3 * L.es);
   L.dao = take(L.M * L.D * L.es);
   L.du = take(L.M * L.D4 * L.es);
-  L.w2t = take((size_t)L.D4 * d.D * 2);
+  L.w2t_stride = al((size_t)L.D4 * d.D * 2);
+  L.w2t = take(L.w2t_stride * (dgelu_as(d) ? d.L : 1));
   L.delta = take((size_t)d.B * d.H * d.T * f4);
   L.dotok = take(L.M * L.Ko * L.es);
   L.dmod = take((size_t)d.B * d.mod_total * f4);
@@ -202,7 +213,8 @@
               size_t scratch_bytes = 0, float* db = nullptr) {
   if (dt == UWU_BF16 && scratch && uwu_gemm_wgrad_scratch_bytes(N, K, M) <= scratch_bytes)
     return uwu_gemm_wgrad(dY, X, dW, db, N, K, M, N, K, K, dt, WGRAD_BLOCKS, scratch, scratch_bytes, st);
-  if (db) {
+  const bool fused_db = db && edge_fuse();
+  if (db && !fused_db) {
     const int rc = uwu_colsum(dY, dt, M, N, N, db, 1, st);
     if (rc != UWU_OK) return rc;
   }
@@ -213,7 +225,7 @@
   int split = (target + tiles - 1) / tiles;
   if (split > ktiles) split = ktiles;
   if (split < 1) split = 1;
-  return uwu_gemm(dY, X, dW, nullptr, nullptr, nullptr, N, K, M, N, K, K, 0, 1, 1, dt, UWU_F32, UWU_EPI_ACCUM, split, st);
+  return uwu_gemm(dY, X, dW, nullptr, fused_db ? db : nullptr, nullptr, N, K, M, N, K, K, 0, 1, 1, dt, UWU_F32, UWU_EPI_ACCUM, split, st);
 }
 
 bool wgrad_pair_ok(int M, int Na, int Ka, int Nb, int Kb, size_t scratch_bytes) {
@@ -472,6 +484,37 @@
   return make_layout(*d).total;
 }
 
+extern "C" int uwu_dit_workspace_region(const uwu_dit_desc* dp, const char* name, int layer, size_t* offset, size_t* bytes) {
+  RUN(check_desc(dp));
+  if (!name || !offset || !bytes) { uwu_set_error("dit_workspace_region: null argument"); return UWU_EINVAL; }
+  const uwu_dit_desc& d = *dp;
+  const Layout L = make_layout(d);
+  const size_t md = L.M * L.D * L.es, md3 = L.M * L.D3 * L.es, md4 = L.M * L.D4 * L.es;
+  const struct { const char* n; size_t sub, sz; } per_layer[] = {
+      {"x0", L.o_x0, md}, {"h1", L.o_h1, md}, {"qkv", L.o_qkv, md3}, {"ao", L.o_ao, md}, {"y1", L.o_y1, md},
+      {"x1", L.o_x1, md}, {"h2", L.o_h2, md}, {"u", L.o_u, md4}, {"f", L.o_f, md4}, {"y2", L.o_y2, md}};
+  for (const auto& e : per_layer)
+    if (!strcmp(name, e.n)) {
+      if (layer < 0 || layer >= d.L) { uwu_set_error("dit_workspace_region: layer %d of %d", layer, d.L); return UWU_EINVAL; }
+      *offset = (L.ckpt && e.sub >= L.keep) ? L.scratch0 + e.sub : L.layer0 + (size_t)layer * L.layer_stride + e.sub;
+      *bytes = e.sz;
+      return UWU_OK;
+    }
+  const struct { const char* n; size_t off, sz; } flat[] = {
+      {"tok", L.tok, L.M * L.Kp * L.es}, {"xF", L.xF, md}, {"hF", L.hF, md}, {"otok", L.otok, L.M * L.Ko * L.es},
+      {"dx", L.dx, md}, {"dy", L.dy, md}, {"dh", L.dh, md}, {"dqkv", L.dqkv, md3}, {"dao", L.dao, md}, {"du", L.du, md4},
+      {"w2t", L.w2t, L.w2t_stride * (dgelu_as(d) ? d.L : 1)}, {"dotok", L.dotok, L.M * L.Ko * L.es},
+      {"dmod", L.dmod, (size_t)d.B * d.mod_total * 4}};
+  for (const auto& e : flat)
+    if (!strcmp(name, e.n)) {
+      *offset = e.off;
+      *bytes = e.sz;
+      return UWU_OK;
+    }
+  uwu_set_error("dit_workspace_region: unknown tensor '%s'", name);
+  return UWU_EINVAL;
+}
+
 extern "C" int64_t uwu_dit_layer_param_stride(int D, int mlp_ratio) {
   const int64_t d = D, d4 = (int64_t)mlp_ratio * D;
   return pad64(3 * d * d) + pad64(3 * d) + pad64(d * d) + pad64(d) + pad64(d4 * d) + pad64(d4) + pad64(d * d4) + pad64(d);
@@ -533,9 +576,14 @@
   }
 
   RUN(uwu_patchify(noisy, P.at(L.tok), B, d.in_ch, d.img, d.img, d.patch, dt, st));
-  RUN(lin_fwd(P.at(L.tok), wb + d.off_patch_w * es, w32 + d.off_patch_b, P.lay(0, L.o_x0), nullptr, M, D, (int)L.Kp, dt,
-              dt, UWU_EPI_BIAS, st));
-  RUN(uwu_add_pos(P.lay(0, L.o_x0), d.pos, B, T, D, dt, st));
+  if (edge_fuse()) {
+    RUN(uwu_gemm_bias_table(P.at(L.tok), wb + d.off_patch_w * es, P.lay(0, L.o_x0), w32 + d.off_patch_b, d.pos, T, M, D, (int)L.Kp,
+                            (int)L.Kp, (int)L.Kp, D, dt, dt, st));
+  } else {
+    RUN(lin_fwd(P.at(L.tok), wb + d.off_patch_w * es, w32 + d.off_patch_b, P.lay(0, L.o_x0), nullptr, M, D, (int)L.Kp, dt,
+                dt, UWU_EPI_BIAS, st));
+    RUN(uwu_add_pos(P.lay(0, L.o_x0), d.pos, B, T, D, dt, st));
+  }
 
   for (int l = 0; l < d.L; ++l) RUN(block_forward(d, L, P, f8, l, false, st));
   {
@@ -582,9 +630,12 @@
   const bool pair_fc = pairs && wgrad_pair_ok(M, D4, D, D, D4, L.wsc_bytes);
   const bool pair_attn = pairs && wgrad_pair_ok(M, D3, D, D, D, L.wsc_bytes);
 
+  const bool w2t_all = dgelu_as(d);
+  if (w2t_all && edge_fuse())
+    RUN(uwu_transpose_bf16_batched(layer_weights(d, 0).fc2_w, P.at(L.w2t), d.L, D, D4, D4, D, d.layer_stride, (int64_t)(L.w2t_stride / 2), st));
+
   RUN(uwu_patchify(dout, P.at(L.dotok), B, d.out_ch, d.img, d.img, d.patch, dt, st));
-  RUN(lin_wgrad(P.at(L.dotok), P.at(L.hF), g + d.off_final_w, M, (int)L.Ko, D, dt, st));
-  RUN(uwu_colsum(P.at(L.dotok), dt, M, (int)L.Ko, (int)L.Ko, g + d.off_final_b, 1, st));
+  RUN(lin_wgrad(P.at(L.dotok), P.at(L.hF), g + d.off_final_w, M, (int)L.Ko, D, dt, st, nullptr, 0, g + d.off_final_b));
   RUN(lin_dgrad(P.at(L.dotok), wb + d.off_final_w * es, P.at(L.dh), nullptr, M, (int)L.Ko, D, dt, st));
   {
     const int l = d.L - 1;
@@ -620,9 +671,10 @@
     side_used[0] = true;
     }
     if (side_used[1]) RUN(join_side(fk, 1));
-    if (dt == UWU_BF16 && D == 384 && M % 256 == 0 && M >= 256 * 256 && D4 % 64 == 0 && D4 >= 1024 && D4 <= 2048) {
-      RUN(uwu_transpose_bf16(w.fc2_w, P.at(L.w2t), D, D4, D4, D, st));
-      RUN(uwu_gemm(P.at(L.dy), P.at(L.w2t), P.at(L.du), nullptr, nullptr, P.lay(l, L.o_u), M, D4, D, D, D, D4, D4, 0, 0, dt, dt,
+    if (w2t_all) {
+      void* w2t = P.at<char>(L.w2t) + (size_t)l * L.w2t_stride;
+      if (!edge_fuse()) RUN(uwu_transpose_bf16(w.fc2_w, w2t, D, D4, D4, D, st));
+      RUN(uwu_gemm(P.at(L.dy), w2t, P.at(L.du), nullptr, nullptr, P.lay(l, L.o_u), M, D4, D, D, D, D4, D4, 0, 0, dt, dt,
                    UWU_EPI_DGELU, 1, st));
     } else {
       RUN(lin_dgrad(P.at(L.dy), w.fc2_w, P.at(L.du), P.lay(l, L.o_u), M, D, D4, dt, st, nullptr));
@@ -709,8 +761,7 @@
   }
   if (fk.on)
     for (int k = 0; k < 4; ++k) RUN(join_side(fk, k));
-  RUN(lin_wgrad(P.at(L.dx), P.at(L.tok), g + d.off_patch_w, M, D, (int)L.Kp, dt, st));
-  RUN(uwu_colsum(P.at(L.dx), dt, M, D, D, g + d.off_patch_b, 1, st));
+  RUN(lin_wgrad(P.at(L.dx), P.at(L.tok), g + d.off_patch_w, M, D, (int)L.Kp, dt, st, nullptr, 0, g + d.off_patch_b));
 
   if (mod_bf16(d)) {
     RUN(uwu_cast_f32_to_bf16(dmod, P.at(L.dmod16), (int64_t)B * ML, st));
diff --git a/uwudiff_amd/csrc/embed.hip b/uwudiff_amd/csrc/embed.hip
--- a/uwudiff_amd/csrc/embed.hip
+++ b/uwudiff_amd/csrc/embed.hip
@@ -157,8 +157,10 @@
 
 namespace {
 __global__ void __launch_bounds__(256) transpose_bf16_kernel(const bf16_t* __restrict__ src, bf16_t* __restrict__ dst, int rows,
-                                                             int cols, int lds, int ldd) {
+                                                             int cols, int lds, int ldd, int64_t ss, int64_t sd) {
   __shared__ bf16_t tile[32][34];
+  src += blockIdx.z * ss;
+  dst += blockIdx.z * sd;
   const int tx = threadIdx.x & 31, ty = threadIdx.x >> 5;
   const int r0 = blockIdx.y * 32, c0 = blockIdx.x * 32;
 #pragma unroll
@@ -178,7 +180,18 @@
 extern "C" int uwu_transpose_bf16(const void* src, void* dst, int rows, int cols, int ld_src, int ld_dst, void* stream) {
   UWU_CHECK_ARG(src && dst && rows > 0 && cols > 0 && ld_src >= cols && ld_dst >= rows, "transpose_bf16: bad argument");
   hipLaunchKernelGGL(transpose_bf16_kernel, dim3((cols + 31) / 32, (rows + 31) / 32), dim3(256), 0, (hipStream_t)stream,
-                     (const bf16_t*)src, (bf16_t*)dst, rows, cols, ld_src, ld_dst);
+                     (const bf16_t*)src, (bf16_t*)dst, rows, cols, ld_src, ld_dst, (int64_t)0, (int64_t)0);
   UWU_LAUNCH_CHECK("transpose_bf16");
   return UWU_OK;
 }
+
+extern "C" int uwu_transpose_bf16_batched(const void* src, void* dst, int batch, int rows, int cols, int ld_src, int ld_dst,
+                                          int64_t stride_src, int64_t stride_dst, void* stream) {
+  UWU_CHECK_ARG(src && dst && rows > 0 && cols > 0 && ld_src >= cols && ld_dst >= rows, "transpose_bf16_batched: bad argument");
+  UWU_CHECK_ARG(batch > 0 && batch <= 65535 && stride_src >= 0 && stride_dst >= (int64_t)(cols - 1) * ld_dst + rows,
+                "transpose_bf16_batched: batch must be 1 .. 65535 and the outputs must not overlap");
+  hipLaunchKernelGGL(transpose_bf16_kernel, dim3((cols + 31) / 32, (rows + 31) / 32, batch), dim3(256), 0, (hipStream_t)stream,
+                     (const bf16_t*)src, (bf16_t*)dst, rows, cols, ld_src, ld_dst, stride_src, stride_dst);
+  UWU_LAUNCH_CHECK("transpose_bf16_batched");
+  return UWU_OK;
+}
diff --git a/uwudiff_amd/csrc/gemm.hip b/uwudiff_amd/csrc/gemm.hip
--- a/uwudiff_amd/csrc/gemm.hip
+++ b/uwudiff_amd/csrc/gemm.hip
@@ -31,7 +31,8 @@
   Stager<T, TA> sa;
   Stager<T, TB> sb;
   EpiPre<T, 4, 4> pre;
-  if constexpr (!ACC && EPI >= 0) epi_prefetch<T, 4, 4, EPI>(pre, g, m0 + wm * 64, n0 + wn * 64, lane & 15, lane >> 4);
+  constexpr bool pre_late = EPI < 0 || (GL && EPI == UWU_EPI_BIAS_TABLE);
+  if constexpr (!ACC && !pre_late) epi_prefetch<T, 4, 4, EPI>(pre, g, m0 + wm * 64, n0 + wn * 64, lane & 15, lane >> 4);
   f32x4 acc[4][4];
 #pragma unroll
   for (int i = 0; i < 4; ++i)
@@ -138,7 +139,7 @@
         }
       }
   } else {
-    if constexpr (EPI < 0) epi_prefetch<T, 4, 4, EPI>(pre, g, m0 + wm * 64, n0 + wn * 64, fr, fq);
+    if constexpr (pre_late) epi_prefetch<T, 4, 4, EPI>(pre, g, m0 + wm * 64, n0 + wn * 64, fr, fq);
     epilogue_tile<T, TC, 4, 4, EPI>(acc, pre, g, m0 + wm * 64, n0 + wn * 64, fr, fq, reinterpret_cast<float*>(smem), wm, wn);
   }
 }
@@ -260,7 +261,8 @@
 #pragma unroll
     for (int j = 0; j < 4; ++j) acc[i][j] = f32x4{0.f, 0.f, 0.f, 0.f};
   EpiPre<T, FI, 4> pre;
-  if constexpr (EPI >= 0) epi_prefetch<T, FI, 4, EPI>(pre, g, m0 + wm * 16 * FI, n0 + wn * 64, fr, fq);
+  constexpr bool pre_late = EPI < 0 || EPI == UWU_EPI_BIAS_TABLE;
+  if constexpr (!pre_late) epi_prefetch<T, FI, 4, EPI>(pre, g, m0 + wm * 16 * FI, n0 + wn * 64, fr, fq);
 
   const unsigned smem_base = (unsigned)(size_t)((const __attribute__((address_space(3))) char*)smem);
   const unsigned a_off = (unsigned)r_swz(wm * 16 * FI + fr, fq);
@@ -318,7 +320,7 @@
         for (int j = 0; j < 4; ++j) mma_frag<T>(bf[j], af[i], acc[i][j]);
     }
   }
-  if constexpr (EPI < 0) epi_prefetch<T, FI, 4, EPI>(pre, g, m0 + wm * 16 * FI, n0 + wn * 64, fr, fq);
+  if constexpr (pre_late) epi_prefetch<T, FI, 4, EPI>(pre, g, m0 + wm * 16 * FI, n0 + wn * 64, fr, fq);
   epilogue_tile<T, TC, FI, 4, EPI>(acc, pre, g, m0 + wm * 16 * FI, n0 + wn * 64, fr, fq, reinterpret_cast<float*>(smem),
                                    wm, wn);
 }
@@ -746,12 +748,11 @@
       if constexpr (sizeof(T) == 2) {
         if (ta == 1 && tb == 1) {
           const int tr = split > 1 ? uwu_gemm_pick_tr(g) : 0;
-          GemmArgs gt = g;
-          gt.bias = nullptr;
-          if (tr == 1) return uwu_launch_gemm_tr<8, 4>(gt, nullptr, 0, st);
-          if (tr == 2) return uwu_launch_gemm_tr<4, 8>(gt, nullptr, 0, st);
+          if (tr == 1) return uwu_launch_gemm_tr<8, 4>(g, nullptr, 0, st);
+          if (tr == 2) return uwu_launch_gemm_tr<4, 8>(g, nullptr, 0, st);
         }
       }
+      if (g.bias && ta == 1 && tb == 1) RETURN_IF(uwu_colsum(g.A, sizeof(T) == 2 ? UWU_BF16 : UWU_F32, g.K, g.M, g.lda, const_cast<float*>(g.bias), 1, st));
       if (ta == 1 && tb == 1) return launch<T, float, true, true, true>(g, split, st);
       if (ta == 0 && tb == 0) return launch<T, float, false, false, true>(g, split, st);
       if (ta == 0 && tb == 1) return launch<T, float, false, true, true>(g, split, st);
@@ -760,6 +761,13 @@
     return UWU_EINVAL;
   }
   constexpr bool hot = sizeof(T) == 2 && sizeof(TC) == 2;
+  if (g.epi == UWU_EPI_BIAS_TABLE) {
+    if constexpr (sizeof(T) == 2) {
+      if (pick_r3(g, false) == 8) return launch_r3<TC, UWU_EPI_BIAS_TABLE, false, 8>(g, st);
+    }
+    if (g.K % GT<T>::BK == 0) return launch<T, TC, false, false, false, true, UWU_EPI_BIAS_TABLE>(g, 1, st);
+    return launch<T, TC, false, false, false, false, UWU_EPI_BIAS_TABLE>(g, 1, st);
+  }
   if (ta == 0 && tb == 0) {
     if constexpr (hot) {
       if (uwu_gemm_p8_ok(g, false)) return uwu_launch_gemm_p8(g, false, st);
@@ -974,6 +982,7 @@
                     "gemm: aux missing/misaligned");
   } else {
     UWU_CHECK_ARG(c_dtype == UWU_F32 && ldc >= N, "gemm: ACCUM needs fp32 C");
+    UWU_CHECK_ARG(!bias || (transA && transB), "gemm: ACCUM takes a bias (+= column sums of A) with transA = transB = 1 only");
   }
   GemmArgs g{};
   g.A = A; g.B = B; g.C = C; g.C2 = C2; g.bias = bias; g.aux = aux;
@@ -996,3 +1005,29 @@
   }
   return dispatch_trans<float, float>(g, transA, transB, acc, split, st);
 }
+
+extern "C" int uwu_gemm_bias_table(const void* A, const void* B, void* C, const float* bias, const float* table, int table_rows,
+                                   int M, int N, int K, int lda, int ldb, int ldc, int dtype, int c_dtype, void* stream) {
+  UWU_CHECK_ARG(A && B && C && bias && table, "gemm_bias_table: null operand");
+  UWU_CHECK_ARG(M > 0 && N > 0 && K > 0 && table_rows > 0, "gemm_bias_table: bad shape M=%d N=%d K=%d table_rows=%d", M, N, K, table_rows);
+  UWU_CHECK_ARG(dtype == UWU_F32 || dtype == UWU_BF16, "gemm_bias_table: bad dtype %d", dtype);
+  UWU_CHECK_ARG(c_dtype == UWU_F32 || c_dtype == dtype, "gemm_bias_table: c_dtype must be fp32 or the operand dtype");
+  const int epc = dtype == UWU_BF16 ? 8 : 4;
+  UWU_CHECK_ARG((((uintptr_t)A | (uintptr_t)B | (uintptr_t)bias | (uintptr_t)table) & 15) == 0, "gemm_bias_table: A, B, bias and table must be 16-byte aligned");
+  UWU_CHECK_ARG(lda % epc == 0 && ldb % epc == 0 && K % epc == 0 && lda >= K && ldb >= K, "gemm_bias_table: K, lda, ldb must be multiples of %d, lda, ldb >= K", epc);
+  UWU_CHECK_ARG(N % 4 == 0 && ldc % 4 == 0 && ldc >= N && ((uintptr_t)C & (c_dtype == UWU_BF16 ? 7 : 15)) == 0, "gemm_bias_table: N and ldc must be multiples of 4, C aligned");
+  UWU_CHECK_ARG((int64_t)table_rows * N < ((int64_t)1 << 31), "gemm_bias_table: table too large");
+  GemmArgs g{};
+  g.A = A; g.B = B; g.C = C; g.bias = bias; g.tab = table; g.tab_rows = table_rows;
+  g.M = M; g.N = N; g.K = K; g.lda = lda; g.ldb = ldb; g.ldc = ldc; g.epi = UWU_EPI_BIAS_TABLE;
+  g.tiles_m = (M + BM - 1) / BM;
+  g.tiles_n = (N + BN - 1) / BN;
+  g.wide = (c_dtype == UWU_BF16 && N % 8 == 0 && ldc % 8 == 0 && ((uintptr_t)C & 15) == 0) ? 1 : 0;
+  g.k_tiles_per_split = (K + (dtype == UWU_BF16 ? 64 : 32) - 1) / (dtype == UWU_BF16 ? 64 : 32);
+  hipStream_t st = (hipStream_t)stream;
+  if (dtype == UWU_BF16) {
+    if (c_dtype == UWU_BF16) return dispatch_trans<bf16_t, bf16_t>(g, 0, 0, false, 1, st);
+    return dispatch_trans<bf16_t, float>(g, 0, 0, false, 1, st);
+  }
+  return dispatch_trans<float, float>(g, 0, 0, false, 1, st);
+}
diff --git a/uwudiff_amd/csrc/gemm_shared.h b/uwudiff_amd/csrc/gemm_shared.h
--- a/uwudiff_amd/csrc/gemm_shared.h
+++ b/uwudiff_amd/csrc/gemm_shared.h
@@ -24,6 +24,8 @@
   int M, N, K, lda, ldb, ldc, ldaux, epi, tiles_m, tiles_n, k_tiles_per_split, wide;
   int xs, nloc, part_m;
   int aux16;
+  const float* tab;
+  int tab_rows;
   int cH, cW, cC, cHo, cWo, cS;
   const void* zero;
   void* q8;
@@ -179,7 +181,18 @@
   typedef typename std::conditional<sizeof(T) == 2, uint2, f32x4>::type AuxRaw;
   f32x4 bias[FJ];
   AuxRaw aux[PD][FJ];
+  f32x4 tab[PD][FJ];
 };
+template <int FI, int FJ>
+__device__ __forceinline__ void epi_load_tab_row(const GemmArgs& g, int m_w, int n_w, int fr, int fq, int i, f32x4 (&dst)[FJ]) {
+  const int m = m_w + 16 * i + fr;
+  const float* row = g.tab + (int64_t)((unsigned)m % (unsigned)g.tab_rows) * g.N;
+#pragma unroll
+  for (int j = 0; j < FJ; ++j) {
+    const int n = n_w + 16 * j + 4 * fq;
+    dst[j] = (m < g.M && n < g.N) ? load4(row + n) : f32x4{0.f, 0.f, 0.f, 0.f};
+  }
+}
 template <typename T, int FI, int FJ>
 __device__ __forceinline__ void epi_load_aux_row(const GemmArgs& g, int m_w, int n_w, int fr, int fq, int i,
                                                  typename EpiPre<T, FI, FJ>::AuxRaw (&dst)[FJ]) {
@@ -212,7 +225,7 @@
 __device__ __forceinline__ void epi_prefetch(EpiPre<T, FI, FJ>& pre, const GemmArgs& g, int m_w, int n_w, int fr,
                                              int fq) {
   const int epi = EPI >= 0 ? EPI : g.epi;
-  const bool has_bias = epi == UWU_EPI_BIAS || epi == UWU_EPI_BIAS_GELU || epi == UWU_EPI_BIAS_SILU;
+  const bool has_bias = epi == UWU_EPI_BIAS || epi == UWU_EPI_BIAS_GELU || epi == UWU_EPI_BIAS_SILU || EPI == UWU_EPI_BIAS_TABLE;
 #pragma unroll
   for (int j = 0; j < FJ; ++j) {
     const int n = n_w + 16 * j + 4 * fq;
@@ -221,6 +234,10 @@
   if (epi == UWU_EPI_DGELU) {
 #pragma unroll
     for (int i = 0; i < EpiPre<T, FI, FJ>::PD; ++i) epi_load_aux_row<T, FI, FJ>(g, m_w, n_w, fr, fq, i, pre.aux[i]);
+  }
+  if constexpr (EPI == UWU_EPI_BIAS_TABLE) {
+#pragma unroll
+    for (int i = 0; i < EpiPre<T, FI, FJ>::PD; ++i) epi_load_tab_row<FI, FJ>(g, m_w, n_w, fr, fq, i, pre.tab[i]);
   }
 }
 
@@ -231,7 +248,7 @@
   TC* C = static_cast<TC*>(g.C);
   TC* C2 = static_cast<TC*>(g.C2);
   const int epi = EPI >= 0 ? EPI : g.epi;
-  const bool has_bias = epi == UWU_EPI_BIAS || epi == UWU_EPI_BIAS_GELU || epi == UWU_EPI_BIAS_SILU;
+  const bool has_bias = epi == UWU_EPI_BIAS || epi == UWU_EPI_BIAS_GELU || epi == UWU_EPI_BIAS_SILU || EPI == UWU_EPI_BIAS_TABLE;
   const bool two = epi == UWU_EPI_BIAS_GELU || epi == UWU_EPI_BIAS_SILU;
   const bool dgelu = epi == UWU_EPI_DGELU;
   constexpr int PD = EpiPre<T, FI, FJ>::PD;
@@ -308,6 +325,19 @@
       sec[j] = f32x4{0.f, 0.f, 0.f, 0.f};
       v[j] = (mok && n < g.N) ? finish(acc[i][j], pre.bias[j], arow[j], sec[j]) : acc[i][j];
       if (colsum && mok && n < g.N) add_cs(csum[j], v[j]);
+    }
+    if constexpr (EPI == UWU_EPI_BIAS_TABLE) {
+      f32x4(&trow)[FJ] = pre.tab[i % PD];
+#pragma unroll
+      for (int j = 0; j < FJ; ++j) {
+        f32x4 r = v[j];
+        if constexpr (sizeof(TC) == 2) {
+#pragma unroll
+          for (int e = 0; e < 4; ++e) r[e] = (float)(bf16_t)r[e];
+        }
+        v[j] = r + trow[j];
+      }
+      if (i + PD < FI) epi_load_tab_row<FI, FJ>(g, m_w, n_w, fr, fq, i + PD, trow);
     }
     if (dgelu && i + PD < FI) epi_load_aux_row<T, FI, FJ>(g, m_w, n_w, fr, fq, i + PD, arow);
     if (wide) {
diff --git a/uwudiff_amd/lib.py b/uwudiff_amd/lib.py
--- a/uwudiff_amd/lib.py
+++ b/uwudiff_amd/lib.py
@@ -109,6 +109,7 @@
     "uwu_allreduce_flat": (c_int, [P, P, c_int64, P]),
     "uwu_comm_destroy": (c_int, [P]),
     "uwu_gemm": (c_int, [P, P, P, P, P, P] + [c_int] * 13 + [P]),
+    "uwu_gemm_bias_table": (c_int, [P, P, P, P, P] + [c_int] * 9 + [P]),
     "uwu_gemm_last_kernel": (c_char_p, []),
     "uwu_gemm_fp8_scratch_bytes": (ctypes.c_size_t, [c_int, c_int, c_int]),
     "uwu_gemm_fp8": (c_int, [P, P, P, P, P, P] + [c_int] * 9 + [P, P, P, ctypes.c_size_t, P]),
@@ -173,6 +174,7 @@
     "uwu_silu_bwd": (c_int, [P, P, P, c_int64, c_int, P]),
     "uwu_add": (c_int, [P, P, P, c_int64, c_int, P]),
     "uwu_transpose_bf16": (c_int, [P, P, c_int, c_int, c_int, c_int, P]),
+    "uwu_transpose_bf16_batched": (c_int, [P, P, c_int, c_int, c_int, c_int, c_int, c_int64, c_int64, P]),
     "uwu_patchify": (c_int, [P, P, c_int, c_int, c_int, c_int, c_int, c_int, P]),
     "uwu_unpatchify": (c_int, [P, c_int, P, c_int, c_int, c_int, c_int, c_int, P]),
     "uwu_add_pos": (c_int, [P, P, c_int, c_int, c_int, c_int, P]),
@@ -196,6 +198,7 @@
     "uwu_nchw_to_cl": (c_int, [P, P, c_int, c_int, c_int, c_int, P]),
     "uwu_cl_to_nchw": (c_int, [P, P, c_int, c_int, c_int, c_int, P]),
     "uwu_dit_workspace_bytes": (c_size_t, [ctypes.POINTER(DitDesc)]),
+    "uwu_dit_workspace_region": (c_int, [ctypes.POINTER(DitDesc), c_char_p, c_int, ctypes.POINTER(c_size_t), ctypes.POINTER(c_size_t)]),
     "uwu_dit_forward": (c_int, [ctypes.POINTER(DitDesc), P, P, P, P, P]),
     "uwu_dit_backward": (c_int, [ctypes.POINTER(DitDesc), P, P]),
     "uwu_dit_backward_cond": (c_int, [ctypes.POINTER(DitDesc), P, P]),
```

Measured after the change: 17990 images/s. Within noise of the previous version (-0.0%).
